# HansiZeng/RIPOR

Hardware: AMD Instinct MI355X
Metric: queries/sec, t5-base beam=10 len=32 over 8.8M-doc trie (constrained beam search) (higher is better)
Workload: dtype f32 via f16x2-split MFMA (fp32 accumulate)

## Files before the change

include/ripor_hip.h:

```cpp
#ifndef RIPOR_HIP_H
#define RIPOR_HIP_H

#include <stdint.h>

#ifdef __cplusplus
extern "C" {
#endif

typedef enum {
  RPR_OK = 0,
  RPR_ERR_INVALID = -1,
  RPR_ERR_HIP = -2,
  RPR_ERR_NO_DEVICE = -3,
  RPR_ERR_OOM = -4
} rpr_status;

typedef struct rpr_ctx rpr_ctx;
typedef struct rpr_model rpr_model;
typedef struct rpr_trie rpr_trie;

typedef struct {
  int32_t vocab_size, d_model, d_kv, d_ff, num_heads;
  int32_t num_layers, num_decoder_layers;
  int32_t rel_buckets, rel_max_distance;
// ... 62 lines not shown
int rpr_abi_version(void);
int rpr_set_precision(rpr_ctx* ctx, int precision);
int rpr_get_precision(const rpr_ctx* ctx);

int rpr_rel_bucket(int rel, int bidirectional, int num_buckets, int max_distance);

int rpr_load_model(rpr_ctx* ctx, const rpr_model_desc* desc, rpr_model** out_model);
void rpr_free_model(rpr_model* model);

int rpr_build_trie(rpr_ctx* ctx, const uint16_t* codes, int64_t N, int32_t L, int32_t V, rpr_trie** out_trie);
void rpr_free_trie(rpr_trie* trie);
int64_t rpr_trie_num_rows(const rpr_trie* trie);
const int64_t* rpr_trie_perm(const rpr_trie* trie);
int rpr_trie_save(const rpr_trie* trie, const char* path);
int rpr_trie_build_file(const uint16_t* codes, int64_t N, int32_t L, int32_t V, const char* keys, int64_t key_bytes,
                        int64_t src_size, int64_t src_mtime_ns, const char* path);
int rpr_trie_file_info(const char* path, int64_t* N, int32_t* L, int32_t* V, int64_t* key_bytes, int64_t* src_size,
                       int64_t* src_mtime_ns);
int rpr_trie_load(rpr_ctx* ctx, const char* path, rpr_trie** out_trie);
int rpr_trie_file_validate(const char* path);
int rpr_trie_dims(const rpr_trie* trie, int64_t* N, int32_t* L, int32_t* V, int64_t* key_bytes);
int rpr_trie_keys(const rpr_trie* trie, char* out);
int rpr_trie_set_vocab(rpr_trie* trie, int32_t V);
int rpr_trie_mask(rpr_ctx* ctx, const rpr_trie* trie, const int32_t* prefix, int32_t R, int32_t T,
                  uint8_t* out_mask);

typedef struct rpr_d2s rpr_d2s;
int rpr_d2s_open(const char* path, rpr_d2s** out);
int rpr_d2s_dims(const rpr_d2s* h, int64_t* N, int32_t* L, int64_t* key_bytes);
int rpr_d2s_copy(const rpr_d2s* h, uint16_t* codes, char* keys);
void rpr_d2s_close(rpr_d2s* h);

int rpr_search(rpr_ctx* ctx, rpr_model* model, rpr_trie* trie, const int32_t* input_ids,
               const int32_t* attention_mask, int32_t Q, int32_t Lq, int32_t B, int32_t L, uint32_t flags,
               int32_t* out_tokens, float* out_scores, int64_t* out_row_lo, int64_t* out_row_hi,
               const rpr_debug_taps* taps, void* stream);

int rpr_search_margins(rpr_ctx* ctx, rpr_model* model, rpr_trie* trie, const int32_t* input_ids,
                       const int32_t* attention_mask, int32_t Q, int32_t Lq, int32_t B, int32_t L, uint32_t flags,
                       int32_t* out_tokens, float* out_scores, int64_t* out_row_lo, int64_t* out_row_hi,
                       double* out_margin, const rpr_debug_taps* taps, void* stream);

int rpr_set_lane_split(rpr_ctx* ctx, int32_t min_rows);
int32_t rpr_lane_split(rpr_ctx* ctx);

int rpr_set_forced_tail(rpr_ctx* ctx, int32_t mode);
int32_t rpr_forced_tail(const rpr_ctx* ctx);
int rpr_set_fork_depths(rpr_ctx* ctx, int32_t n, const int32_t* depths);
int rpr_fork_depths(rpr_ctx* ctx, rpr_model* model, rpr_trie* trie, int32_t Q, int32_t B, int32_t L, uint32_t flags,
                    int32_t* out_depths);
int rpr_set_l0_table(rpr_ctx* ctx, int32_t mode);
int64_t rpr_l0_table_bytes(const rpr_ctx* ctx, const rpr_model* model);
int rpr_trie_single_frac(const uint16_t* codes, int64_t N, int32_t Lc, int32_t L, double* out_frac);
int rpr_last_fork_stats(rpr_ctx* ctx, int32_t* out_depths, int32_t* out_forced, int32_t* out_left);

int rpr_lngknp_forward(rpr_ctx* ctx, rpr_model* model, const int32_t* input_ids, const int32_t* attention_mask,
                       int32_t bz, int32_t Lq, const int32_t* doc_codes, int32_t n_docs, int32_t L,
                       const float* teacher_pos, const float* teacher_neg, const int32_t* prefix_lens, int32_t n_prefix,
                       float* out_losses, float* out_position_scores, void* stream);

int64_t rpr_param_count(rpr_model* model);
int64_t rpr_param_total(rpr_model* model);
int rpr_param_info(rpr_model* model, int64_t index, const float** ptr, int64_t* numel, int64_t* offset);
int rpr_lngknp_backward(rpr_ctx* ctx, rpr_model* model, const int32_t* input_ids, const int32_t* attention_mask, int32_t bz,
                        int32_t Lq, const int32_t* doc_codes, int32_t L, const float* teacher_pos, const float* teacher_neg,
                        const int32_t* prefix_lens, int32_t n_prefix, float* out_losses, float* flat_grads, void* stream);
typedef void (*rpr_grad_bucket_cb)(void* user, int64_t offset, int64_t numel);
int rpr_lngknp_backward_buckets(rpr_ctx* ctx, rpr_model* model, const int32_t* input_ids, const int32_t* attention_mask,
                                int32_t bz, int32_t Lq, const int32_t* doc_codes, int32_t L, const float* teacher_pos,
                                const float* teacher_neg, const int32_t* prefix_lens, int32_t n_prefix, float* out_losses,
                                float* flat_grads, void* stream, void* comm_stream, rpr_grad_bucket_cb on_bucket, void* user);
int rpr_seq2seq_forward(rpr_ctx* ctx, rpr_model* model, const int32_t* input_ids, const int32_t* attention_mask, int32_t bz,
                        int32_t Lq, const int32_t* labels, int32_t L, float* out_loss, float* out_label_logprob, void* stream);
int rpr_seq2seq_backward(rpr_ctx* ctx, rpr_model* model, const int32_t* input_ids, const int32_t* attention_mask, int32_t bz,
                         int32_t Lq, const int32_t* labels, int32_t L, float* out_loss, float* flat_grads, void* stream);
int rpr_seq2seq_backward_buckets(rpr_ctx* ctx, rpr_model* model, const int32_t* input_ids, const int32_t* attention_mask,
                                 int32_t bz, int32_t Lq, const int32_t* labels, int32_t L, float* out_loss, float* flat_grads,
                                 void* stream, void* comm_stream, rpr_grad_bucket_cb on_bucket, void* user);
int rpr_adamw_step(rpr_ctx* ctx, rpr_model* model, const float* flat_grads, float* exp_avg, float* exp_avg_sq, int64_t step,
                   float lr, float beta1, float beta2, float eps, float weight_decay, float max_grad_norm,
                   float* out_grad_norm, void* stream);

#define RPR_STATUS_SATURATED 1u
#define RPR_STATUS_EMPTY_QUERY 2u
#define RPR_STATUS_TAIL_LEFTOVER 4u
int rpr_get_status(rpr_ctx* ctx, void* stream, uint32_t* out_flags, int clear);
int rpr_status_words_async(rpr_ctx* ctx, void* stream, uint32_t* host_words, int clear);
int rpr_model_f32_only(const rpr_model* model);

int rpr_profile_enable(rpr_ctx* ctx, int enable);
int rpr_profile_reset(rpr_ctx* ctx);
int rpr_profile_get(rpr_ctx* ctx, int kernel_class, rpr_kernel_stats* out);
int64_t rpr_workspace_bytes(const rpr_ctx* ctx);

int rpr_op_linear(rpr_ctx* ctx, const float* A, const float* W, const float* residual, float* C,
                  int32_t M, int32_t N, int32_t K, int32_t relu, void* stream);
int rpr_op_linear_bf16(rpr_ctx* ctx, const float* A, const float* W, const float* residual, float* C,
                       int32_t M, int32_t N, int32_t K, int32_t relu, int32_t n_products, void* stream);
int rpr_op_rmsnorm(rpr_ctx* ctx, const float* x, const float* w, float* out, int32_t rows, int32_t d,
                   float eps, void* stream);
int rpr_encode(rpr_ctx* ctx, rpr_model* model, const int32_t* input_ids, const int32_t* attention_mask,
               int32_t Q, int32_t Lq, float* out, void* stream);

int rpr_rq_train(rpr_ctx* ctx, const float* x, int64_t n, int32_t d, int32_t M, int32_t K, int32_t niter,
                 const int32_t* init_idx, float* codebooks, double* level_mse, void* stream);
int rpr_rq_encode(rpr_ctx* ctx, const float* x, int64_t n, int32_t d, const float* codebooks, int32_t M, int32_t K,
// ... 17 lines not shown
```

ripor_amd/_lib.py:

```python
from __future__ import annotations

import ctypes as C
import os
from typing import Optional

LIB_NAME = "libripor_hip_dev.so" if os.environ.get("RPR_DEV_LIB", "0") not in ("", "0") else "libripor_hip.so"
LIB_PATH = os.path.join(os.path.dirname(os.path.abspath(__file__)), LIB_NAME)

(K_GEMM, K_DEC_SELF_ATTN, K_DEC_CROSS_ATTN, K_ENC_ATTN, K_RMSNORM, K_SELECT, K_OTHER, K_GEMM_SMALL, K_TAIL_SELF_ATTN, K_FORK,
 K_COUNT) = range(11)
KERNEL_CLASS_NAMES = ["gemm", "dec_self_attn", "dec_cross_attn", "enc_attn", "rmsnorm", "select", "other", "gemm_small",
                      "tail_self_attn", "fork"]
STATUS_SATURATED, STATUS_EMPTY_QUERY, STATUS_TAIL_LEFTOVER = 1, 2, 4
ABI_VERSION = 4

PREC_F32, PREC_F16X2, PREC_BF16 = 0, 1, 2
FLAG_LOG_SOFTMAX = 1
FLAG_NO_GRAPH = 2


class RiporHipError(RuntimeError):
    pass


# ... 50 lines not shown
                                     C.POINTER(C.c_int64), C.POINTER(C.c_int64), C.POINTER(C.c_int64)]),
    "rpr_trie_file_validate": (C.c_int, [C.c_char_p]),
    "rpr_trie_dims": (C.c_int, [C.c_void_p, C.POINTER(C.c_int64), C.POINTER(C.c_int32), C.POINTER(C.c_int32),
                                C.POINTER(C.c_int64)]),
    "rpr_trie_keys": (C.c_int, [C.c_void_p, C.c_void_p]),
    "rpr_trie_set_vocab": (C.c_int, [C.c_void_p, C.c_int32]),
    "rpr_d2s_open": (C.c_int, [C.c_char_p, C.POINTER(C.c_void_p)]),
    "rpr_d2s_dims": (C.c_int, [C.c_void_p, C.POINTER(C.c_int64), C.POINTER(C.c_int32), C.POINTER(C.c_int64)]),
    "rpr_d2s_copy": (C.c_int, [C.c_void_p, C.c_void_p, C.c_void_p]),
    "rpr_d2s_close": (None, [C.c_void_p]),
    "rpr_trie_mask": (C.c_int, [C.c_void_p, C.c_void_p, C.c_void_p, C.c_int32, C.c_int32, C.c_void_p]),
    "rpr_search": (C.c_int, [C.c_void_p, C.c_void_p, C.c_void_p, C.c_void_p, C.c_void_p, C.c_int32, C.c_int32,
                             C.c_int32, C.c_int32, C.c_uint32, C.c_void_p, C.c_void_p, C.c_void_p, C.c_void_p,
                             C.POINTER(DebugTaps), C.c_void_p]),
    "rpr_search_margins": (C.c_int, [C.c_void_p, C.c_void_p, C.c_void_p, C.c_void_p, C.c_void_p, C.c_int32, C.c_int32,
                                     C.c_int32, C.c_int32, C.c_uint32, C.c_void_p, C.c_void_p, C.c_void_p, C.c_void_p,
                                     C.c_void_p, C.POINTER(DebugTaps), C.c_void_p]),
    "rpr_lngknp_forward": (C.c_int, [C.c_void_p, C.c_void_p, C.c_void_p, C.c_void_p, C.c_int32, C.c_int32, C.c_void_p,
                                     C.c_int32, C.c_int32, C.c_void_p, C.c_void_p, C.c_void_p, C.c_int32, C.c_void_p,
                                     C.c_void_p, C.c_void_p]),
    "rpr_param_count": (C.c_int64, [C.c_void_p]),
    "rpr_param_total": (C.c_int64, [C.c_void_p]),
    "rpr_param_info": (C.c_int, [C.c_void_p, C.c_int64, C.POINTER(C.c_void_p), C.POINTER(C.c_int64), C.POINTER(C.c_int64)]),
    "rpr_lngknp_backward": (C.c_int, [C.c_void_p, C.c_void_p, C.c_void_p, C.c_void_p, C.c_int32, C.c_int32, C.c_void_p, C.c_int32,
                                      C.c_void_p, C.c_void_p, C.c_void_p, C.c_int32, C.c_void_p, C.c_void_p, C.c_void_p]),
    "rpr_lngknp_backward_buckets": (C.c_int, [C.c_void_p, C.c_void_p, C.c_void_p, C.c_void_p, C.c_int32, C.c_int32, C.c_void_p,
                                              C.c_int32, C.c_void_p, C.c_void_p, C.c_void_p, C.c_int32, C.c_void_p, C.c_void_p,
                                              C.c_void_p, C.c_void_p, C.c_void_p, C.c_void_p]),
    "rpr_seq2seq_forward": (C.c_int, [C.c_void_p, C.c_void_p, C.c_void_p, C.c_void_p, C.c_int32, C.c_int32, C.c_void_p, C.c_int32,
                                      C.c_void_p, C.c_void_p, C.c_void_p]),
    "rpr_seq2seq_backward": (C.c_int, [C.c_void_p, C.c_void_p, C.c_void_p, C.c_void_p, C.c_int32, C.c_int32, C.c_void_p, C.c_int32,
                                       C.c_void_p, C.c_void_p, C.c_void_p]),
    "rpr_seq2seq_backward_buckets": (C.c_int, [C.c_void_p, C.c_void_p, C.c_void_p, C.c_void_p, C.c_int32, C.c_int32, C.c_void_p,
                                               C.c_int32, C.c_void_p, C.c_void_p, C.c_void_p, C.c_void_p, C.c_void_p, C.c_void_p]),
    "rpr_adamw_step": (C.c_int, [C.c_void_p, C.c_void_p, C.c_void_p, C.c_void_p, C.c_void_p, C.c_int64, C.c_float, C.c_float,
                                 C.c_float, C.c_float, C.c_float, C.c_float, C.c_void_p, C.c_void_p]),
    "rpr_get_status": (C.c_int, [C.c_void_p, C.c_void_p, C.POINTER(C.c_uint32), C.c_int]),
    "rpr_status_words_async": (C.c_int, [C.c_void_p, C.c_void_p, C.c_void_p, C.c_int]),
    "rpr_model_f32_only": (C.c_int, [C.c_void_p]),
    "rpr_profile_enable": (C.c_int, [C.c_void_p, C.c_int]),
    "rpr_profile_reset": (C.c_int, [C.c_void_p]),
    "rpr_profile_get": (C.c_int, [C.c_void_p, C.c_int, C.POINTER(KernelStats)]),
    "rpr_workspace_bytes": (C.c_int64, [C.c_void_p]),
    "rpr_set_lane_split": (C.c_int, [C.c_void_p, C.c_int32]),
    "rpr_lane_split": (C.c_int32, [C.c_void_p]),
    "rpr_set_l0_table": (C.c_int, [C.c_void_p, C.c_int32]),
    "rpr_l0_table_bytes": (C.c_int64, [C.c_void_p, C.c_void_p]),
    "rpr_set_forced_tail": (C.c_int, [C.c_void_p, C.c_int32]),
    "rpr_forced_tail": (C.c_int32, [C.c_void_p]),
    "rpr_set_fork_depths": (C.c_int, [C.c_void_p, C.c_int32, C.POINTER(C.c_int32)]),
    "rpr_fork_depths": (C.c_int, [C.c_void_p, C.c_void_p, C.c_void_p, C.c_int32, C.c_int32, C.c_int32, C.c_uint32,
                                  C.POINTER(C.c_int32)]),
    "rpr_trie_single_frac": (C.c_int, [C.c_void_p, C.c_int64, C.c_int32, C.c_int32, C.POINTER(C.c_double)]),
    "rpr_last_fork_stats": (C.c_int, [C.c_void_p, C.POINTER(C.c_int32), C.POINTER(C.c_int32), C.POINTER(C.c_int32)]),
    "rpr_op_linear": (C.c_int, [C.c_void_p, C.c_void_p, C.c_void_p, C.c_void_p, C.c_void_p, C.c_int32, C.c_int32,
                                C.c_int32, C.c_int32, C.c_void_p]),
    "rpr_op_linear_bf16": (C.c_int, [C.c_void_p, C.c_void_p, C.c_void_p, C.c_void_p, C.c_void_p, C.c_int32, C.c_int32,
                                     C.c_int32, C.c_int32, C.c_int32, C.c_void_p]),
    "rpr_op_rmsnorm": (C.c_int, [C.c_void_p, C.c_void_p, C.c_void_p, C.c_void_p, C.c_int32, C.c_int32, C.c_float,
                                 C.c_void_p]),
    "rpr_encode": (C.c_int, [C.c_void_p, C.c_void_p, C.c_void_p, C.c_void_p, C.c_int32, C.c_int32, C.c_void_p,
                             C.c_void_p]),
    "rpr_rq_train": (C.c_int, [C.c_void_p, C.c_void_p, C.c_int64, C.c_int32, C.c_int32, C.c_int32, C.c_int32,
                               C.POINTER(C.c_int32), C.c_void_p, C.POINTER(C.c_double), C.c_void_p]),
    "rpr_rq_encode": (C.c_int, [C.c_void_p, C.c_void_p, C.c_int64, C.c_int32, C.c_void_p, C.c_int32, C.c_int32,
                                C.c_void_p, C.POINTER(C.c_double), C.c_void_p]),
    "rpr_rq_encode_beam": (C.c_int, [C.c_void_p, C.c_void_p, C.c_int64, C.c_int32, C.c_void_p, C.c_int32, C.c_int32, C.c_int32,
                                     C.c_void_p, C.POINTER(C.c_double), C.c_void_p]),
    "rpr_embed": (C.c_int, [C.c_void_p, C.c_void_p, C.c_void_p, C.c_void_p, C.c_int32, C.c_int32, C.c_void_p, C.c_void_p]),
    "rpr_rq_search": (C.c_int, [C.c_void_p, C.c_void_p, C.c_int32, C.c_int32, C.c_void_p, C.c_int32, C.c_int32, C.c_void_p,
                                C.c_int64, C.c_int32, C.c_void_p, C.c_void_p, C.c_void_p]),
    "rpr_flat_search": (C.c_int, [C.c_void_p, C.c_void_p, C.c_int32, C.c_int32, C.c_void_p, C.c_int64, C.c_int64, C.c_int32,
                                  C.c_void_p, C.c_void_p, C.c_int32, C.c_void_p]),
}

_lib: Optional[C.CDLL] = None


def load() -> C.CDLL:
    global _lib
    if _lib is not None:
        return _lib
    if not os.path.exists(LIB_PATH):
        raise RiporHipError(
            f"{LIB_PATH} not found: build it with `python -c 'import __graft_entry__ as g; g.build()'` "
            "(hipcc --offload-arch=gfx950). There is no CPU fallback for the search path.")
    import torch
    hip_rt = os.path.join(os.path.dirname(torch.__file__), "lib", "libamdhip64.so")
    if os.path.exists(hip_rt):
        C.CDLL(hip_rt, mode=C.RTLD_GLOBAL)
    lib = C.CDLL(LIB_PATH)
    for name, (res, args) in SIGNATURES.items():
        fn = getattr(lib, name)
        fn.restype = res
        fn.argtypes = args
    _lib = lib
    return lib


def check(status: int, what: str = "") -> None:
    if status != 0:
        msg = load().rpr_last_error()
        raise RiporHipError(f"{what or 'libripor_hip'} failed (status {status}): "
                            f"{msg.decode('utf-8', 'replace') if msg else ''}")
```

ripor_amd/csrc/api.hip:

```cpp
#include <algorithm>
#include <cmath>
#include <cstdio>
#include <cstdlib>
#include <cstring>
#include <map>
#include <memory>
#include <tuple>
#include <vector>

#include "internal.h"

namespace rpr {

static thread_local std::string g_err;
void set_error(const std::string& msg) { g_err = msg; }
int hip_fail(hipError_t e, const char* what, const char* file, int line) {
  g_err = std::string("HIP error ") + hipGetErrorName(e) + " (" + hipGetErrorString(e) + ") in " + what + " at " +
          file + ":" + std::to_string(line);
  (void)hipGetLastError();
  return e == hipErrorOutOfMemory ? RPR_ERR_OOM : RPR_ERR_HIP;
}

int rel_bucket(int rel, int bidirectional, int num_buckets, int max_distance) {
  int bucket = 0, n;
  if (bidirectional) {
    num_buckets /= 2;
    if (rel > 0) bucket += num_buckets;
    n = rel < 0 ? -rel : rel;
  } else {
    n = rel < 0 ? -rel : 0;
  }
  const int max_exact = num_buckets / 2;
  if (n < max_exact) return bucket + n;
  const float v = logf((float)n / (float)max_exact) / (float)log((double)max_distance / (double)max_exact) *
                  (float)(num_buckets - max_exact);
  int large = max_exact + (int)v;
  if (large > num_buckets - 1) large = num_buckets - 1;
  return bucket + large;
}

int compute_logit_bound(rpr_ctx* c, rpr_model* m, hipStream_t s, float* out) {
  const auto& d = m->d;
  float* slot = reinterpret_cast<float*>(c->status + 9);
  RPR_HIP(hipMemsetAsync(slot, 0, 4, s));
  RPR_HIP(launch_max_row_norm(d.out_embeds, d.dec_final_ln, d.L * d.V, d.d_model, slot, s));
  float mx = 0.f;
  RPR_HIP(hipMemcpyAsync(&mx, slot, 4, hipMemcpyDeviceToHost, s));
  RPR_HIP(hipStreamSynchronize(s));
  const float post = d.scaleup_output_hidden ? (float)pow((double)d.d_model, -0.5) : 1.0f;
  *out = 1.001f * mx * sqrtf((float)d.d_model) * post + 1.0f;
  return RPR_OK;
}

int refresh_weight_planes(rpr_ctx* c, rpr_model* m, hipStream_t s) {
  unsigned int* probe = c->status + 8;
  RPR_HIP(hipMemsetAsync(probe, 0, 4, s));
  for (const auto& j : m->plane_jobs)
    RPR_HIP(launch_split_planes(j.w, j.dst, j.n, j.plane_stride ? j.plane_stride : j.n, s, W_PLANE_SCALE * j.pre, j.ln, m->d.d_model, probe));
  unsigned int sat = 0;
  RPR_HIP(hipMemcpyAsync(&sat, probe, 4, hipMemcpyDeviceToHost, s));
  RPR_HIP(hipStreamSynchronize(s));
  m->f32_only = sat != 0;
  m->l0_valid = false;
  float lb = m->logit_bound;
  const int e = compute_logit_bound(c, m, s, &lb);
  if (e) return e;
  if (lb != m->logit_bound) {
    m->logit_bound = lb;
    for (auto it = c->graphs.begin(); it != c->graphs.end();) {
      if (it->first.m == m) { (void)hipGraphExecDestroy(it->second); it = c->graphs.erase(it); } else ++it;
    }
  }
  return RPR_OK;
}

}

using namespace rpr;

namespace {

struct PrecGuard {
  rpr_ctx* c; int saved;
  PrecGuard(rpr_ctx* c_, const rpr_model* m) : c(c_), saved(c_->precision) {
    if (c->precision == RPR_PREC_BF16) c->precision = RPR_PREC_F16X2;
    if (m && m->f32_only) c->precision = RPR_PREC_F32;
  }
  ~PrecGuard() { c->precision = saved; }
};

int flush_profile(rpr_ctx* c) {
  std::map<const int*, int> live;
  for (auto& r : c->recs) {
    RPR_HIP(hipEventSynchronize(r.b));
    float ms = 0.f;
    RPR_HIP(hipEventElapsedTime(&ms, r.a, r.b));
    double scale = 1.0;
    if (r.live_dev && r.live_static > 0) {
      auto it = live.find(r.live_dev);
      if (it == live.end()) {
        int n = r.live_static;
        RPR_HIP(hipMemcpy(&n, r.live_dev, sizeof(int), hipMemcpyDeviceToHost));
        it = live.emplace(r.live_dev, n).first;
      }
      scale = (double)std::min(std::max(it->second, 0), r.live_static) / (double)r.live_static;
    }
    auto& d = c->done[r.cls];
    d.total_ms += ms; d.launches += 1; d.flops += r.flops * scale; d.bytes += r.bytes * scale;
    c->pool.push_back(r.a); c->pool.push_back(r.b);
  }
  c->recs.clear();
  return 0;
}

}

extern "C" {

int rpr_abi_version(void) { return 4; }
const char* rpr_last_error(void) { return g_err.c_str(); }

int rpr_rel_bucket(int rel, int bidirectional, int num_buckets, int max_distance) {
  return rel_bucket(rel, bidirectional, num_buckets, max_distance);
}

int rpr_init(int device, rpr_ctx** out_ctx) {
// ... 240 lines not shown

int64_t rpr_trie_num_rows(const rpr_trie* t) { return t ? t->N : 0; }
const int64_t* rpr_trie_perm(const rpr_trie* t) { return t ? t->perm.data() : nullptr; }

int rpr_trie_save(const rpr_trie* t, const char* path) {
  RPR_REQUIRE(t && path, "NULL argument");
  if (save_trie_file(path, t->host_sorted, t->perm, t->N, t->L, t->V, t->keys, 0, 0) != 0) {
    set_error(std::string("cannot write trie file ") + path);
    return RPR_ERR_INVALID;
  }
  return RPR_OK;
}

int rpr_trie_build_file(const uint16_t* codes, int64_t N, int32_t L, int32_t V, const char* keys, int64_t key_bytes,
                        int64_t src_size, int64_t src_mtime_ns, const char* path) {
  RPR_REQUIRE(codes && path, "NULL argument");
  RPR_REQUIRE(N > 0 && N < ((int64_t)1 << 31) - 1, "N out of range");
  RPR_REQUIRE(L >= 1 && L <= 4096 && V >= 1 && V <= 65536, "L or V out of range");
  RPR_REQUIRE(key_bytes >= 0 && (key_bytes == 0 || keys), "keys missing");
  for (int64_t i = 0; i < N * L; ++i) RPR_REQUIRE(codes[i] < V, "code >= V");
  try {
    std::vector<uint16_t> sorted;
    std::vector<int64_t> perm;
    sort_codes(codes, N, L, sorted, perm);
    const std::string k = key_bytes ? std::string(keys, (size_t)key_bytes) : std::string();
    if (save_trie_file(path, sorted, perm, N, L, V, k, src_size, src_mtime_ns) != 0) {
      set_error(std::string("cannot write trie file ") + path);
      return RPR_ERR_INVALID;
    }
  } catch (const std::exception& ex) {
    set_error(std::string("rpr_trie_build_file: ") + ex.what());
    return RPR_ERR_OOM;
  }
  return RPR_OK;
}

int rpr_trie_single_frac(const uint16_t* codes, int64_t N, int32_t Lc, int32_t L, double* out_frac) {
  RPR_REQUIRE(codes && out_frac, "NULL argument");
  RPR_REQUIRE(N > 0 && N < ((int64_t)1 << 31) - 1 && Lc >= 1 && Lc <= 4096 && L >= 1 && L <= Lc, "N, Lc or L out of range");
  try {
    std::vector<uint16_t> sorted;
    std::vector<int64_t> perm;
    sort_codes(codes, N, Lc, sorted, perm);
    std::vector<double> f;
    trie_single_frac(sorted.data(), N, Lc, L, f);
    for (int t = 0; t <= L; ++t) out_frac[t] = f[(size_t)t];
  } catch (const std::exception& ex) {
    set_error(std::string("rpr_trie_single_frac: ") + ex.what());
    return RPR_ERR_OOM;
  }
  return RPR_OK;
}

int rpr_trie_file_info(const char* path, int64_t* N, int32_t* L, int32_t* V, int64_t* key_bytes, int64_t* src_size,
                       int64_t* src_mtime_ns) {
  RPR_REQUIRE(path, "NULL argument");
  int64_t h[6];
  if (trie_file_info(path, h) != 0) { set_error(std::string("not a readable RPRTRIE2 file: ") + path); return RPR_ERR_INVALID; }
  if (N) *N = h[0];
  if (L) *L = (int32_t)h[1];
  if (V) *V = (int32_t)h[2];
  if (key_bytes) *key_bytes = h[3];
  if (src_size) *src_size = h[4];
  if (src_mtime_ns) *src_mtime_ns = h[5];
  return RPR_OK;
}

int rpr_trie_file_validate(const char* path) {
  RPR_REQUIRE(path, "NULL argument");
  try {
    std::vector<uint16_t> sorted; std::vector<int64_t> perm; std::string keys, err;
    int64_t N; int L, V;
    if (load_trie_file(path, sorted, perm, N, L, V, keys, err) != 0) {
      set_error(std::string("invalid trie file ") + path + ": " + err);
      return RPR_ERR_INVALID;
    }
  } catch (const std::exception& ex) {
    set_error(std::string("rpr_trie_file_validate: ") + ex.what());
    return RPR_ERR_OOM;
  }
  return RPR_OK;
}

int rpr_trie_load(rpr_ctx* c, const char* path, rpr_trie** out) {
  RPR_REQUIRE(c && path && out, "NULL argument");
  try {
    auto t = std::make_unique<rpr_trie>();
    t->ctx = c;
    std::string err;
    if (load_trie_file(path, t->host_sorted, t->perm, t->N, t->L, t->V, t->keys, err) != 0) {
      set_error(std::string("cannot load trie file ") + path + ": " + err);
      return RPR_ERR_INVALID;
    }
    int e = upload_trie(c, t);
    if (e) return e;
    *out = t.release();
  } catch (const std::exception& ex) {
    set_error(std::string("rpr_trie_load: ") + ex.what());
    return RPR_ERR_OOM;
  }
  return RPR_OK;
}

int rpr_trie_dims(const rpr_trie* t, int64_t* N, int32_t* L, int32_t* V, int64_t* key_bytes) {
  RPR_REQUIRE(t, "NULL trie");
  if (N) *N = t->N;
// ... 61 lines not shown
  DevTmp dp, dm;
  RPR_HIP(dp.alloc((size_t)R * T * 4));
  RPR_HIP(dm.alloc((size_t)R * t->V));
  RPR_HIP(hipMemcpy(dp.p, prefix, (size_t)R * T * 4, hipMemcpyHostToDevice));
  RPR_HIP(launch_prefix_mask(t->codes, t->L, t->N, dp.as<int32_t>(), R, T, t->V, dm.as<uint8_t>(), nullptr));
  RPR_HIP(hipMemcpy(out_mask, dm.p, (size_t)R * t->V, hipMemcpyDeviceToHost));
  return RPR_OK;
}

}

namespace {

bool ensure_lanes(rpr_ctx* c) {
  if (c->lanes_state) return c->lanes_state > 0;
  c->lanes_state = -1;
  hipDeviceProp_t prop;
  if (hipGetDeviceProperties(&prop, c->device) != hipSuccess) { (void)hipGetLastError(); return false; }
  const int cus = prop.multiProcessorCount, words = (cus + 31) / 32;
  if (cus < 64 || words > 32) return false;
  c->lane_cus = cus / 2;
  for (int i = 0; i < 2; ++i) {
    uint32_t mask[32] = {0};
    for (int k = (i == 0 ? 0 : cus / 2); k < (i == 0 ? cus / 2 : cus); ++k) mask[k >> 5] |= 1u << (k & 31);
    if (hipExtStreamCreateWithCUMask(&c->lanes[i].stream, (uint32_t)words, mask) != hipSuccess ||
        hipEventCreateWithFlags(&c->lanes[i].done, hipEventDisableTiming) != hipSuccess) {
      (void)hipGetLastError();
      return false;
    }
  }
  if (hipEventCreateWithFlags(&c->fork_ev, hipEventDisableTiming) != hipSuccess) { (void)hipGetLastError(); return false; }
  c->lanes_state = 1;
  return true;
}

std::vector<int> choose_forks(rpr_ctx* c, const rpr_model* m, rpr_trie* tr, int Q, int B, int L, unsigned flags, bool taps,
                              bool* drop_last) {
  std::vector<int> forks;
  *drop_last = false;
  if (!c->forced_tail || taps || L < 3 || !std::isfinite(m->logit_bound)) return forks;
  const double per_step = 2.0 * (double)m->logit_bound + ((flags & RPR_FLAG_LOG_SOFTMAX) ? log((double)m->d.V) : 0.0);
  if (1e8 - L * per_step <= 1e7) return forks;
  if (c->n_fork_override >= 0) {
    int prev = 0;
    for (int i = 0; i < c->n_fork_override; ++i) {
      const int t = c->fork_override[i];
      if (t > prev && t <= L - 1) { forks.push_back(t); prev = t; }
    }
    *drop_last = c->forced_tail == 2 && !forks.empty();
    return forks;
  }
  auto it = tr->single_frac.find(L);
  if (it == tr->single_frac.end()) {
    std::vector<double> f;
    trie_single_frac(tr->host_sorted.data(), tr->N, tr->L, L, f);
    it = tr->single_frac.emplace(L, std::move(f)).first;
  }
  const std::vector<double>& f = it->second;
  auto p_forced = [&](int t) { return std::pow(f[(size_t)t], (double)B); };
  int t0 = 0;
  for (int t = 1; t <= L - 2 && !t0; ++t) if (p_forced(t) >= 0.5) t0 = t;
  const int min_tail = (int64_t)Q * B <= 4096 ? 2 : 8;
  if (!t0 || L - t0 < min_tail) return forks;
  forks.push_back(t0);
  if (c->forced_tail == 2 && (double)Q * (1.0 - p_forced(t0)) <= 0.05) { *drop_last = true; return forks; }
  for (int t = t0 + 1; t <= L - 2 && t <= t0 + 12; ++t)
    if ((double)Q * (1.0 - p_forced(t)) <= 0.05) { forks.push_back(t); break; }
  *drop_last = c->forced_tail == 2 && forks.size() == 2;
  return forks;
}

int pack_forks(const std::vector<int>& forks, bool drop_last) {
  int v = drop_last ? (1 << 30) : 0;
  for (size_t i = 0; i < forks.size(); ++i) v |= forks[i] << (8 * i);
  return v;
}

int search_one(rpr_ctx* c, rpr_model* m, rpr_trie* tr, const int32_t* input_ids, const int32_t* attention_mask, int32_t Q,
               int32_t Lq, int32_t B, int32_t L, uint32_t flags, int32_t* out_tokens, float* out_scores, int64_t* out_row_lo,
               int64_t* out_row_hi, double* out_margin, const rpr_debug_taps* taps, hipStream_t s, int lane) {
  struct WsGuard {
    rpr_ctx* c; int lane;
    WsGuard(rpr_ctx* c_, int l) : c(c_), lane(l) { if (lane >= 0) { std::swap(c->ws, c->lanes[lane].ws); c->cur_cus = c->lane_cus; c->cur_lane = lane; } }
    ~WsGuard() { if (lane >= 0) { std::swap(c->ws, c->lanes[lane].ws); c->cur_cus = 0; c->cur_lane = -1; } }
  } ws_guard(c, lane);
  PrecGuard prec_guard(c, m);
  bool drop_last = false;
  const std::vector<int> forks = choose_forks(c, m, tr, Q, B, L, flags, taps != nullptr, &drop_last);
  int e = alloc_workspace(c, m, Q, Lq, B, L, forks, drop_last, (flags & RPR_FLAG_LOG_SOFTMAX) != 0);
  if (e) return e;
  c->last_forks = forks;
  c->last_ws_mask |= lane >= 0 ? (2 << lane) : 1;
  Workspace& w = c->ws;
  const size_t T = (size_t)Q * Lq, R = (size_t)Q * B;
  RPR_HIP(hipMemcpyAsync(w.ids.p, input_ids, T * 4, hipMemcpyDeviceToDevice, s));
  RPR_HIP(hipMemcpyAsync(w.mask.p, attention_mask, T * 4, hipMemcpyDeviceToDevice, s));

  const bool eager = (flags & RPR_FLAG_NO_GRAPH) || taps || c->profiling;
  if (eager) {
    Launcher Ln{c, s};
    enqueue_search(Ln, c, m, tr, Q, Lq, B, L, flags, taps, forks, drop_last);
    if (Ln.err) return Ln.err;
  } else {
    auto env_int = [](const char* n, int dflt) { const char* e = getenv(n); return e ? atoi(e) : dflt; };
    const unsigned dbg = (env_int("RPR_TAIL_RANK_REPLAY", 0) ? 1u : 0u) | ((unsigned)(env_int("RPR_SELECT_RADIX", -1) + 1) << 1);
    const unsigned l0 = m->l0_ready(c) ? (unsigned)c->l0_mode : 0u;
    const unsigned mg = c->cur_margins ? 1u : 0u;
    GraphKey key{m, tr, Q, Lq, B, L, flags | ((unsigned)c->precision << 16) | (dbg << 20) | (l0 << 24) | (mg << 28), lane,
                 pack_forks(forks, drop_last)};
    auto it = c->graphs.find(key);
    if (it == c->graphs.end()) {
      hipGraph_t graph = nullptr;
      RPR_HIP(hipStreamBeginCapture(c->cap_stream, hipStreamCaptureModeThreadLocal));
      Launcher Ln{c, c->cap_stream};
      enqueue_search(Ln, c, m, tr, Q, Lq, B, L, flags, nullptr, forks, drop_last);
      hipError_t ce = hipStreamEndCapture(c->cap_stream, &graph);
      if (Ln.err) { if (graph) (void)hipGraphDestroy(graph); return Ln.err; }
      if (ce != hipSuccess) return hip_fail(ce, "hipStreamEndCapture", __FILE__, __LINE__);
      hipGraphExec_t exec = nullptr;
      hipError_t ie = hipGraphInstantiate(&exec, graph, nullptr, nullptr, 0);
      (void)hipGraphDestroy(graph);
      if (ie != hipSuccess) return hip_fail(ie, "hipGraphInstantiate", __FILE__, __LINE__);
      it = c->graphs.emplace(key, exec).first;
    }
    RPR_HIP(hipGraphLaunch(it->second, s));
  }
  RPR_HIP(hipMemcpyAsync(out_tokens, w.o_tokens.p, R * (size_t)L * 4, hipMemcpyDeviceToDevice, s));
  RPR_HIP(hipMemcpyAsync(out_scores, w.o_scores.p, R * 4, hipMemcpyDeviceToDevice, s));
  if (out_row_lo) RPR_HIP(hipMemcpyAsync(out_row_lo, w.o_lo.p, R * 8, hipMemcpyDeviceToDevice, s));
  if (out_row_hi) RPR_HIP(hipMemcpyAsync(out_row_hi, w.o_hi.p, R * 8, hipMemcpyDeviceToDevice, s));
  if (out_margin) RPR_HIP(hipMemcpyAsync(out_margin, w.o_margin.p, (size_t)Q * 8, hipMemcpyDeviceToDevice, s));
  return RPR_OK;
}

int search_entry(rpr_ctx* c, rpr_model* m, rpr_trie* tr, const int32_t* input_ids, const int32_t* attention_mask,
                 int32_t Q, int32_t Lq, int32_t B, int32_t L, uint32_t flags, int32_t* out_tokens, float* out_scores,
                 int64_t* out_row_lo, int64_t* out_row_hi, double* out_margin, const rpr_debug_taps* taps, void* stream) {
  RPR_REQUIRE(c && m && tr && input_ids && attention_mask && out_tokens && out_scores, "NULL argument");
  struct MarginMode { rpr_ctx* c; MarginMode(rpr_ctx* c_, bool on) : c(c_) { c->cur_margins = on ? 1 : 0; } ~MarginMode() { c->cur_margins = 0; } }
      margin_mode(c, out_margin != nullptr);
  RPR_REQUIRE(m->ctx == c && tr->ctx == c, "model/trie belong to another ctx");
  RPR_REQUIRE(Q >= 1 && B >= 1 && B <= 65535, "Q or B out of range");
  RPR_REQUIRE(Lq >= 1 && Lq <= MAX_LQ, "Lq out of range (1..256)");
  RPR_REQUIRE(L >= 1 && L <= m->d.L && L <= tr->L, "L exceeds the model's decoder length or the trie depth");
  RPR_REQUIRE(tr->V == m->d.V, "trie V differs from the model's decoder vocab size");
  RPR_REQUIRE((int64_t)Q * B < ((int64_t)1 << 24), "Q*B too large");
  RPR_REQUIRE((int64_t)Q * B * m->d.num_heads < ((int64_t)1 << 32) / std::max<int64_t>(B, m->d.num_heads),
              "Q * num_beams * num_heads too large for this beam count: search fewer queries per call");
  RPR_REQUIRE(select_fits(B, m->Vp()), "num_beams * decoder vocab size too large for the select kernel (about 1600 beams at V=256)");
  RPR_REQUIRE(!taps || m->Vp() == m->d.V, "debug taps need a decoder vocab size that is a multiple of 64");
  RPR_HIP(hipSetDevice(c->device));
  hipStream_t s = reinterpret_cast<hipStream_t>(stream);
  { const int pe = ensure_weight_planes(c, m, s); if (pe) return pe; }
  { const int te = ensure_l0_table(c, m, s); if (te) return te; }
  c->last_ws_mask = 0;
  if (c->lane_min_rows > 0 && (int64_t)Q * B >= c->lane_min_rows && Q >= 2 && !taps && ensure_lanes(c)) {
    const int32_t Qh[2] = {(Q + 1) / 2, Q / 2};
    for (int i = 0; i < 2; ++i) {
      std::swap(c->ws, c->lanes[i].ws);
      int e;
      {
        PrecGuard prec_guard(c, m);
// ... 14 lines not shown
                         out_tokens + r0 * L, out_scores + r0, out_row_lo ? out_row_lo + r0 : nullptr,
                         out_row_hi ? out_row_hi + r0 : nullptr, out_margin ? out_margin + q0 : nullptr, nullptr, ln.stream, i);
      if (e) {
        for (int k = 0; k < 2; ++k) (void)hipStreamSynchronize(c->lanes[k].stream);
        return e;
      }
      RPR_HIP(hipEventRecord(ln.done, ln.stream));
      q0 += Qh[i];
    }
    for (int i = 0; i < 2; ++i) RPR_HIP(hipStreamWaitEvent(s, c->lanes[i].done, 0));
    return RPR_OK;
  }
  return search_one(c, m, tr, input_ids, attention_mask, Q, Lq, B, L, flags, out_tokens, out_scores, out_row_lo, out_row_hi, out_margin,
                    taps, s, -1);
}

}

extern "C" {

int rpr_search(rpr_ctx* c, rpr_model* m, rpr_trie* tr, const int32_t* input_ids, const int32_t* attention_mask,
               int32_t Q, int32_t Lq, int32_t B, int32_t L, uint32_t flags, int32_t* out_tokens, float* out_scores,
               int64_t* out_row_lo, int64_t* out_row_hi, const rpr_debug_taps* taps, void* stream) {
  return search_entry(c, m, tr, input_ids, attention_mask, Q, Lq, B, L, flags, out_tokens, out_scores, out_row_lo, out_row_hi,
                      nullptr, taps, stream);
}

int rpr_search_margins(rpr_ctx* c, rpr_model* m, rpr_trie* tr, const int32_t* input_ids, const int32_t* attention_mask,
                       int32_t Q, int32_t Lq, int32_t B, int32_t L, uint32_t flags, int32_t* out_tokens, float* out_scores,
                       int64_t* out_row_lo, int64_t* out_row_hi, double* out_margin, const rpr_debug_taps* taps, void* stream) {
  RPR_REQUIRE(out_margin != nullptr, "out_margin is NULL");
  return search_entry(c, m, tr, input_ids, attention_mask, Q, Lq, B, L, flags, out_tokens, out_scores, out_row_lo, out_row_hi,
                      out_margin, taps, stream);
}

int rpr_set_lane_split(rpr_ctx* c, int32_t min_rows) {
  RPR_REQUIRE(c && min_rows >= 0, "NULL ctx or negative threshold");
  c->lane_min_rows = min_rows;
  return RPR_OK;
}
int32_t rpr_lane_split(rpr_ctx* c) {
  if (!c || c->lane_min_rows <= 0) return 0;
  (void)hipSetDevice(c->device);
  return ensure_lanes(c) ? c->lane_min_rows : 0;
}

int rpr_set_l0_table(rpr_ctx* c, int32_t mode) {
  RPR_REQUIRE(c && mode >= 0 && mode <= 2, "mode must be 0 (never), 1 (where the ping-pong GEMM would run) or 2 (always)");
  c->l0_mode = mode;
  return RPR_OK;
}
int64_t rpr_l0_table_bytes(const rpr_ctx* c, const rpr_model* m) { return c && m && m->l0_ready(c) ? (int64_t)m->l0_bytes() : 0; }

int rpr_set_forced_tail(rpr_ctx* c, int32_t mode) {
  RPR_REQUIRE(c && mode >= 0 && mode <= 2, "mode must be 0 (off), 1 (exact) or 2 (optimistic)");
  c->forced_tail = mode;
  return RPR_OK;
}
int32_t rpr_forced_tail(const rpr_ctx* c) { return c ? c->forced_tail : -1; }

int rpr_set_fork_depths(rpr_ctx* c, int32_t n, const int32_t* depths) {
  RPR_REQUIRE(c && n >= -1 && n <= MAX_FORKS && (n <= 0 || depths), "n out of range (-1 = automatic, 0..2 explicit depths)");
  c->n_fork_override = n;
  for (int i = 0; i < n; ++i) {
    RPR_REQUIRE(depths[i] >= 1 && depths[i] < 256 && (i == 0 || depths[i] > depths[i - 1]), "fork depths must be ascending and >= 1");
    c->fork_override[i] = depths[i];
  }
  return RPR_OK;
}

int rpr_fork_depths(rpr_ctx* c, rpr_model* m, rpr_trie* tr, int32_t Q, int32_t B, int32_t L, uint32_t flags, int32_t* out_depths) {
  RPR_REQUIRE(c && m && tr && out_depths, "NULL argument");
  RPR_REQUIRE(Q >= 1 && B >= 1 && L >= 1 && L <= tr->L, "Q, B or L out of range");
  bool drop_last = false;
  const std::vector<int> f = choose_forks(c, m, tr, Q, B, L, flags, false, &drop_last);
  for (size_t i = 0; i < f.size(); ++i) out_depths[i] = f[i];
  return (int)f.size();
}

int rpr_last_fork_stats(rpr_ctx* c, int32_t* out_depths, int32_t* out_forced, int32_t* out_left) {
  RPR_REQUIRE(c && out_depths && out_forced && out_left, "NULL argument");
  RPR_HIP(hipSetDevice(c->device));
  RPR_HIP(hipDeviceSynchronize());
  const int n = (int)c->last_forks.size();
  for (int k = 0; k < n; ++k) {
    out_depths[k] = c->last_forks[(size_t)k]; out_forced[k] = 0; out_left[k] = 0;
    const Workspace* wss[3] = {&c->ws, &c->lanes[0].ws, &c->lanes[1].ws};
    for (int i = 0; i < 3; ++i) {
      if (!(c->last_ws_mask & (1 << i)) || !wss[i]->tail[k].cnt.p || !wss[i]->stage[k].cnt.p) continue;
      int32_t a = 0, b = 0;
      RPR_HIP(hipMemcpy(&a, wss[i]->tail[k].cnt.p, 4, hipMemcpyDeviceToHost));
      RPR_HIP(hipMemcpy(&b, wss[i]->stage[k].cnt.p, 4, hipMemcpyDeviceToHost));
      out_forced[k] += a; out_left[k] += b;
    }
  }
  return n;
}

int rpr_lngknp_forward(rpr_ctx* c, rpr_model* m, const int32_t* input_ids, const int32_t* attention_mask, int32_t bz,
                       int32_t Lq, const int32_t* doc_codes, int32_t n_docs, int32_t L, const float* teacher_pos,
                       const float* teacher_neg, const int32_t* prefix_lens, int32_t n_prefix, float* out_losses,
                       float* out_position_scores, void* stream) {
  RPR_REQUIRE(c && m && input_ids && attention_mask && doc_codes, "NULL argument");
  RPR_REQUIRE(m->ctx == c, "model belongs to another ctx");
  RPR_REQUIRE(bz >= 1 && Lq >= 1 && Lq <= MAX_LQ, "bz or Lq out of range");
  RPR_REQUIRE(L >= 1 && L <= m->d.L && L <= MAX_LQ, "smtid length exceeds the model's decoder length");
  RPR_REQUIRE(n_docs >= 1 && (int64_t)bz * n_docs * L < ((int64_t)1 << 24), "n_docs out of range");
  RPR_REQUIRE(m->d.d_kv == DKV, "the teacher-forced kernels are written for d_kv == 64 (t5-base / t5-large)");
  RPR_REQUIRE(n_prefix >= 0 && n_prefix <= 8, "n_prefix out of range (0..8)");
  RPR_REQUIRE(n_prefix == 0 || (n_docs == 2 && teacher_pos && teacher_neg && prefix_lens && out_losses),
              "the margin losses need n_docs == 2 (positive, negative), teacher scores, prefix lengths and out_losses");
  RPR_REQUIRE(out_losses || out_position_scores, "nothing to return");
  RPR_HIP(hipSetDevice(c->device));
  hipStream_t s = reinterpret_cast<hipStream_t>(stream);
  int e = ensure_weight_planes(c, m, s);
  if (e) return e;
  e = alloc_train_workspace(c, m, bz, Lq, n_docs, L);
  if (e) return e;
  Workspace& w = c->ws;
  const size_t T = (size_t)bz * Lq, R = (size_t)bz * n_docs * L;
  RPR_HIP(hipMemcpyAsync(w.ids.p, input_ids, T * 4, hipMemcpyDeviceToDevice, s));
  RPR_HIP(hipMemcpyAsync(w.mask.p, attention_mask, T * 4, hipMemcpyDeviceToDevice, s));
  float* scores = P<float>(w.tr_misc);
  int32_t* codes = reinterpret_cast<int32_t*>(scores + R);
  RPR_HIP(hipMemcpyAsync(codes, doc_codes, R * 4, hipMemcpyDeviceToDevice, s));
  PrecGuard prec_guard(c, m);
  Launcher Ln{c, s};
  enqueue_train_forward(Ln, c, m, bz, Lq, n_docs, L, codes, scores);
  if (Ln.err) return Ln.err;
  if (n_prefix > 0)
    RPR_HIP(launch_margin_mse(scores, teacher_pos, teacher_neg, prefix_lens, n_prefix, bz, L, out_losses, nullptr, s));
  if (out_position_scores) RPR_HIP(hipMemcpyAsync(out_position_scores, scores, R * 4, hipMemcpyDeviceToDevice, s));
  return RPR_OK;
}

int rpr_encode(rpr_ctx* c, rpr_model* m, const int32_t* input_ids, const int32_t* attention_mask, int32_t Q,
               int32_t Lq, float* out, void* stream) {
  RPR_REQUIRE(c && m && input_ids && attention_mask && out, "NULL argument");
  RPR_REQUIRE(Q >= 1 && Lq >= 1 && Lq <= MAX_LQ, "Q or Lq out of range");
  RPR_HIP(hipSetDevice(c->device));
  hipStream_t s = reinterpret_cast<hipStream_t>(stream);
  int e = ensure_weight_planes(c, m, s);
  if (e) return e;
  e = alloc_workspace(c, m, Q, Lq, 1, 1);
// ... 157 lines not shown
```

ripor_amd/csrc/common.h:

```cpp
#pragma once
#include <hip/hip_runtime.h>
#include <hip/hip_fp16.h>
#include <stdint.h>
#include <stdlib.h>
#include <string>

#include "../../include/ripor_hip.h"

namespace rpr {

constexpr int WAVE = 64;
constexpr int MAX_LQ = 256;
constexpr int MAX_DEC_LEN = 64;
constexpr int DKV = 64;

#ifdef RPR_DEV_SWITCHES
inline const char* dev_getenv(const char* name) { return getenv(name); }
#else
inline const char* dev_getenv(const char*) { return nullptr; }
#endif

void set_error(const std::string& msg);
int hip_fail(hipError_t e, const char* what, const char* file, int line);

// ... 341 lines not shown
  const int* nq_dev;
};
hipError_t launch_select(const SelectArgs& a, hipStream_t s);
bool select_radix_fits(int B, int V);
bool select_radix_wanted(int B, int V);
size_t select_radix_ws_bytes(int Q, int B, int V);
void select_radix_carve(RadixWs& w, void* base, int32_t* chi, int Q, int B, int V);
hipError_t init_select_radix_attributes();
hipError_t launch_select_radix_reset(const RadixWs& w, int Q, hipStream_t s);
hipError_t launch_select_radix(const SelectArgs& a, hipStream_t s);
bool select_fits(int B, int V);

struct MarginArgs {
  const float* logits;
  const double* cur_score;
  const double* nxt_score;
  const unsigned long long* valid;
  const uint16_t* codes; int Lc, t;
  const int32_t* cur_lo; const int32_t* cur_hi;
  int Q, B, V, Vreal, log_softmax, shared0;
  const int* nq_dev;
  const int32_t* qmap;
  double* out;
};
constexpr int MARGIN_MAX_V = 65536;
hipError_t launch_margin_init(double* out, int Q, hipStream_t s);
hipError_t launch_prune_margin(const MarginArgs& a, hipStream_t s);

struct FinalizeArgs {
  BeamState st;
  int Q, B, L;
  int32_t* out_tokens;
  float* out_scores;
  int64_t* out_lo;
  int64_t* out_hi;
  const int* nq_dev;
  const int32_t* qmap;
};
hipError_t launch_finalize(const FinalizeArgs& a, hipStream_t s);

hipError_t launch_prefix_mask(const uint16_t* codes, int Lc, int64_t N, const int32_t* prefix, int R, int T,
                              int V, uint8_t* out_mask, hipStream_t s);
hipError_t launch_zero_u64(unsigned long long* p, size_t n, hipStream_t s);
hipError_t launch_mask_lengths(const int32_t* mask, int32_t* lens, int Q, int Lq, hipStream_t s,
                               unsigned int* status = nullptr);

struct ForkArgs {
  BeamState st;
  const uint16_t* codes; int Lc;
  int Qcap; const int* nq_dev;
  int B, T, L;
  double spread_max;
  int32_t* flag;
};
hipError_t launch_fork_classify(const ForkArgs& a, hipStream_t s);
hipError_t launch_fork_scan(const int32_t* flag, int Qcap, const int* nq_dev, int B, int Lt, int32_t* flist, int32_t* tail_cnt,
                            int32_t* src, int32_t* next_cnt, hipStream_t s);
struct StageIO {
  const int32_t* qmap;
  const int32_t* offs;
  const int32_t* last;
  const int32_t* mask;
};
struct StageOut { int32_t* qmap; int32_t* offs; int32_t* last; int32_t* mask; };
hipError_t launch_gather_stage_io(const StageIO& src, const StageOut& dst, const int32_t* list, const int* n_dev, int Qcap, int Lq,
                                  hipStream_t s);
hipError_t launch_compact_beams(const BeamState& from, const BeamState& to, const int32_t* src, const int* n_dev, int Qcap, int B, int T,
                                hipStream_t s);
struct KvCopyArgs {
  const float* k_from; const float* v_from; float* k_to; float* v_to;
  size_t layer_from, q_from, h_from;
  size_t layer_to, q_to, h_to;
  const int32_t* src; const int* n_dev;
  int Qcap, nd, H, n;
};
hipError_t launch_kv_copy(const KvCopyArgs& a, hipStream_t s);
hipError_t launch_tail_tokens(const BeamState& st, const uint16_t* codes, int Lc, const int32_t* flist, const int* nf_dev, int Qcap,
                              int B, int T, int L, uint16_t* tokens, hipStream_t s);
hipError_t launch_tail_embed(const float* in_embeds, const uint16_t* tokens, float* out, int rows, const int* rows_dev, int T, int L,
                             int d, int V, hipStream_t s, XOut xo = XOut{});
hipError_t launch_tail_l0_qkv(const float* table, const uint16_t* tokens, float* qkv, int rows, const int* rows_dev, int T, int L,
                              int V, int n3, hipStream_t s);
struct TailSelfAttnArgs {
  const float* qkv;
  const float* kcache;
  const float* vcache;
  size_t q_stride, h_stride, pos_stride, slot_stride;
  const uint16_t* anc; int anc_ld;
  const int32_t* flist;
  const int* nseq_dev;
  const float* rel_bias; const int32_t* bucket;
  float* out; __half* out_h; size_t o_ps; unsigned int* sat;
  int nseq_cap, B, H, T, L;
  int dkv = 0;
};
hipError_t launch_tail_self_attn(const TailSelfAttnArgs& a, hipStream_t s);
hipError_t launch_tail_cross_attn(const DecCrossAttnArgs& a, hipStream_t s);
hipError_t launch_step_cross_attn(const DecCrossAttnArgs& a, hipStream_t s);
hipError_t launch_tail_gold(const float* x, const float* ln, const float* out_embeds, const uint16_t* tokens, float* gold, int rows,
                            const int* rows_dev, int T, int L, int d, int V, float eps, float post, hipStream_t s,
                            const __half* x_h = nullptr, size_t x_ps = 0);
hipError_t launch_tail_logprob(const float* logits, const uint16_t* tokens, float* gold, int rows, const int* rows_dev, int T, int L,
                               int V, hipStream_t s);
struct TailRankArgs {
  BeamState st;
  const int32_t* flist; const int32_t* qmap; const int* nf_dev;
  const uint16_t* tokens;
  const float* gold;
  int Qcap, B, T, L;
  int32_t* out_tokens; float* out_scores; int64_t* out_lo; int64_t* out_hi;
  int replay = 0;
};
hipError_t launch_tail_rank(const TailRankArgs& a, hipStream_t s);
hipError_t launch_flag_nonzero(const int* cnt, unsigned int* flag, hipStream_t s);
hipError_t launch_max_row_norm(const float* E, const float* w, int rows, int d, float* out , hipStream_t s);
hipError_t init_tail_kernel_attributes();

hipError_t launch_train_dec_embed(const float* start, const float* in_embeds, const int32_t* codes, float* out, int S,
                                  int L, int d, int V, hipStream_t s, XOut xo = XOut{});
hipError_t launch_gold_scores(const float* x, const float* ln, const float* out_embeds, const int32_t* codes, float* scores,
                              int S, int L, int d, int V, float eps, float post, hipStream_t s,
                              const __half* x_h = nullptr, size_t x_ps = 0, float* hidden = nullptr);
hipError_t launch_margin_mse(const float* scores, const float* teacher_pos, const float* teacher_neg, const int32_t* prefix_lens,
                             int n_prefix, int bz, int L, float* losses, float* margins, hipStream_t s);
hipError_t init_train_kernel_attributes();
hipError_t launch_absmax2(const float* x0, size_t n0, const float* x1, size_t n1, float* out, hipStream_t s);
hipError_t launch_split_dyn(const float* x, int R, int C, int ldi, __half* out, const float* amax, hipStream_t s);
hipError_t launch_split_dyn_T(const float* x, int R, int C, int ldi, int Rpad, __half* out_t, __half* out_plain, const float* amax,
                              hipStream_t s);
hipError_t launch_to_bf16(const float* x, int R, int C, int ldi, void* out, hipStream_t s);
hipError_t launch_to_bf16_T(const float* x, int R, int C, int ldi, int Rpad, void* out_t, void* out_plain, hipStream_t s,
                            const float* relu_act = nullptr, int ldt = 0);
struct WSeg { const float* src; int R, C; unsigned long long off; };
hipError_t launch_weights_bf16(const WSeg* segs, const int* pref, int nseg, int ntiles, void* plain, void* tr, hipStream_t s);
hipError_t launch_transpose_pad(const float* in, float* out, int R, int C, int ldi, int Rpad, hipStream_t s);
hipError_t launch_relu_bwd(float* dy, const float* act, size_t n, hipStream_t s);
hipError_t launch_rmsnorm_bf16_T(const float* x, const float* w, int rows, int d, float eps, float post, void* out_plain, void* out_t,
                                 int Rpad, int ldt, hipStream_t s);
hipError_t launch_rmsnorm_bwd(const float* x, const float* w, const float* dh, const float* dres, float* dx_out, float* w_part,
                              float* dw, int rows, int d, float eps, float post, int accumulate_dw, hipStream_t s);
struct ColsumSites {
  static constexpr int MAXS = 4;
  const float* part[MAXS]; float* out[MAXS]; int nparts[MAXS]; int n;
};
int rmsnorm_bwd_parts(int rows);
hipError_t launch_colsum_multi(const ColsumSites& p, int d, hipStream_t s);
size_t self_attn_bwd_smem(int Ls, int buckets);
hipError_t launch_self_attn_bwd(const float* qkv, const float* dO, const int32_t* mask, const float* rel_bias, const int32_t* bucket,
                                float* dqkv, float* dbias_part, float* dbias, int S, int Ls, int H, int buckets, int causal,
                                hipStream_t s);
size_t cross_attn_bwd_smem(int n, int Lq);
hipError_t launch_cross_attn_bwd(const float* q, const float* xk, const float* xv, int xld, const int32_t* mask, const float* dO,
                                 float* dq, float* dxk, float* dxv, int bz, int n, int Lq, int H, hipStream_t s);
hipError_t launch_scatter_rows_fix(const float* src, const int32_t* idx, unsigned long long* acc, int rows, int d, hipStream_t s);
hipError_t launch_fix_flush(unsigned long long* acc, float* dst, size_t n, hipStream_t s);
hipError_t launch_train_indices(const int32_t* codes, int32_t* in_idx, int32_t* out_idx, int S, int L, int V, hipStream_t s);
hipError_t launch_sum_selected_rows(const float* src, const int32_t* sel, float* out, int rows, int d, hipStream_t s);
hipError_t launch_margin_mse_bwd(const float* margins, const float* teacher_pos, const float* teacher_neg, const int32_t* prefix_lens,
                                 int n_prefix, int bz, int L, float* dscores, hipStream_t s);
hipError_t launch_gold_score_bwd(const float* x, const float* ln, const float* out_embeds, const int32_t* out_idx, const float* dscores,
                                 float* dh, float* de, int rows, int d, float eps, float post, hipStream_t s);
int s2s_head_smem_ok(int V);
hipError_t launch_s2s_head_fwd(const float* hF, const float* E, const int32_t* labels, float* dlogits, float* row_loss, float* label_lp,
                               float* loss, int bz, int L, int d, int V, hipStream_t s);
// ... 10 lines not shown
```

ripor_amd/csrc/internal.h:

```cpp
#pragma once
#include <map>
#include <memory>
#include <string>
#include <tuple>
#include <type_traits>
#include <vector>

#include "common.h"
#include "gemm_route.h"
#include "trie.h"

namespace rpr {

struct DevBuf {
  void* p = nullptr;
  size_t cap = 0;
};

}

using rpr::DevBuf;

struct rpr_model {
  rpr_ctx* ctx;
// ... 9 lines not shown
  int Vp() const { return (d.V + 63) & ~63; }
  bool f32_only = false;
  bool planes_dirty = false;
  float* l0_table = nullptr;
  bool l0_valid = false;
  unsigned l0_epoch = 0;
  int l0_state = 0;
  size_t l0_rows() const { return rpr::l0_table_rows(d.L, d.V); }
  size_t l0_bytes() const { return rpr::l0_table_bytes(d.L, d.V, inner()); }
  bool l0_ready(const rpr_ctx* c) const;
  std::vector<void*> owned;
  struct PlaneJob { const float* w; size_t n; __half* dst; const float* ln; float pre; size_t plane_stride; };
  std::vector<PlaneJob> plane_jobs;
  struct ParamRef { int kind; int layer; float* ptr; size_t numel; size_t offset; };
  std::vector<ParamRef> params;
  size_t params_total = 0;
  float logit_bound = INFINITY;
  int inner() const { return d.num_heads * d.d_kv; }
  ~rpr_model() {
    if (enc_bucket) (void)hipFree(enc_bucket);
    if (dec_bucket) (void)hipFree(dec_bucket);
    for (void* p : owned) (void)hipFree(p);
  }
};

struct rpr_trie {
  rpr_ctx* ctx;
  int64_t N;
  int L, V;
  uint16_t* codes = nullptr;
  int32_t* lvl0 = nullptr;
  int32_t* lvl1 = nullptr;
  int lvl_V = 0;
  int32_t* idx2 = nullptr;
  int32_t* d_start[rpr::TRIE_MAX_DEEP] = {};
  uint16_t* d_tok[rpr::TRIE_MAX_DEEP] = {};
  int d_n[rpr::TRIE_MAX_DEEP] = {};
  int n_deep = 0;
  void free_levels() {
    if (lvl0) (void)hipFree(lvl0);
    if (lvl1) (void)hipFree(lvl1);
    if (idx2) (void)hipFree(idx2);
    for (int i = 0; i < rpr::TRIE_MAX_DEEP; ++i) {
      if (d_start[i]) (void)hipFree(d_start[i]);
      if (d_tok[i]) (void)hipFree(d_tok[i]);
      d_start[i] = nullptr; d_tok[i] = nullptr; d_n[i] = 0;
    }
    lvl0 = lvl1 = idx2 = nullptr; n_deep = 0; lvl_V = 0;
  }
  std::vector<int64_t> perm;
  std::vector<uint16_t> host_sorted;
  std::string keys;
  std::map<int, std::vector<double>> single_frac;
  ~rpr_trie() { if (codes) (void)hipFree(codes); free_levels(); }
};

struct rpr_d2s {
  std::vector<uint16_t> codes;
  std::string keys;
  int64_t N = 0;
  int L = 0;
};

struct GraphKey {
  const rpr_model* m; const rpr_trie* t; int Q, Lq, B, L; unsigned flags; int lane;
  int forks;
  bool operator<(const GraphKey& o) const {
    return std::tie(m, t, Q, Lq, B, L, flags, lane, forks) < std::tie(o.m, o.t, o.Q, o.Lq, o.B, o.L, o.flags, o.lane, o.forks);
  }
};

struct StageBufs {
  DevBuf qmap;
  DevBuf cnt;
  DevBuf src;
  DevBuf offs, last, mask;
  DevBuf kcache, vcache;
  DevBuf score[2], lo[2], hi[2], tokens[2], anc[2];
};
struct TailBufs {
  DevBuf flag, flist;
  DevBuf cnt;
  DevBuf qmap, offs, last, mask;
  DevBuf tokens;
  DevBuf gold;
};
constexpr int MAX_FORKS = 2;

struct Workspace {
  DevBuf ids, mask, last, offs, row_src, ex, eh, eqkv, eattn, eff, enc_out, xkv;
  DevBuf x, h, q, attn, ff, logits, kcache, vcache, lb;
  DevBuf sel_rs;
  DevBuf score[2], lo[2], hi[2], tokens[2], anc[2];
  DevBuf o_tokens, o_scores, o_lo, o_hi;
  DevBuf mg_valid, o_margin;
  DevBuf eattn_h, eff_h, enc_out_h, attn_h, ff_h, ex_h, x_h, ssq_e, ssq_d;
  DevBuf tr_x, tr_misc;
  DevBuf part;
  StageBufs stage[MAX_FORKS];
  TailBufs tail[MAX_FORKS];
  DevBuf t_x, t_h, t_qkv, t_q, t_attn, t_ff, t_x_h, t_attn_h, t_ff_h, t_ssq;
  DevBuf t_logits;
  DevBuf rq_r, rq_code, rq_hist, rq_order, rq_cnorm, rq_part, rq_idx;
  DevBuf rq_lut, rq_sel;
  DevBuf flat_sc;
  DevBuf rq_r2, rq_bnorm, rq_cand, rq_bhist;
};

static_assert(sizeof(Workspace) % sizeof(DevBuf) == 0 && std::is_standard_layout<Workspace>::value,
              "Workspace must consist of DevBuf members only (rpr_free_ctx walks it as an array)");

struct Lane {
  Workspace ws;
  hipStream_t stream = nullptr;
  hipEvent_t done = nullptr;
};

struct rpr_ctx {
  int device;
  int precision = RPR_PREC_F16X2;
  unsigned int* status = nullptr;
  unsigned int* status_host = nullptr;
  struct TrainWs* tws = nullptr;
  Workspace ws;
  Lane lanes[2];
  int lanes_state = 0;
  int lane_min_rows = 10240;
  hipEvent_t fork_ev = nullptr;
  int cur_cus = 0;
  int lane_cus = 0;
  int cur_lane = -1;
  int cur_no_row_split = 0;
  int cur_small_live = 0;
  int cur_margins = 0;
  int forced_tail = 1;
  int fork_override[MAX_FORKS] = {0, 0};
  int n_fork_override = -1;
  std::vector<int> last_forks;
  int last_ws_mask = 0;
  size_t ws_bytes = 0;
  int enc_rows_accounted = 0;
  unsigned l0_epoch = 0;
  int l0_mode = 1;
  hipStream_t cap_stream = nullptr;
  std::map<GraphKey, hipGraphExec_t> graphs;
  bool profiling = false;
  struct Rec { int cls; hipEvent_t a, b; double flops, bytes; const int* live_dev; int live_static; };
  std::vector<Rec> recs;
  std::vector<hipEvent_t> pool;
  rpr_kernel_stats done[RPR_K_COUNT];
};

inline bool rpr_model::l0_ready(const rpr_ctx* c) const { return c->l0_mode > 0 && l0_table && l0_valid && l0_epoch == c->l0_epoch; }

namespace rpr {

int refresh_weight_planes(rpr_ctx* c, rpr_model* m, hipStream_t s);
inline int ensure_weight_planes(rpr_ctx* c, rpr_model* m, hipStream_t s) {
  if (!m->planes_dirty) return 0;
  const int e = refresh_weight_planes(c, m, s);
  if (!e) m->planes_dirty = false;
  return e;
}
int ensure_l0_table(rpr_ctx* c, rpr_model* m, hipStream_t s);
void free_train_ws(rpr_ctx* c);
void train_forget_model(rpr_ctx* c, const rpr_model* m);

inline int ensure(rpr_ctx* c, DevBuf& b, size_t bytes) {
  if (bytes <= b.cap) return 0;
  if (b.p) {
    RPR_HIP(hipFree(b.p));
    c->ws_bytes -= b.cap;
    b.p = nullptr; b.cap = 0;
    for (auto& g : c->graphs) (void)hipGraphExecDestroy(g.second);
    c->graphs.clear();
  }
  const size_t want = (bytes + 255) & ~(size_t)255;
  RPR_HIP(hipMalloc(&b.p, want));
  b.cap = want;
  c->ws_bytes += want;
  return 0;
}

template <class T> T* P(const DevBuf& b) { return reinterpret_cast<T*>(b.p); }

struct DevTmp {
  void* p = nullptr;
  hipError_t alloc(size_t bytes) { return hipMalloc(&p, bytes); }
  ~DevTmp() { if (p) (void)hipFree(p); }
  template <class T> T* as() const { return reinterpret_cast<T*>(p); }
};

struct Launcher {
  rpr_ctx* c;
  hipStream_t s;
  int err = 0;
  const int* live_dev = nullptr;
  int live_static = 0;
  void account_live(const int* dev, int rows_static) { live_dev = dev; live_static = rows_static; }
  hipEvent_t get_event() {
    if (!c->pool.empty()) { hipEvent_t e = c->pool.back(); c->pool.pop_back(); return e; }
    hipEvent_t e = nullptr;
    if (hipEventCreate(&e) != hipSuccess) return nullptr;
    return e;
  }
  template <class F> void run(int cls, double flops, double bytes, F&& f, const int* cls_after = nullptr) {
    if (err) return;
    hipEvent_t ea = nullptr, eb = nullptr;
    if (c->profiling) {
// ... 46 lines not shown
```

ripor_amd/csrc/passes.hip:

```cpp
#include <cmath>
#include <vector>

#include "internal.h"

namespace rpr {

LinOut out_f32(float* p, int ld, int N, const float* resid, int relu) {
  LinOut o{};
  o.f[0] = o.f[1] = o.f[2] = p; o.ldo[0] = o.ldo[1] = o.ldo[2] = ld; o.split_n = N; o.resid = resid; o.relu = relu;
  return o;
}

namespace {

GemmH2Args h2_args(const rpr_ctx* c, const LinIn& A, const LinW& W, int M, const LinOut& O, const int* m_dev) {
  const int Nh = W.Nh ? W.Nh : W.N;
  GemmH2Args g{};
  g.A = A.h; g.a_ps = A.ps; g.lda = A.ld; g.W = W.h; g.w_ps = W.ps ? W.ps : (size_t)W.N * W.K; g.ldw = W.K;
  g.resid = O.resid; g.ldr = O.ldo[0];
  for (int i = 0; i < 3; ++i) { g.out[i] = O.f[i]; g.ldo[i] = O.ldo[i]; }
  g.split_n = O.split_n; g.out_h = O.h; g.o_ps = O.ps; g.ldoh = O.ldh;
  g.M = M; g.N = Nh; g.K = W.K; g.relu = O.relu;
  g.rm_B = O.rm_B; g.rm_stride = O.rm_stride; g.rm_slot = O.rm_slot; g.rm_head = O.rm_head; g.rm_dshift = O.rm_dshift;
  g.m_dev = m_dev; g.acc_scale = 1.0f / (W_PLANE_SCALE * A.scale); g.plane_scale = O.plane_scale;
  g.row_ssq = A.ssq; g.inv_d_fix = A.inv_d_fix; g.eps = A.eps;
  g.resid_h = O.resid_h; g.r_ps = O.ps; g.ldrh = O.ldh; g.ssq_out = O.ssq_out;
  g.sat = c->status;
  g.cus = c->cur_cus;
  g.small_live = m_dev ? c->cur_small_live : 0;
  g.no_row_split = W.row_split_ok ? 0 : c->cur_no_row_split;
  g.force_pp = W.force_pp ? 1 : 0;
  if (!W.no_scratch) { g.part = P<float>(c->ws.part); g.part_cap = c->ws.part.cap / sizeof(float); g.mid_split = 1; }
  return g;
}

}

void linear(Launcher& L, const LinIn& A, const LinW& W, int M, const LinOut& O, const int* m_dev, int m_acc) {
  const double Ma = m_acc >= 0 ? m_acc : M;
  const double fl = 2.0 * Ma * (double)W.N * W.K;
  const double by = 4.0 * (Ma * W.K + (double)W.N * W.K + Ma * W.N * ((O.resid || O.resid_h) ? 2 : 1));
  hipStream_t s = L.s;
  if (L.c->precision == RPR_PREC_F16X2) {
    GemmH2Args g = h2_args(L.c, A, W, M, O, m_dev);
    L.run(RPR_K_GEMM, fl, by, [&] { return launch_gemm_h2(g, s); }, &g.kernel_cls);
  } else {
    GemmArgs g{};
    g.A = A.f; g.lda = A.ld; g.W = W.f; g.ldw = W.K; g.resid = O.resid; g.ldr = O.ldo[0];
    for (int i = 0; i < 3; ++i) { g.out[i] = O.f[i]; g.ldo[i] = O.ldo[i]; }
    g.split_n = O.split_n; g.M = M; g.N = W.N; g.K = W.K; g.relu = O.relu;
    g.rm_B = O.rm_B; g.rm_stride = O.rm_stride; g.rm_slot = O.rm_slot; g.rm_head = O.rm_head; g.rm_dshift = O.rm_dshift;
    g.m_dev = m_dev;
    L.run(RPR_K_GEMM, fl, by, [&] { return launch_gemm(g, s); });
  }
}

int alloc_workspace(rpr_ctx* c, const rpr_model* m, int Q, int Lq, int B, int L, const std::vector<int>& forks, bool drop_last, bool log_softmax) {
  const auto& d = m->d;
  const size_t T = (size_t)Q * Lq, R = (size_t)Q * B, inner = m->inner(), dm = d.d_model, dff = d.d_ff;
  const size_t nd = d.num_decoder_layers, ne = d.num_layers, f = sizeof(float);
  Workspace& w = c->ws;
  int e = 0;
  auto E = [&](DevBuf& b, size_t bytes) { if (!e) e = ensure(c, b, bytes); };
  E(w.ids, T * 4); E(w.mask, T * 4); E(w.last, (size_t)Q * 4); E(w.offs, ((size_t)Q + 1) * 4); E(w.row_src, T * 4);
  E(w.ex, T * dm * f); E(w.eh, T * dm * f); E(w.eqkv, T * 3 * inner * f); E(w.eattn, T * inner * f);
  E(w.eff, T * dff * f); E(w.enc_out, T * dm * f); E(w.xkv, T * nd * 2 * inner * f);
  E(w.x, R * dm * f); E(w.h, R * dm * f); E(w.q, R * inner * f); E(w.attn, R * inner * f);
  E(w.ff, R * dff * f); E(w.logits, R * (size_t)m->Vp() * f);
  const size_t depth0 = forks.empty() ? (size_t)L : (size_t)forks[0];
  E(w.kcache, nd * depth0 * R * inner * f); E(w.vcache, nd * depth0 * R * inner * f);
  E(w.lb, R * (size_t)m->Vp() * 4 * 2);
  if (select_radix_wanted(B, m->Vp())) E(w.sel_rs, select_radix_ws_bytes(Q, B, m->Vp()));
  for (int i = 0; i < 2; ++i) {
    E(w.score[i], R * 8); E(w.lo[i], R * 4); E(w.hi[i], R * 4);
    E(w.tokens[i], R * (size_t)L * 2); E(w.anc[i], R * (size_t)L * 2);
  }
  E(w.o_tokens, R * (size_t)L * 4); E(w.o_scores, R * 4); E(w.o_lo, R * 8); E(w.o_hi, R * 8);
  if (c->cur_margins) { E(w.mg_valid, R * (size_t)m->Vp() / 8); E(w.o_margin, (size_t)Q * 8); }
  const size_t hb = sizeof(__half) * 2;
  E(w.eattn_h, T * inner * hb); E(w.eff_h, T * dff * hb); E(w.enc_out_h, T * dm * hb);
  E(w.attn_h, R * inner * hb); E(w.ff_h, R * dff * hb);
  E(w.ex_h, T * dm * hb); E(w.x_h, R * dm * hb);
  E(w.ssq_e, (2 * ne + 1) * T * 8); E(w.ssq_d, (3 * nd + 1) * R * 8);
  E(w.part, (size_t)9 << 20 << 2);
  for (size_t k = 0; k < forks.size(); ++k) {
    const size_t depth = k + 1 < forks.size() ? (size_t)forks[k + 1] : (size_t)L, Lt = (size_t)(L - forks[k]);
    StageBufs& sb = w.stage[k];
    E(sb.cnt, 16); E(sb.src, (size_t)Q * 4);
    if (!(drop_last && k + 1 == forks.size())) {
      E(sb.qmap, (size_t)Q * 4); E(sb.offs, (size_t)Q * 4); E(sb.last, (size_t)Q * 4); E(sb.mask, T * 4);
      E(sb.kcache, nd * depth * R * inner * f); E(sb.vcache, nd * depth * R * inner * f);
      for (int i = 0; i < 2; ++i) {
        E(sb.score[i], R * 8); E(sb.lo[i], R * 4); E(sb.hi[i], R * 4);
        E(sb.tokens[i], R * (size_t)L * 2); E(sb.anc[i], R * (size_t)L * 2);
      }
    }
    TailBufs& tb = w.tail[k];
    E(tb.flag, (size_t)Q * 4); E(tb.flist, (size_t)Q * 4); E(tb.cnt, 16);
    E(tb.qmap, (size_t)Q * 4); E(tb.offs, (size_t)Q * 4); E(tb.last, (size_t)Q * 4); E(tb.mask, T * 4);
    E(tb.tokens, R * (size_t)L * 2); E(tb.gold, R * Lt * f);
  }
  if (!forks.empty()) {
    const size_t Rt = R * (size_t)(L - forks[0]);
    E(w.t_qkv, Rt * 3 * inner * f); E(w.t_q, Rt * inner * f);
    if (c->precision == RPR_PREC_F16X2 && !m->f32_only) {
      E(w.t_x_h, Rt * dm * hb); E(w.t_attn_h, Rt * inner * hb); E(w.t_ff_h, Rt * dff * hb); E(w.t_ssq, (3 * nd + 1) * Rt * 8);
    } else {
      E(w.t_x, Rt * dm * f); E(w.t_h, Rt * dm * f); E(w.t_attn, Rt * inner * f); E(w.t_ff, Rt * dff * f);
    }
    if (log_softmax) { E(w.t_h, Rt * dm * f); E(w.t_logits, Rt * (size_t)d.V * f); }
  }
  return e;
}

namespace {

struct XStream {
  __half* x_h; size_t ps; unsigned long long* ssq; size_t rows; int dm; float eps;
  LinIn in(int site) const {
    LinIn a{nullptr, x_h, ps, dm, X_PLANE_SCALE};
    a.ssq = ssq + (size_t)site * rows; a.inv_d_fix = 1.0f / ((float)dm * SSQ_FIX); a.eps = eps;
    return a;
  }
  LinOut out(int site) const {
    LinOut o{};
    o.split_n = dm; o.h = x_h; o.ps = ps; o.ldh = dm; o.plane_scale = X_PLANE_SCALE;
    o.resid_h = x_h; o.ssq_out = ssq + (size_t)site * rows;
    return o;
  }
};

struct PassBufs { const DevBuf &x, &h, &attn, &ff, &x_h, &attn_h, &ff_h, &ssq; };

struct Pass {
  Launcher& Ln;
  const bool h2;
  const int spl, layers, dm, inner, dff;
  int M; const int* const m_dev; int m_acc;
  const int norm_acc;
  float *const x, *const h, *const attn, *const ff; __half *const attn_h, *const ff_h;
  const size_t ps_i, ps_f;
  const XStream xs;
  const float post;

  Pass(Launcher& Ln_, const rpr_model* m, const PassBufs& b, int spl_, int layers_, int rows_cap, const int* m_dev_, int m_acc_)
      : Ln(Ln_), h2(Ln_.c->precision == RPR_PREC_F16X2), spl(spl_), layers(layers_), dm(m->d.d_model), inner(m->inner()),
        dff(m->d.d_ff), M(rows_cap), m_dev(m_dev_), m_acc(m_acc_), norm_acc(m_acc_), x(P<float>(b.x)), h(P<float>(b.h)),
        attn(P<float>(b.attn)), ff(P<float>(b.ff)), attn_h(P<__half>(b.attn_h)), ff_h(P<__half>(b.ff_h)),
        ps_i((size_t)rows_cap * inner), ps_f((size_t)rows_cap * dff),
        xs{P<__half>(b.x_h), (size_t)rows_cap * dm, P<unsigned long long>(b.ssq), (size_t)rows_cap, dm, m->d.layer_norm_eps},
        post(m->d.scaleup_output_hidden ? (float)pow((double)dm, -0.5) : 1.0f) {}

  void rows(int M_, int m_acc_) { M = M_; m_acc = m_acc_; }
  int site(int layer, int k) const { return layer * spl + k; }
  void zero_ssq() {
    if (h2) Ln.run(RPR_K_OTHER, 0, 0, [&] { return launch_zero_u64(xs.ssq, (size_t)(spl * layers + 1) * xs.rows, Ln.s); });
// ... 181 lines not shown
        DecCrossAttnArgs a{qb, xk, xk + inner, xld, sv.io.mask, p.attn, Q, Bt, H, Lq, p.attn_planes(), p.ps_i,
                           sv.io.last, sv.io.offs, 0, c->status, sv.nq_dev};
        a.dkv = d.d_kv;
        Ln.run(RPR_K_DEC_CROSS_ATTN, 4.0 * Ma * H * (double)Lq * d.d_kv,
               4.0 * ((double)Ma * inner * 2 + 2.0 * (Ma / Bt) * (double)Lq * inner), [&] { return launch_step_cross_attn(a, s); });
      }
      p.attn_out(i, 1, m->dec_xo[i], m->h_dec_xo[i]);
      p.ff_block(i, 2, m->dec_ln2[i], m->dec_wi[i], m->h_dec_wi[i], m->dec_wo[i], m->h_dec_wo[i]);
    }
    float* lg = (taps && taps->step_logits) ? taps->step_logits + (size_t)t * R * V : logits;
    {
      LinW wt{d.out_embeds + (size_t)t * V * dm, m->h_out_embeds + (size_t)t * Vp * dm, V, dm};
      wt.ps = (size_t)d.L * Vp * dm; wt.Nh = Vp; wt.no_scratch = true; wt.row_split_ok = true;
      p.project(p.normed(nd, 0, d.dec_final_ln, p.post), wt, out_f32(lg, Vp, p.h2 ? Vp : V));
    }
    SelectArgs sa{};
    sa.logits = lg; sa.codes = tr->codes; sa.Lc = tr->L; sa.cur = cur; sa.nxt = nxt;
    sa.lb_scratch = P<int32_t>(w.lb); sa.Q = Q; sa.B = B; sa.V = Vp; sa.Vreal = V; sa.t = t;
    if (tr->lvl_V == tr->V) {
      sa.lvl0 = tr->lvl0; sa.lvl1 = tr->lvl1; sa.lvl_V = tr->lvl_V;
      sa.idx2 = tr->idx2; sa.n_deep = tr->n_deep;
      for (int i = 0; i < tr->n_deep; ++i) { sa.d_start[i] = tr->d_start[i]; sa.d_tok[i] = tr->d_tok[i]; sa.d_n[i] = tr->d_n[i]; }
    }
    if (w.sel_rs.p && select_radix_wanted(B, Vp) && w.sel_rs.cap >= select_radix_ws_bytes(Q, B, Vp))
      select_radix_carve(sa.rs, w.sel_rs.p, P<int32_t>(w.lb) + (size_t)R * Vp, Q, B, Vp);
    sa.log_softmax = (sd.flags & RPR_FLAG_LOG_SOFTMAX) ? 1 : 0;
    sa.shared0 = (Bt != B) ? 1 : 0;
    sa.nq_dev = sv.nq_dev;
    if (taps) {
      sa.tap_scores = taps->step_scores ? taps->step_scores + (size_t)t * R : nullptr;
      sa.tap_tokens = taps->step_tokens ? taps->step_tokens + (size_t)t * R : nullptr;
      sa.tap_parent = taps->step_parent ? taps->step_parent + (size_t)t * R : nullptr;
      sa.tap_valid = taps->step_valid ? reinterpret_cast<unsigned long long*>(taps->step_valid) + (size_t)t * ((size_t)R * V / 64) : nullptr;
    }
    if (c->cur_margins && !sa.tap_valid && !sa.shared0) sa.tap_valid = P<unsigned long long>(w.mg_valid);
    Ln.run(RPR_K_SELECT, 0, (double)Ma * V * 4 + (double)Ma * 40, [&] { return launch_select(sa, s); });
    if (c->cur_margins) {
      MarginArgs ma{lg, cur.score, nxt.score, sa.tap_valid, tr->codes, tr->L, t, cur.lo, cur.hi, Q, B, Vp, V, sa.log_softmax,
                    sa.shared0, sv.nq_dev, sv.io.qmap, P<double>(w.o_margin)};
      Ln.run(RPR_K_SELECT, 0, (double)Ma * V * 4, [&] { return launch_prune_margin(ma, s); });
    }
  }
  Ln.account_live(nullptr, 0);
}

StageView enqueue_fork(Launcher& Ln, rpr_ctx* c, const rpr_model* m, const rpr_trie* tr, const SearchDims& sd, const StageView& sv,
                       int T, int next_depth, TailBufs& tb, StageBufs& nb, bool compact) {
  const auto& d = m->d;
  const int Q = sv.Qcap, B = sd.B, L = sd.L, Lq = sd.Lq, inner = m->inner(), nd = d.num_decoder_layers, H = d.num_heads;
  hipStream_t s = Ln.s;
  const BeamState st = sv.st[T & 1];
  const double per_step = (sd.flags & RPR_FLAG_LOG_SOFTMAX) ? 2.0 * (double)m->logit_bound + log((double)d.V) : 2.0 * (double)m->logit_bound;
  const double spread_max = 1e8 - (double)(L - T) * per_step;
  ForkArgs fa{st, tr->codes, tr->L, Q, sv.nq_dev, B, T, L, spread_max, P<int32_t>(tb.flag)};
  Ln.run(RPR_K_FORK, 0, 0, [&] { return launch_fork_classify(fa, s); });
  Ln.run(RPR_K_FORK, 0, 0, [&] {
    return launch_fork_scan(P<int32_t>(tb.flag), Q, sv.nq_dev, B, L - T, P<int32_t>(tb.flist), P<int32_t>(tb.cnt), P<int32_t>(nb.src),
                            P<int32_t>(nb.cnt), s);
  });
  Ln.run(RPR_K_FORK, 0, 0, [&] {
    return launch_gather_stage_io(sv.io, StageOut{P<int32_t>(tb.qmap), P<int32_t>(tb.offs), P<int32_t>(tb.last), P<int32_t>(tb.mask)},
                                  P<int32_t>(tb.flist), P<int>(tb.cnt), Q, Lq, s);
  });
  Ln.run(RPR_K_FORK, 0, 0, [&] {
    return launch_tail_tokens(st, tr->codes, tr->L, P<int32_t>(tb.flist), P<int>(tb.cnt), Q, B, T, L, P<uint16_t>(tb.tokens), s);
  });
  StageView nv{};
  if (!compact) {
    Ln.run(RPR_K_FORK, 0, 0, [&] { return launch_flag_nonzero(P<int>(nb.cnt), c->status + 2, s); });
    return nv;
  }
  nv.Qcap = Q; nv.nq_dev = P<int>(nb.cnt); nv.nrows_dev = P<int>(nb.cnt) + 1;
  nv.io = StageIO{P<int32_t>(nb.qmap), P<int32_t>(nb.offs), P<int32_t>(nb.last), P<int32_t>(nb.mask)};
  nv.kcache = P<float>(nb.kcache); nv.vcache = P<float>(nb.vcache); nv.depth = next_depth; nv.dkv = sv.dkv;
  for (int i = 0; i < 2; ++i) nv.st[i] = beam_state(nb.score, nb.lo, nb.hi, nb.tokens, nb.anc, i, L);
  Ln.run(RPR_K_FORK, 0, 0, [&] {
    return launch_gather_stage_io(sv.io, StageOut{P<int32_t>(nb.qmap), P<int32_t>(nb.offs), P<int32_t>(nb.last), P<int32_t>(nb.mask)},
                                  P<int32_t>(nb.src), nv.nq_dev, Q, Lq, s);
  });
  Ln.run(RPR_K_FORK, 0, 0, [&] { return launch_compact_beams(st, nv.st[T & 1], P<int32_t>(nb.src), nv.nq_dev, Q, B, T, s); });
  KvCopyArgs kc{sv.kcache, sv.vcache, nv.kcache, nv.vcache, sv.kv_layer(B, inner), sv.kv_q(B, inner), sv.kv_h(B),
                nv.kv_layer(B, inner), nv.kv_q(B, inner), nv.kv_h(B), P<int32_t>(nb.src), nv.nq_dev, Q, nd, H, T * B * sv.dkv};
  Ln.run(RPR_K_FORK, 0, 0, [&] { return launch_kv_copy(kc, s); });
  return nv;
}

void enqueue_tail(Launcher& Ln, rpr_ctx* c, const rpr_model* m, const SearchDims& sd, const StageView& sv, int T, TailBufs& tb) {
  const auto& d = m->d;
  Workspace& w = c->ws;
  const int Q = sv.Qcap, B = sd.B, L = sd.L, Lq = sd.Lq, Lt = L - T, S = Q * B, R = S * Lt;
  const int inner = m->inner(), dm = d.d_model, H = d.num_heads, nd = d.num_decoder_layers, V = d.V, xld = sd.xld;
  hipStream_t s = Ln.s;
  const int* nf_dev = P<int>(tb.cnt);
  const int* nseq_dev = nf_dev + 1;
  const int* nrows_dev = nf_dev + 2;
  const int Ra = live_count(Ln, nrows_dev, R);
  float *qkv = P<float>(w.t_qkv), *qb = P<float>(w.t_q);
  Pass p(Ln, m, {w.t_x, w.t_h, w.t_attn, w.t_ff, w.t_x_h, w.t_attn_h, w.t_ff_h, w.t_ssq}, 3, nd, R, nrows_dev, Ra);
  p.zero_ssq();
  Ln.run(RPR_K_OTHER, 0, 2.0 * Ra * dm * 4, [&] {
    return launch_tail_embed(d.in_embeds, P<uint16_t>(tb.tokens), p.x, R, nrows_dev, T, L, dm, V, s, p.embed_out());
  });
  const size_t kv_pos = (size_t)B * sv.dkv;
  for (int i = 0; i < nd; ++i) {
    const LinOut o_qkv = out_f32(qkv, 3 * inner, 3 * inner);
    if (i == 0 && p.l0_replaces(m, o_qkv))
      Ln.run(RPR_K_OTHER, 0, 2.0 * Ra * 3 * inner * 4, [&] {
        return launch_tail_l0_qkv(m->l0_table, P<uint16_t>(tb.tokens), qkv, R, nrows_dev, T, L, V, 3 * inner, s);
      });
    else
      p.project(p.normed(i, 0, m->dec_ln0[i]), {m->dec_qkv[i], m->h_dec_qkv[i], 3 * inner, dm}, o_qkv);
    {
      const size_t ls = sv.kv_layer(B, inner);
      TailSelfAttnArgs a{qkv, sv.kcache + i * ls, sv.vcache + i * ls, sv.kv_q(B, inner), sv.kv_h(B), kv_pos, (size_t)sv.dkv,
                         sv.st[T & 1].anc, L, P<int32_t>(tb.flist), nseq_dev, d.dec_rel_bias, m->dec_bucket, p.attn,
                         p.attn_planes(), p.ps_i, c->status, S, B, H, T, L};
      a.dkv = d.d_kv;
      Ln.run(RPR_K_TAIL_SELF_ATTN, 2.0 * Ra * H * (double)(L + T + 1) * sv.dkv, 4.0 * ((double)Ra * 4 * inner + 2.0 * (Ra / Lt) * (double)T * inner),
             [&] { return launch_tail_self_attn(a, s); });
    }
    p.attn_out(i, 0, m->dec_o[i], m->h_dec_o[i]);
    p.project(p.normed(i, 1, m->dec_ln1[i]), {m->dec_xq[i], m->h_dec_xq[i], inner, dm}, out_f32(qb, inner, inner));
    {
      const float* xk = P<float>(w.xkv) + (size_t)i * 2 * inner;
      DecCrossAttnArgs a{qb, xk, xk + inner, xld, P<int32_t>(tb.mask), p.attn, Q, B * Lt, H, Lq, p.attn_planes(), p.ps_i,
                         P<int32_t>(tb.last), P<int32_t>(tb.offs), 0, c->status, nf_dev};
      a.dkv = d.d_kv;
      Ln.run(RPR_K_DEC_CROSS_ATTN, 4.0 * Ra * H * (double)Lq * sv.dkv, 4.0 * ((double)Ra * inner * 2 + 2.0 * (Ra / (B * Lt)) * (double)Lq * inner),
             [&] { return launch_tail_cross_attn(a, s); });
    }
    p.attn_out(i, 1, m->dec_xo[i], m->h_dec_xo[i]);
    p.ff_block(i, 2, m->dec_ln2[i], m->dec_wi[i], m->h_dec_wi[i], m->dec_wo[i], m->h_dec_wo[i]);
  }
  if (sd.flags & RPR_FLAG_LOG_SOFTMAX) {
    float* lg = P<float>(w.t_logits);
    Ln.run(RPR_K_RMSNORM, 0, 2.0 * Ra * dm * 4, [&] {
      return launch_rmsnorm(p.x, d.dec_final_ln, p.h, R, dm, p.xs.eps, s, p.post, nullptr, 0, nrows_dev, nullptr, p.x_planes(), p.xs.ps);
    });
    for (int pos = T; pos < L; ++pos) {
      GemmArgs g{};
      g.A = p.h + (size_t)(pos - T) * dm; g.lda = Lt * dm;
      g.W = d.out_embeds + (size_t)pos * V * dm; g.ldw = dm;
      for (int i = 0; i < 3; ++i) { g.out[i] = lg + (size_t)(pos - T) * V; g.ldo[i] = Lt * V; }
      g.split_n = V; g.M = S; g.N = V; g.K = dm; g.m_dev = nseq_dev;
      Ln.run(RPR_K_GEMM_SMALL, 2.0 * (Ra / Lt) * (double)V * dm, 4.0 * ((double)(Ra / Lt) * (dm + V) + (double)V * dm),
             [&] { return launch_gemm(g, s); });
    }
    Ln.run(RPR_K_OTHER, 0, 4.0 * Ra * V, [&] {
      return launch_tail_logprob(lg, P<uint16_t>(tb.tokens), P<float>(tb.gold), R, nrows_dev, T, L, V, s);
    });
  } else {
    Ln.run(RPR_K_OTHER, 2.0 * Ra * dm, 4.0 * 2 * Ra * dm, [&] {
      return launch_tail_gold(p.x, d.dec_final_ln, d.out_embeds, P<uint16_t>(tb.tokens), P<float>(tb.gold), R, nrows_dev, T, L, dm, V, p.xs.eps,
                              p.post, s, p.x_planes(), p.xs.ps);
    });
  }
  TailRankArgs ra{sv.st[T & 1], P<int32_t>(tb.flist), P<int32_t>(tb.qmap), nf_dev, P<uint16_t>(tb.tokens), P<float>(tb.gold), Q, B, T, L,
                  P<int32_t>(w.o_tokens), P<float>(w.o_scores), P<int64_t>(w.o_lo), P<int64_t>(w.o_hi)};
  Ln.run(RPR_K_FORK, 0, 0, [&] { return launch_tail_rank(ra, s); });
  Ln.account_live(nullptr, 0);
}

}

void enqueue_search(Launcher& Ln, rpr_ctx* c, const rpr_model* m, const rpr_trie* tr, int Q, int Lq, int B, int L,
                    unsigned flags, const rpr_debug_taps* taps, const std::vector<int>& forks, bool drop_last) {
  const auto& d = m->d;
  Workspace& w = c->ws;
  const int T = Q * Lq, inner = m->inner(), dm = d.d_model;
  const int nd = d.num_decoder_layers;
  hipStream_t s = Ln.s;
  Ln.run(RPR_K_OTHER, 0, 0, [&] { return launch_mask_lengths(P<int32_t>(w.mask), P<int32_t>(w.last), Q, Lq, s, c->status + 1); });
  const bool packed = !taps;
  c->cur_no_row_split = packed ? 1 : 0;
  enqueue_encoder(Ln, c, m, Q, Lq, packed);
  if (taps && taps->encoder_out && !Ln.err) {
    hipError_t e = hipMemcpyAsync(taps->encoder_out, w.enc_out.p, (size_t)T * dm * 4, hipMemcpyDeviceToDevice, s);
    if (e != hipSuccess) { Ln.err = hip_fail(e, "tap copy", __FILE__, __LINE__); return; }
  }
  const int xld = nd * 2 * inner;
  Ln.account_live(packed ? P<int>(w.offs) + Q : nullptr, T);
  linear(Ln, {P<float>(w.enc_out), P<__half>(w.enc_out_h), (size_t)T * dm, dm}, {d.dec_xkv, m->h_dec_xkv, xld, dm}, T,
         out_f32(P<float>(w.xkv), xld, xld), packed ? P<int>(w.offs) + Q : nullptr, c->enc_rows_accounted);
  Ln.account_live(nullptr, 0);
  c->cur_no_row_split = 0;

  const SearchDims sd{Q, Lq, B, L, xld, packed, flags};
  StageView sv{};
  sv.Qcap = Q;
  sv.io = StageIO{nullptr, packed ? P<int32_t>(w.offs) : nullptr, P<int32_t>(w.last), P<int32_t>(w.mask)};
  sv.kcache = P<float>(w.kcache); sv.vcache = P<float>(w.vcache); sv.depth = forks.empty() ? L : forks[0]; sv.dkv = d.d_kv;
  for (int i = 0; i < 2; ++i) sv.st[i] = beam_state(w.score, w.lo, w.hi, w.tokens, w.anc, i, L);
  Ln.run(RPR_K_OTHER, 0, 0, [&] { return launch_init_beams(sv.st[0], Q, B, tr->N, s); });
  if (c->cur_margins) Ln.run(RPR_K_OTHER, 0, 0, [&] { return launch_margin_init(P<double>(w.o_margin), Q, s); });
  if (w.sel_rs.p && select_radix_wanted(B, m->Vp()) && w.sel_rs.cap >= select_radix_ws_bytes(Q, B, m->Vp())) {
    RadixWs rs;
    select_radix_carve(rs, w.sel_rs.p, nullptr, Q, B, m->Vp());
    Ln.run(RPR_K_OTHER, 0, 0, [&] { return launch_select_radix_reset(rs, Q, s); });
  }

  const bool shared0 = !taps && B > 1;
  struct SmallLive { rpr_ctx* c; ~SmallLive() { c->cur_small_live = 0; } } small_guard{c};
  constexpr int small_live_rows = 1024;
  int t0 = 0;
  for (size_t k = 0; k <= forks.size(); ++k) {
    const int t1 = k < forks.size() ? forks[k] : L;
    c->cur_small_live = k >= 1 ? small_live_rows : 0;
    enqueue_steps(Ln, c, m, tr, sd, sv, t0, t1, shared0, taps);
    if (k < forks.size()) {
      const int next_depth = k + 1 < forks.size() ? forks[k + 1] : L;
      const bool last_dropped = drop_last && k + 1 == forks.size();
      const StageView nv = enqueue_fork(Ln, c, m, tr, sd, sv, t1, next_depth, w.tail[k], w.stage[k], !last_dropped);
      enqueue_tail(Ln, c, m, sd, sv, t1, w.tail[k]);
      if (last_dropped) return;
      sv = nv;
    }
    t0 = t1;
  }
  FinalizeArgs fa{sv.st[L & 1], sv.Qcap, B, L, P<int32_t>(w.o_tokens), P<float>(w.o_scores),
                  P<int64_t>(w.o_lo), P<int64_t>(w.o_hi), sv.nq_dev, sv.io.qmap};
  Ln.run(RPR_K_OTHER, 0, 0, [&] { return launch_finalize(fa, s); });
}

void enqueue_train_forward(Launcher& Ln, rpr_ctx* c, const rpr_model* m, int bz, int Lq, int ndoc, int L,
                           const int32_t* codes , float* pos_scores , float* hidden) {
  const auto& d = m->d;
  Workspace& w = c->ws;
  const int T = bz * Lq, S = bz * ndoc, R = S * L, inner = m->inner(), dm = d.d_model, H = d.num_heads;
  const int nd = d.num_decoder_layers, V = d.V;
  hipStream_t s = Ln.s;
  Ln.run(RPR_K_OTHER, 0, 0, [&] { return launch_mask_lengths(P<int32_t>(w.mask), P<int32_t>(w.last), bz, Lq, s, c->status + 1); });
  c->cur_no_row_split = 1;
  enqueue_encoder(Ln, c, m, bz, Lq, true);
  const int xld = nd * 2 * inner;
  linear(Ln, {P<float>(w.enc_out), P<__half>(w.enc_out_h), (size_t)T * dm, dm}, {d.dec_xkv, m->h_dec_xkv, xld, dm}, T,
         out_f32(P<float>(w.xkv), xld, xld), P<int>(w.offs) + bz, c->enc_rows_accounted);
  Ln.account_live(nullptr, 0);
  c->cur_no_row_split = 0;

  float *qkv = P<float>(w.tr_x), *qb = P<float>(w.q);
  Pass p(Ln, m, {w.x, w.h, w.attn, w.ff, w.x_h, w.attn_h, w.ff_h, w.ssq_d}, 3, nd, R, nullptr, R);
  p.zero_ssq();
  Ln.run(RPR_K_OTHER, 0, 2.0 * R * dm * 4, [&] {
    return launch_train_dec_embed(d.start_embed, d.in_embeds, codes, p.x, S, L, dm, V, s, p.embed_out());
  });
  for (int i = 0; i < nd; ++i) {
    p.project(p.normed(i, 0, m->dec_ln0[i]), {m->dec_qkv[i], m->h_dec_qkv[i], 3 * inner, dm}, out_f32(qkv, 3 * inner, 3 * inner));
    {
      EncAttnArgs a{qkv, nullptr, d.dec_rel_bias, m->dec_bucket, p.attn, S, L, H, d.rel_buckets,
                    p.attn_planes(), p.ps_i, nullptr, nullptr, c->status, 1};
      Ln.run(RPR_K_ENC_ATTN, 2.0 * S * H * (double)L * L * DKV, 4.0 * R * 4 * inner, [&] { return launch_enc_attn(a, s); });
    }
    p.attn_out(i, 0, m->dec_o[i], m->h_dec_o[i]);
    p.project(p.normed(i, 1, m->dec_ln1[i]), {m->dec_xq[i], m->h_dec_xq[i], inner, dm}, out_f32(qb, inner, inner));
    {
      const float* xk = P<float>(w.xkv) + (size_t)i * 2 * inner;
      DecCrossAttnArgs a{qb, xk, xk + inner, xld, P<int32_t>(w.mask), p.attn, bz, ndoc * L, H, Lq, p.attn_planes(), p.ps_i,
                         P<int32_t>(w.last), P<int32_t>(w.offs), 0, c->status};
      Ln.run(RPR_K_DEC_CROSS_ATTN, 4.0 * R * H * (double)Lq * DKV, 4.0 * ((double)R * inner * 2 + 2.0 * bz * (double)Lq * inner),
             [&] { return launch_dec_cross_attn(a, s); });
    }
    p.attn_out(i, 1, m->dec_xo[i], m->h_dec_xo[i]);
    p.ff_block(i, 2, m->dec_ln2[i], m->dec_wi[i], m->h_dec_wi[i], m->dec_wo[i], m->h_dec_wo[i]);
  }
  Ln.run(RPR_K_OTHER, 2.0 * R * dm, 4.0 * 2 * R * dm, [&] {
    return launch_gold_scores(p.x, d.dec_final_ln, d.out_embeds, codes, pos_scores, S, L, dm, V, p.xs.eps, p.post, s,
// ... 15 lines not shown
```

ripor_amd/csrc/tail_kernels.hip:

```cpp
#include <algorithm>
#include <cstdlib>

#include "common.h"
#include "kernel_utils.h"

namespace rpr {

__global__ __launch_bounds__(256) void fork_classify_kernel(ForkArgs a) {
  const int q = blockIdx.x * 4 + (threadIdx.x >> 6), lane = threadIdx.x & 63;
  if (q >= a.Qcap || (a.nq_dev && q >= *a.nq_dev)) return;
  const int r0 = q * a.B;
  bool ok = true;
  double smin = INFINITY, smax = -INFINITY;
  for (int b = lane; b < a.B; b += 64) {
    const int lo = a.st.lo[r0 + b], hi = a.st.hi[r0 + b];
    const double s = a.st.score[r0 + b];
    smin = fmin(smin, s); smax = fmax(smax, s);
    if (lo >= hi) { ok = false; continue; }
    if (hi - lo > 1) {
      const uint16_t* first = a.codes + (size_t)lo * a.Lc;
      const uint16_t* last = a.codes + (size_t)(hi - 1) * a.Lc;
      for (int p = a.T; p < a.L; ++p)
        if (first[p] != last[p]) { ok = false; break; }
    }
  }
#pragma unroll
  for (int o = 32; o > 0; o >>= 1) {
    smin = fmin(smin, __shfl_xor(smin, o, 64));
    smax = fmax(smax, __shfl_xor(smax, o, 64));
  }
  const bool all_ok = __all(ok);
  if (lane == 0) a.flag[q] = (all_ok && (smax - smin) < a.spread_max) ? 1 : 0;
}

hipError_t launch_fork_classify(const ForkArgs& a, hipStream_t s) {
  hipLaunchKernelGGL(fork_classify_kernel, dim3((a.Qcap + 3) / 4), dim3(256), 0, s, a);
  return hipGetLastError();
}

__global__ __launch_bounds__(1024) void fork_scan_kernel(const int32_t* __restrict__ flag, int Qcap, const int* __restrict__ nq_dev,
                                                          int B, int Lt, int32_t* __restrict__ flist, int32_t* __restrict__ tail_cnt,
                                                          int32_t* __restrict__ src, int32_t* __restrict__ next_cnt) {
  __shared__ int part[1024];
  __shared__ int carry;
  const int tid = threadIdx.x;
  const int n = nq_dev ? min(*nq_dev, Qcap) : Qcap;
  if (tid == 0) carry = 0;
  __syncthreads();
  for (int q0 = 0; q0 < n; q0 += 1024) {
    const int q = q0 + tid;
    const int v = (q < n && flag[q] != 0) ? 1 : 0;
    part[tid] = v;
    __syncthreads();
    for (int o = 1; o < 1024; o <<= 1) {
      const int add = tid >= o ? part[tid - o] : 0;
      __syncthreads();
      part[tid] += add;
      __syncthreads();
    }
    if (q < n) {
      const int nf_before = carry + part[tid] - v;
      if (v) flist[nf_before] = q; else src[q - nf_before] = q;
    }
    __syncthreads();
    if (tid == 1023) carry += part[1023];
    __syncthreads();
  }
  if (tid == 0) {
    const int nf = carry, nu = n - carry;
    tail_cnt[0] = nf; tail_cnt[1] = nf * B; tail_cnt[2] = nf * B * Lt; tail_cnt[3] = 0;
    next_cnt[0] = nu; next_cnt[1] = nu * B; next_cnt[2] = 0; next_cnt[3] = 0;
  }
}

hipError_t launch_fork_scan(const int32_t* flag, int Qcap, const int* nq_dev, int B, int Lt, int32_t* flist, int32_t* tail_cnt,
                            int32_t* src, int32_t* next_cnt, hipStream_t s) {
  hipLaunchKernelGGL(fork_scan_kernel, dim3(1), dim3(1024), 0, s, flag, Qcap, nq_dev, B, Lt, flist, tail_cnt, src, next_cnt);
  return hipGetLastError();
}

__global__ __launch_bounds__(256) void gather_stage_io_kernel(StageIO src, StageOut dst, const int32_t* __restrict__ list,
                                                               const int* __restrict__ n_dev, int Qcap, int Lq) {
  const int i = blockIdx.x * 4 + (threadIdx.x >> 6), lane = threadIdx.x & 63;
  if (i >= Qcap || i >= *n_dev) return;
  const int q = list[i];
  if (lane == 0) {
    dst.qmap[i] = src.qmap ? src.qmap[q] : q;
    dst.offs[i] = src.offs ? src.offs[q] : q * Lq;
    dst.last[i] = src.last[q];
  }
  for (int j = lane; j < Lq; j += 64) dst.mask[(size_t)i * Lq + j] = src.mask[(size_t)q * Lq + j];
}

hipError_t launch_gather_stage_io(const StageIO& src, const StageOut& dst, const int32_t* list, const int* n_dev, int Qcap, int Lq,
                                  hipStream_t s) {
  hipLaunchKernelGGL(gather_stage_io_kernel, dim3((Qcap + 3) / 4), dim3(256), 0, s, src, dst, list, n_dev, Qcap, Lq);
  return hipGetLastError();
}

__global__ __launch_bounds__(256) void compact_beams_kernel(BeamState from, BeamState to, const int32_t* __restrict__ src,
                                                             const int* __restrict__ n_dev, int B, int T) {
  const int i = blockIdx.x, tid = threadIdx.x;
  if (i >= *n_dev) return;
  const int q = src[i];
  const size_t rf = (size_t)q * B, rt = (size_t)i * B;
  for (int b = tid; b < B; b += 256) {
    to.score[rt + b] = from.score[rf + b];
    to.lo[rt + b] = from.lo[rf + b];
    to.hi[rt + b] = from.hi[rf + b];
  }
  for (int k = tid; k < B * T; k += 256) {
    const int b = k / T, p = k - b * T;
    to.tokens[(rt + b) * to.ld + p] = from.tokens[(rf + b) * from.ld + p];
    to.anc[(rt + b) * to.ld + p] = from.anc[(rf + b) * from.ld + p];
  }
}

hipError_t launch_compact_beams(const BeamState& from, const BeamState& to, const int32_t* src, const int* n_dev, int Qcap, int B, int T,
                                hipStream_t s) {
  hipLaunchKernelGGL(compact_beams_kernel, dim3(Qcap), dim3(256), 0, s, from, to, src, n_dev, B, T);
  return hipGetLastError();
}

__global__ __launch_bounds__(256) void kv_copy_kernel(KvCopyArgs a) {
  const int i = blockIdx.x;
  if (i >= *a.n_dev) return;
  const int lh = blockIdx.y, layer = lh / a.H, h = lh - layer * a.H;
  const size_t of = (size_t)layer * a.layer_from + (size_t)a.src[i] * a.q_from + (size_t)h * a.h_from;
  const size_t ot = (size_t)layer * a.layer_to + (size_t)i * a.q_to + (size_t)h * a.h_to;
  const float4* kf = reinterpret_cast<const float4*>(a.k_from + of);
// ... 30 lines not shown

__global__ __launch_bounds__(256) void tail_embed_kernel(const float* __restrict__ in_embeds, const uint16_t* __restrict__ tokens,
                                                          float* __restrict__ out, int rows, const int* __restrict__ rows_dev,
                                                          int T, int L, int d, int V, XOut xo) {
  const int row = blockIdx.x * 4 + (threadIdx.x >> 6), lane = threadIdx.x & 63;
  if (row >= rows || row >= *rows_dev) return;
  const int Lt = L - T, seq = row / Lt, p = T + (row - seq * Lt);
  const int tok = tokens[(size_t)seq * L + (p - 1)];
  copy_row_x(reinterpret_cast<const float4*>(in_embeds + ((size_t)(p - 1) * V + tok) * d), out, row, d, lane, xo);
}

hipError_t launch_tail_embed(const float* in_embeds, const uint16_t* tokens, float* out, int rows, const int* rows_dev, int T, int L,
                             int d, int V, hipStream_t s, XOut xo) {
  if (rows <= 0 || T < 1) return rows <= 0 ? hipSuccess : hipErrorInvalidValue;
  hipLaunchKernelGGL(tail_embed_kernel, dim3((rows + 3) / 4), dim3(256), 0, s, in_embeds, tokens, out, rows, rows_dev, T, L, d, V, xo);
  return hipGetLastError();
}

__global__ __launch_bounds__(256) void tail_l0_qkv_kernel(const float* __restrict__ table, const uint16_t* __restrict__ tokens,
                                                           float* __restrict__ qkv, int rows, const int* __restrict__ rows_dev,
                                                           int T, int L, int V, int n4) {
  const int row = blockIdx.x * 4 + (threadIdx.x >> 6), lane = threadIdx.x & 63;
  if (row >= rows || row >= *rows_dev) return;
  const int Lt = L - T, seq = row / Lt, p = T + (row - seq * Lt);
  const int tok = tokens[(size_t)seq * L + (p - 1)];
  const float4* src = reinterpret_cast<const float4*>(table) + ((size_t)(p - 1) * V + tok) * n4;
  float4* dst = reinterpret_cast<float4*>(qkv) + (size_t)row * n4;
#pragma unroll 4
  for (int i = lane; i < n4; i += 64) dst[i] = src[i];
}

hipError_t launch_tail_l0_qkv(const float* table, const uint16_t* tokens, float* qkv, int rows, const int* rows_dev, int T, int L,
                              int V, int n3, hipStream_t s) {
  if (rows <= 0 || T < 1 || (n3 & 3)) return rows <= 0 ? hipSuccess : hipErrorInvalidValue;
  hipLaunchKernelGGL(tail_l0_qkv_kernel, dim3((rows + 3) / 4), dim3(256), 0, s, table, tokens, qkv, rows, rows_dev, T, L, V, n3 >> 2);
  return hipGetLastError();
}

template <int D>
__global__ __launch_bounds__(256) void tail_self_attn_kernel(TailSelfAttnArgs a) {
  extern __shared__ __attribute__((aligned(16))) float smem[];
  constexpr int NV = D / 64;
  const int H = a.H, L = a.L, T = a.T, Lt = L - T, inner = H * D, ld = 3 * inner;
  const int seq = blockIdx.x / H, h = blockIdx.x - seq * H;
  if (seq >= *a.nseq_dev) return;
  float* Ks = smem;
  float* Vs = smem + (size_t)L * (D + 1);
  float* Ps = Vs + (size_t)L * D;
  float* Bs = Ps + 4 * 64;
  const int tid = threadIdx.x, lane = tid & 63, wave = tid >> 6;
  const int fi = seq / a.B, b = seq - fi * a.B;
  const int qi = a.flist[fi];
  const uint16_t* ancr = a.anc + ((size_t)qi * a.B + b) * a.anc_ld;
  const size_t cbase = (size_t)qi * a.q_stride + (size_t)h * a.h_stride;
  const float* tbase = a.qkv + (size_t)seq * Lt * ld + h * D;
  for (int i = tid; i < L * (D / 4); i += 256) {
    const int j = i / (D / 4), c = (i - j * (D / 4)) * 4;
    float4 kv, vv;
    if (j < T) {
      const size_t off = cbase + (size_t)j * a.pos_stride + (size_t)ancr[j] * a.slot_stride + c;
      kv = *reinterpret_cast<const float4*>(a.kcache + off);
      vv = *reinterpret_cast<const float4*>(a.vcache + off);
    } else {
      const float* r = tbase + (size_t)(j - T) * ld + c;
      kv = *reinterpret_cast<const float4*>(r + inner);
      vv = *reinterpret_cast<const float4*>(r + 2 * inner);
    }
    float* kd = Ks + j * (D + 1) + c;
    kd[0] = kv.x; kd[1] = kv.y; kd[2] = kv.z; kd[3] = kv.w;
    *reinterpret_cast<float4*>(Vs + j * D + c) = vv;
  }
  if (tid < 64) Bs[tid] = a.rel_bias[a.bucket[tid] * H + h];
  __syncthreads();
  float* P = Ps + wave * 64;
  for (int i = T + wave; i < L; i += 4) {
    float qv[NV];
#pragma unroll
    for (int v = 0; v < NV; ++v) qv[v] = tbase[(size_t)(i - T) * ld + 64 * v + lane];
    const int jc = lane <= i ? lane : i;
    const float* kr = Ks + jc * (D + 1);
    float acc = 0.f;
#pragma unroll
    for (int v = 0; v < NV; ++v)
#pragma unroll
      for (int d = 0; d < 64; ++d) {
        const float qd = __int_as_float(__builtin_amdgcn_readlane(__float_as_int(qv[v]), d));
        acc = fmaf(qd, kr[64 * v + d], acc);
      }
    const float sc = lane <= i ? acc + Bs[i - lane] : -INFINITY;
    const float mx = wave_max(sc);
    const float e = (sc == -INFINITY) ? 0.f : expf(sc - mx);
    const float sum = wave_sum(e);
    P[lane] = e / sum;
    __builtin_amdgcn_wave_barrier();
    float o[NV];
#pragma unroll
    for (int v = 0; v < NV; ++v) o[v] = 0.f;
    for (int j = 0; j <= i; ++j)
#pragma unroll
      for (int v = 0; v < NV; ++v) o[v] = fmaf(P[j], Vs[j * D + 64 * v + lane], o[v]);
#pragma unroll
    for (int v = 0; v < NV; ++v) {
      const size_t oidx = ((size_t)seq * Lt + (i - T)) * inner + h * D + 64 * v + lane;
      if (a.out_h) {
        __half hi, lo;
        split_f16(o[v] * A_PLANE_SCALE, hi, lo, a.sat);
        a.out_h[oidx] = hi;
// ... 63 lines not shown
      o[1] = __builtin_amdgcn_mfma_f32_32x32x2f32(p[kt][kk], vr[32], o[1], 0, 0, 0);
    }
}

__device__ __forceinline__ void store_o_tile(const f32x16 (&o)[2], float* strip, int lane, int i0, int nrows, size_t row_base, int inner,
                                             int hcol, float* out, __half* out_h, size_t o_ps, unsigned int* sat) {
  const int d = lane & 31, half = lane >> 5;
  __builtin_amdgcn_wave_barrier();
#pragma unroll
  for (int r = 0; r < 16; ++r) {
    const int i = (r & 3) + 8 * (r >> 2) + 4 * half;
    strip[i * 64 + d] = o[0][r];
    strip[i * 64 + 32 + d] = o[1][r];
  }
  __builtin_amdgcn_wave_barrier();
  const int c8 = (lane & 7) * 8;
#pragma unroll
  for (int k = 0; k < 4; ++k) {
    const int il = k * 8 + (lane >> 3), i = i0 + il;
    if (i >= nrows) continue;
    const float4 v0 = *reinterpret_cast<const float4*>(strip + il * 64 + c8);
    const float4 v1 = *reinterpret_cast<const float4*>(strip + il * 64 + c8 + 4);
    const size_t oidx = (row_base + i) * inner + hcol + c8;
    if (out_h) {
      __half h[8], l[8];
      const float x[8] = {v0.x, v0.y, v0.z, v0.w, v1.x, v1.y, v1.z, v1.w};
#pragma unroll
      for (int e = 0; e < 8; ++e) split_f16(x[e] * A_PLANE_SCALE, h[e], l[e], sat);
      *reinterpret_cast<uint4*>(out_h + oidx) = *reinterpret_cast<uint4*>(h);
      *reinterpret_cast<uint4*>(out_h + o_ps + oidx) = *reinterpret_cast<uint4*>(l);
    } else {
      *reinterpret_cast<float4*>(out + oidx) = v0;
      *reinterpret_cast<float4*>(out + oidx + 4) = v1;
    }
  }
  __builtin_amdgcn_wave_barrier();
}

template <int NKT, int OCC = 2>
__global__ __launch_bounds__(256, OCC) void tail_self_attn_mfma_kernel(TailSelfAttnArgs a) {
  extern __shared__ __attribute__((aligned(16))) float smem[];
  const int H = a.H, L = a.L, T = a.T, Lt = L - T, inner = H * DKV, ld = 3 * inner;
  const int wave = threadIdx.x >> 6, lane = threadIdx.x & 63, half = lane >> 5;
  const int w = blockIdx.x * 4 + wave;
  const int seq = w / H, h = w - seq * H;
  if (seq >= *a.nseq_dev) return;
  constexpr int WAVE_FLOATS = NKT * 32 * 64 + 64 + (NKT > 1 ? 32 * 64 : 0);
  float* Vs = smem + (size_t)wave * WAVE_FLOATS;
  float* Bs = Vs + NKT * 32 * 64;
  float* Os = NKT > 1 ? Bs + 64 : Vs;
  const int fi = seq / a.B, b = seq - fi * a.B;
  const int qi = a.flist[fi];
  const uint16_t* ancr = a.anc + ((size_t)qi * a.B + b) * a.anc_ld;
  const size_t cbase = (size_t)qi * a.q_stride + (size_t)h * a.h_stride;
  const float* tbase = a.qkv + (size_t)seq * Lt * ld + h * DKV;
  {
    const int g = lane >> 4, li = lane & 15;
#pragma unroll
    for (int it = 0; it < NKT * 8; ++it) {
      const int j = it * 4 + g;
      float4 v = make_float4(0.f, 0.f, 0.f, 0.f);
      if (j < L) {
        const float* vr = j < T ? a.vcache + cbase + (size_t)j * a.pos_stride + (size_t)ancr[j] * a.slot_stride
                                : tbase + (size_t)(j - T) * ld + 2 * inner;
        v = *reinterpret_cast<const float4*>(vr + li * 4);
      }
      *reinterpret_cast<float4*>(Vs + j * 64 + li * 4) = v;
    }
  }
  Bs[lane] = a.rel_bias[a.bucket[lane] * H + h];
  float4 kreg[NKT][8];
#pragma unroll
  for (int kt = 0; kt < NKT; ++kt) {
    const int j = kt * 32 + (lane & 31);
    const float* kr = nullptr;
    if (j < L)
      kr = j < T ? a.kcache + cbase + (size_t)j * a.pos_stride + (size_t)ancr[j] * a.slot_stride : tbase + (size_t)(j - T) * ld + inner;
    load_row_pieces(kr, half, kreg[kt]);
  }
  __builtin_amdgcn_wave_barrier();
  for (int i0 = 0; i0 < Lt; i0 += 32) {
    const int i = i0 + (lane & 31);
    float4 qreg[8];
    load_row_pieces(i < Lt ? tbase + (size_t)i * ld : nullptr, half, qreg);
    f32x16 s[NKT];
#pragma unroll
    for (int kt = 0; kt < NKT; ++kt) {
#pragma unroll
      for (int r = 0; r < 16; ++r) s[kt][r] = 0.f;
      mfma_scores(kreg[kt], qreg, s[kt]);
    }
    const int pq = T + (i < Lt ? i : Lt - 1);
#pragma unroll
    for (int kt = 0; kt < NKT; ++kt)
#pragma unroll
      for (int r = 0; r < 16; ++r) {
        const int j = kt * 32 + kappa(r, half);
        s[kt][r] = j <= pq ? s[kt][r] + Bs[pq - j] : -INFINITY;
      }
    softmax_rows<NKT>(s);
    f32x16 o[2];
#pragma unroll
    for (int r = 0; r < 16; ++r) { o[0][r] = 0.f; o[1][r] = 0.f; }
    mfma_pv<NKT>(s, Vs, lane, o);
    store_o_tile(o, Os, lane, i0, Lt, (size_t)seq * Lt, inner, h * DKV, a.out, a.out_h, a.o_ps, a.sat);
  }
}
// ... 138 lines not shown
        uint4 hi, lo;
        split8(x0, x1, hi, lo, bad);
        *reinterpret_cast<uint4*>(out_h_t + off) = hi;
        *reinterpret_cast<uint4*>(out_h_t + o_ps + off) = lo;
      } else {
        *reinterpret_cast<float4*>(out_t + off) = x0;
        *reinterpret_cast<float4*>(out_t + off + 4) = x1;
      }
    }
  }
  __builtin_amdgcn_wave_barrier();
}

__device__ __forceinline__ void softmax_row16(f32x16& s, int r_end = 16) {
  float mx = fmaxf(fmaxf(s[0], s[1]), fmaxf(s[2], s[3]));
#pragma unroll
  for (int q4 = 1; q4 < 4; ++q4)
    if (q4 * 4 < r_end) mx = fmaxf(mx, fmaxf(fmaxf(s[q4 * 4], s[q4 * 4 + 1]), fmaxf(s[q4 * 4 + 2], s[q4 * 4 + 3])));
  mx = fmaxf(mx, __shfl_xor(mx, 32, 64));
  float sum = 0.f;
#pragma unroll
  for (int q4 = 0; q4 < 4; ++q4) {
    if (q4 * 4 < r_end) {
#pragma unroll
      for (int r = q4 * 4; r < q4 * 4 + 4; ++r) {
        const float e = exp_nonpos(s[r] - mx);
        s[r] = e;
        sum += e;
      }
    } else {
#pragma unroll
      for (int r = q4 * 4; r < q4 * 4 + 4; ++r) s[r] = 0.f;
    }
  }
  sum += __shfl_xor(sum, 32, 64);
  const float inv = sum > 0.f ? 1.0f / sum : 0.f;
#pragma unroll
  for (int r = 0; r < 16; ++r) s[r] *= inv;
}

template <int OCC>
__global__ __launch_bounds__(256, OCC) void tail_self_attn_mfma_v2_kernel(TailSelfAttnArgs a, int HB, unsigned hb_magic, unsigned b_magic) {
  extern __shared__ __attribute__((aligned(16))) float smem[];
  const int H = a.H, L = a.L, T = a.T, Lt = L - T, inner = H * DKV, ld = 3 * inner;
  const int wave = __builtin_amdgcn_readfirstlane(threadIdx.x >> 6);
  const int lane = threadIdx.x & 63, half = lane >> 5, ln = lane & 31;
  const int seq = udiv_magic(blockIdx.x, HB, hb_magic);
  const int h = ((int)blockIdx.x - seq * HB) * 4 + wave;
  if (h >= H || seq >= *a.nseq_dev) return;
  float* Os = smem + wave * (32 * 64);
  const int fi = udiv_magic((unsigned)seq, a.B, b_magic), b = seq - fi * a.B;
  const int qi = a.flist[fi];
  const uint16_t* ancr = a.anc + ((size_t)qi * a.B + b) * a.anc_ld;
  const float* kc = a.kcache + (size_t)qi * a.q_stride + (size_t)h * a.h_stride;
  const float* vc = a.vcache + (size_t)qi * a.q_stride + (size_t)h * a.h_stride;
  const float* tbase = a.qkv + (size_t)seq * Lt * ld + h * DKV;
  const int kk_end = L > 24 ? 16 : L > 16 ? 12 : L > 8 ? 8 : 4;
  float4 kreg[8], qreg[8];
  {
    const int j = min(ln, L - 1);
    const int slot = ancr[j];
    const float* kr = j < T ? kc + (size_t)j * a.pos_stride + (size_t)slot * a.slot_stride : tbase + (j - T) * ld + inner;
    load_row_pieces(kr, half, kreg);
    load_row_pieces(tbase + min(ln, Lt - 1) * ld, half, qreg);
  }
  Os[lane < 32 ? 31 - lane : lane] = lane < 32 ? a.rel_bias[a.bucket[ln] * H + h] : 0.f;
  float v0[16], v1[16];
#pragma unroll
  for (int kk = 0; kk < 4; ++kk) {
    const int j = min(kk + 4 * half, L - 1);
    const int slot = ancr[j];
    const float* vr = j < T ? vc + (size_t)j * a.pos_stride + (size_t)slot * a.slot_stride : tbase + (j - T) * ld + 2 * inner;
    v0[kk] = vr[ln]; v1[kk] = vr[ln + 32];
  }
  const int voff = 4 * half * ld + ln;
#pragma unroll
  for (int q4 = 1; q4 < 4; ++q4) {
    if (q4 * 4 < kk_end) {
#pragma unroll
      for (int kk = q4 * 4; kk < q4 * 4 + 4; ++kk) {
        const int j0 = kappa(kk, 0);
        if (j0 + 4 < L) {
          const float* sb = tbase + 2 * inner + (j0 - T) * ld;
          v0[kk] = sb[voff]; v1[kk] = sb[voff + 32];
        } else {
          const float* vr = tbase + 2 * inner + (min(j0 + 4 * half, L - 1) - T) * ld;
          v0[kk] = vr[ln]; v1[kk] = vr[ln + 32];
        }
      }
    } else {
#pragma unroll
      for (int kk = q4 * 4; kk < q4 * 4 + 4; ++kk) { v0[kk] = 0.f; v1[kk] = 0.f; }
    }
  }
  const f32x16 z = {0.f, 0.f, 0.f, 0.f, 0.f, 0.f, 0.f, 0.f, 0.f, 0.f, 0.f, 0.f, 0.f, 0.f, 0.f, 0.f};
  f32x16 sc = mfma_scores_c(kreg, qreg, z);
  const int pq = T + min(ln, Lt - 1);
  {
    const float* brow = Os + (31 - pq + 4 * half);
    const int jl = pq - 4 * half;
#pragma unroll
    for (int r = 0; r < 16; ++r) {
      const int j0 = kappa(r, 0);
      sc[r] = j0 <= jl ? sc[r] + brow[j0] : -INFINITY;
    }
  }
  softmax_row16(sc, kk_end);
  f32x16 o[2];
// ... 596 lines not shown
  };
  float ss = 0.f;
  for (int k = lane; k < n4; k += 64) {
    const float4 v = load4(k);
    ss += v.x * v.x + v.y * v.y + v.z * v.z + v.w * v.w;
  }
  ss = wave_sum(ss);
  const float rs = rsqrtf(ss / (float)d + eps);
  float acc = 0.f;
  for (int k = lane; k < n4; k += 64) {
    const float4 v = load4(k), g = wr[k], e = er[k];
    float4 hd = make_float4(g.x * (v.x * rs), g.y * (v.y * rs), g.z * (v.z * rs), g.w * (v.w * rs));
    if (post != 1.0f) { hd.x *= post; hd.y *= post; hd.z *= post; hd.w *= post; }
    acc += (hd.x * e.x + hd.y * e.y) + (hd.z * e.z + hd.w * e.w);
  }
  acc = wave_sum(acc);
  if (lane == 0) gold[row] = acc;
}

hipError_t launch_tail_gold(const float* x, const float* ln, const float* out_embeds, const uint16_t* tokens, float* gold, int rows,
                            const int* rows_dev, int T, int L, int d, int V, float eps, float post, hipStream_t s, const __half* x_h,
                            size_t x_ps) {
  if (rows <= 0) return hipSuccess;
  hipLaunchKernelGGL(tail_gold_kernel, dim3((rows + 3) / 4), dim3(256), 0, s, x, ln, out_embeds, tokens, gold, rows, rows_dev, T, L, d, V,
                     eps, post, x_h, x_ps);
  return hipGetLastError();
}

__global__ __launch_bounds__(256) void tail_logprob_kernel(const float* __restrict__ logits, const uint16_t* __restrict__ tokens,
                                                            float* __restrict__ gold, int rows, const int* __restrict__ rows_dev, int T,
                                                            int L, int V) {
  const int row = blockIdx.x * 4 + (threadIdx.x >> 6), lane = threadIdx.x & 63;
  if (row >= rows || row >= *rows_dev) return;
  const int Lt = L - T, seq = row / Lt, p = T + (row - seq * Lt);
  const int tok = tokens[(size_t)seq * L + p];
  const float* lr = logits + (size_t)row * V;
  float mx = -INFINITY;
  for (int c = lane; c < V; c += 64) mx = fmaxf(mx, lr[c]);
  mx = wave_max(mx);
  float sm = 0.f;
  for (int c = lane; c < V; c += 64) sm += expf(lr[c] - mx);
#pragma unroll
  for (int o = 32; o > 0; o >>= 1) sm += __shfl_xor(sm, o, 64);
  if (lane == 0) gold[row] = (lr[tok] - mx) - logf(sm);
}

hipError_t launch_tail_logprob(const float* logits, const uint16_t* tokens, float* gold, int rows, const int* rows_dev, int T, int L,
                               int V, hipStream_t s) {
  if (rows <= 0) return hipSuccess;
  hipLaunchKernelGGL(tail_logprob_kernel, dim3((rows + 3) / 4), dim3(256), 0, s, logits, tokens, gold, rows, rows_dev, T, L, V);
  return hipGetLastError();
}

__global__ __launch_bounds__(1024) void tail_rank_kernel(TailRankArgs a) {
  extern __shared__ __attribute__((aligned(16))) unsigned char smem_raw[];
  const int i = blockIdx.x, tid = threadIdx.x, nt = blockDim.x;
  if (i >= *a.nf_dev) return;
  const int B = a.B, T = a.T, L = a.L, Lt = L - T;
  double* S = reinterpret_cast<double*>(smem_raw);
  int* pos = reinterpret_cast<int*>(S + B);
  int* npos = pos + B;
  __shared__ int tie;
  const int q = a.flist[i];
  const size_t r0 = (size_t)q * B;
  if (tid == 0) tie = a.replay;
  for (int b = tid; b < B; b += nt) {
    double s = a.st.score[r0 + b];
    const float* g = a.gold + ((size_t)i * B + b) * Lt;
    for (int t = 0; t < Lt; ++t) s = ((double)g[t] + 0.0) + s;
    S[b] = s / (double)(L + 1);
    pos[b] = b;
  }
  __syncthreads();
  for (int b = tid; b < B; b += nt) {
    const double s = S[b];
    int gt = 0, eq = 0;
    for (int k = 0; k < B; ++k) { const double o = S[k]; gt += o > s; eq += o == s; }
    npos[b] = gt;
    if (eq > 1) tie = 1;
  }
  __syncthreads();
  if (tie) {
    for (int b = tid; b < B; b += nt) S[b] = a.st.score[r0 + b];
    __syncthreads();
    for (int t = 0; t < Lt; ++t) {
      for (int b = tid; b < B; b += nt) S[b] = ((double)a.gold[((size_t)i * B + b) * Lt + t] + 0.0) + S[b];
      __syncthreads();
      for (int b = tid; b < B; b += nt) {
        const double s = S[b];
        const int pb = pos[b];
        int rk = 0;
        for (int k = 0; k < B; ++k) rk += (S[k] > s) || (S[k] == s && pos[k] < pb);
        npos[b] = rk;
      }
      __syncthreads();
      for (int b = tid; b < B; b += nt) pos[b] = npos[b];
      __syncthreads();
    }
    for (int b = tid; b < B; b += nt) S[b] = S[b] / (double)(L + 1);
    __syncthreads();
    for (int b = tid; b < B; b += nt) {
      const double s = S[b];
      const int pb = pos[b];
      int rk = 0;
      for (int k = 0; k < B; ++k) rk += (S[k] > s) || (S[k] == s && pos[k] > pb);
      npos[b] = rk;
    }
    __syncthreads();
  }
  const size_t o0 = (size_t)a.qmap[i] * B;
  for (int b = tid; b < B; b += nt) {
    const int rk = npos[b];
    a.out_scores[o0 + rk] = (float)S[b];
    a.out_lo[o0 + rk] = a.st.lo[r0 + b];
    a.out_hi[o0 + rk] = a.st.hi[r0 + b];
  }
  for (int k = tid; k < B * L; k += nt) {
    const int b = k / L, p = k - b * L;
    a.out_tokens[(o0 + npos[b]) * L + p] = (int32_t)a.tokens[((size_t)i * B + b) * L + p];
  }
}

hipError_t launch_tail_rank(const TailRankArgs& a_in, hipStream_t s) {
  const char* rp = getenv("RPR_TAIL_RANK_REPLAY");
  const int replay = rp ? atoi(rp) : 0;
  TailRankArgs a = a_in;
  if (replay) a.replay = 1;
  const size_t smem = (size_t)a.B * (sizeof(double) + 2 * sizeof(int)) + 16;
  hipLaunchKernelGGL(tail_rank_kernel, dim3(a.Qcap), dim3(a.B > 256 ? 1024 : 256), smem, s, a);
  return hipGetLastError();
}

__global__ void flag_nonzero_kernel(const int* __restrict__ cnt, unsigned int* __restrict__ flag) {
  if (threadIdx.x == 0 && *cnt != 0) *flag = 1u;
}

hipError_t launch_flag_nonzero(const int* cnt, unsigned int* flag, hipStream_t s) {
  hipLaunchKernelGGL(flag_nonzero_kernel, dim3(1), dim3(64), 0, s, cnt, flag);
  return hipGetLastError();
}

__global__ __launch_bounds__(256) void max_row_norm_kernel(const float* __restrict__ E, const float* __restrict__ w, int rows, int d,
                                                            float* __restrict__ out) {
  const int row = blockIdx.x * 4 + (threadIdx.x >> 6), lane = threadIdx.x & 63;
  if (row >= rows) return;
  float ss = 0.f;
  for (int k = lane; k < d; k += 64) {
    const float v = E[(size_t)row * d + k] * (w ? w[k] : 1.0f);
    ss = fmaf(v, v, ss);
  }
  ss = wave_sum(ss);
  if (lane == 0) {
    float n = sqrtf(ss);
    if (!(n >= 0.f)) n = INFINITY;
    atomicMax(reinterpret_cast<unsigned int*>(out), __float_as_uint(n));
  }
}

hipError_t launch_max_row_norm(const float* E, const float* w, int rows, int d, float* out, hipStream_t s) {
  if (rows <= 0) return hipSuccess;
  hipLaunchKernelGGL(max_row_norm_kernel, dim3((rows + 3) / 4), dim3(256), 0, s, E, w, rows, d, out);
  return hipGetLastError();
}

hipError_t init_tail_kernel_attributes() {
  hipError_t e = hipFuncSetAttribute(reinterpret_cast<const void*>(tail_self_attn_kernel<128>), hipFuncAttributeMaxDynamicSharedMemorySize,
                                     (int)tail_self_attn_smem(MAX_DEC_LEN, 128));
  if (e != hipSuccess) return e;
  e = hipFuncSetAttribute(reinterpret_cast<const void*>(tail_self_attn_mfma_kernel<2>), hipFuncAttributeMaxDynamicSharedMemorySize, 112 * 1024);
  if (e != hipSuccess) return e;
  e = hipFuncSetAttribute(reinterpret_cast<const void*>(tail_cross_attn_mfma_kernel<2>), hipFuncAttributeMaxDynamicSharedMemorySize, 80 * 1024);
  if (e != hipSuccess) return e;
  return hipFuncSetAttribute(reinterpret_cast<const void*>(tail_rank_kernel), hipFuncAttributeMaxDynamicSharedMemorySize, 64 * 1024);
}

}
```

ripor_amd/csrc/trie.cpp:

```cpp
#include <algorithm>
#include <atomic>
#include <cstdio>
#include <cstdlib>
#include <exception>
#include <string>
#include <thread>
#include <cstring>
#include <numeric>
#include <vector>

#include "trie.h"

namespace rpr {

struct SortKey {
  uint64_t key;
  int32_t idx;
};

int sort_codes(const uint16_t* codes, int64_t N, int L, std::vector<uint16_t>& sorted, std::vector<int64_t>& perm) {
  std::vector<SortKey> keys((size_t)N);
  const int pk = L < 4 ? L : 4;
  std::vector<int64_t> start(65537, 0);
  for (int64_t i = 0; i < N; ++i) start[(size_t)codes[i * L] + 1]++;
// ... 7 lines not shown
    }
  }
  auto cmp = [codes, L, pk](const SortKey& a, const SortKey& b) {
    if (a.key != b.key) return a.key < b.key;
    const uint16_t* ra = codes + (int64_t)a.idx * L;
    const uint16_t* rb = codes + (int64_t)b.idx * L;
    for (int l = pk; l < L; ++l)
      if (ra[l] != rb[l]) return ra[l] < rb[l];
    return a.idx < b.idx;
  };
  unsigned nthreads = std::thread::hardware_concurrency();
  if (const char* e = std::getenv("RPR_TRIE_THREADS")) nthreads = (unsigned)std::atoi(e);
  if (nthreads < 1) nthreads = 1;
  if (nthreads > 32) nthreads = 32;
  if (N < (1 << 16)) nthreads = 1;
  std::atomic<int> next{0};
  auto worker = [&] {
    for (;;) {
      const int v = next.fetch_add(1);
      if (v >= 65536) break;
      if (start[(size_t)v + 1] - start[(size_t)v] > 1)
        std::sort(keys.begin() + start[(size_t)v], keys.begin() + start[(size_t)v + 1], cmp);
    }
  };
  if (nthreads == 1) {
    worker();
  } else {
    std::vector<std::thread> pool;
    for (unsigned t = 0; t < nthreads; ++t) pool.emplace_back(worker);
    for (auto& th : pool) th.join();
  }
  sorted.resize((size_t)N * L);
  perm.resize((size_t)N);
  auto gather = [&](int64_t lo, int64_t hi) {
    for (int64_t i = lo; i < hi; ++i) {
      perm[(size_t)i] = keys[(size_t)i].idx;
      std::memcpy(&sorted[(size_t)i * L], codes + (int64_t)keys[(size_t)i].idx * L, sizeof(uint16_t) * L);
    }
  };
  if (nthreads == 1) {
    gather(0, N);
  } else {
    std::vector<std::thread> pool;
    const int64_t chunk = (N + nthreads - 1) / nthreads;
    for (unsigned t = 0; t < nthreads; ++t) {
      const int64_t lo = (int64_t)t * chunk, hi = lo + chunk < N ? lo + chunk : N;
      if (lo < hi) pool.emplace_back(gather, lo, hi);
    }
    for (auto& th : pool) th.join();
  }
  return 0;
}

void trie_single_frac(const uint16_t* sorted, int64_t N, int Lc, int L, std::vector<double>& frac) {
  std::vector<int64_t> nodes((size_t)L + 2, 0), single((size_t)L + 2, 0);
  int a = -1;
  for (int64_t i = 1; i <= N; ++i) {
    int c = -1;
    if (i < N) {
      const uint16_t* p = sorted + (size_t)(i - 1) * Lc;
      const uint16_t* q = p + Lc;
      c = 0;
      while (c < L && p[c] == q[c]) ++c;
      if (c == L) continue;
    }
    nodes[(size_t)(a + 1)] += 1;
    single[(size_t)((a > c ? a : c) + 1)] += 1;
    a = c;
  }
  frac.assign((size_t)L + 1, 0.0);
  int64_t n = 0, s = 0;
  for (int t = 0; t <= L; ++t) {
    n += nodes[(size_t)t];
    s += single[(size_t)t];
    frac[(size_t)t] = n ? (double)s / (double)n : 0.0;
  }
}

void build_child_levels(const uint16_t* sorted, int64_t N, int Lc, int V, int narrow, int max_levels, int64_t max_entries,
                        ChildLevels& out) {
  out = ChildLevels{};
  if (N <= 0 || Lc < 1 || V < 1) return;
  out.lvl0.assign((size_t)V + 1, (int32_t)N);
  {
    int next = 0;
    for (int64_t r = 0; r < N; ++r) {
      const int v = sorted[(size_t)r * Lc];
      while (next <= v) out.lvl0[(size_t)next++] = (int32_t)r;
    }
  }
  if (Lc < 2 || V > 1024) return;
  out.lvl1.assign((size_t)V * V + 1, (int32_t)N);
  {
    int64_t next = 0;
    for (int64_t r = 0; r < N; ++r) {
      const int64_t v = (int64_t)sorted[(size_t)r * Lc] * V + sorted[(size_t)r * Lc + 1];
      while (next <= v) out.lvl1[(size_t)next++] = (int32_t)r;
    }
  }
  if (Lc < 3 || max_levels < 1) return;
  std::vector<uint8_t> lcp((size_t)N, 0);
  for (int64_t r = 1; r < N; ++r) {
    const uint16_t* p = sorted + (size_t)(r - 1) * Lc;
    const uint16_t* q = p + Lc;
    int c = 0;
    while (c < Lc && c < 255 && p[c] == q[c]) ++c;
    lcp[(size_t)r] = (uint8_t)c;
  }
  out.idx2.assign((size_t)V * V, -1);
  int64_t total = 0;
  for (int t = 2; t < Lc && t < 255 && (int)out.deep.size() < max_levels; ++t) {
    ChildLevels::Level lv;
    int64_t a = 0;
    for (int64_t r = 1; r <= N; ++r) {
      if (r < N && lcp[(size_t)r] >= t) continue;
      if (r - a > narrow) {
        if (t == 2) out.idx2[(size_t)sorted[(size_t)a * Lc] * V + sorted[(size_t)a * Lc + 1]] = (int32_t)lv.start.size();
        for (int64_t k = a; k < r; ++k)
          if (k == a || lcp[(size_t)k] < t + 1) { lv.start.push_back((int32_t)k); lv.tok.push_back(sorted[(size_t)k * Lc + t]); }
      }
      a = r;
    }
    if (lv.start.empty()) break;
    total += (int64_t)lv.start.size();
    if (total > max_entries) { if (t == 2) std::fill(out.idx2.begin(), out.idx2.end(), -1); break; }
    out.deep.push_back(std::move(lv));
  }
}
// ... 153 lines not shown
```

ripor_amd/csrc/trie.h:

```cpp
#pragma once
#include <stdint.h>
#include <string>
#include <vector>

namespace rpr {
int sort_codes(const uint16_t* codes, int64_t N, int L, std::vector<uint16_t>& sorted, std::vector<int64_t>& perm);
int save_trie_file(const char* path, const std::vector<uint16_t>& sorted, const std::vector<int64_t>& perm,
                   int64_t N, int L, int V, const std::string& keys, int64_t src_size, int64_t src_mtime_ns);
int load_trie_file(const char* path, std::vector<uint16_t>& sorted, std::vector<int64_t>& perm, int64_t& N, int& L,
                   int& V, std::string& keys, std::string& err);
void trie_single_frac(const uint16_t* sorted, int64_t N, int Lc, int L, std::vector<double>& frac);
struct ChildLevels {
  std::vector<int32_t> lvl0, lvl1, idx2;
  struct Level { std::vector<int32_t> start; std::vector<uint16_t> tok; };
  std::vector<Level> deep;
};
void build_child_levels(const uint16_t* sorted, int64_t N, int Lc, int V, int narrow, int max_levels, int64_t max_entries,
                        ChildLevels& out);
int trie_file_info(const char* path, int64_t hdr_out[6]);
int read_docid_to_smtid(const char* path, std::vector<uint16_t>& codes, std::string& keys, int64_t& N, int& L,
                        std::string& err);
}
```

ripor_amd/engine.py:

```python
from __future__ import annotations

import ctypes as C
import threading
from dataclasses import dataclass
from typing import Dict, List, Optional, Sequence

import numpy as np
import torch

from . import _lib
from ._lib import RiporHipError, check

_contexts: Dict[int, "Context"] = {}


def _stream_ptr(device: torch.device) -> C.c_void_p:
    return C.c_void_p(torch.cuda.current_stream(device).cuda_stream)


class Context:

    def __init__(self, device_index: int):
        if not torch.cuda.is_available():
            raise RiporHipError("no HIP device visible to torch: the search path has no CPU fallback")
        self.lib = _lib.load()
        self.device = torch.device("cuda", device_index)
        h = C.c_void_p()
        check(self.lib.rpr_init(device_index, C.byref(h)), "rpr_init")
        self.handle = h

    @staticmethod
    def get(device=None) -> "Context":
        if device is None:
            idx = torch.cuda.current_device() if torch.cuda.is_available() else 0
        else:
            dev = torch.device(device) if not isinstance(device, int) else torch.device("cuda", device)
            if dev.type != "cuda":
                raise RiporHipError(f"device {dev} is not a HIP device: the search path has no CPU fallback")
            idx = dev.index if dev.index is not None else torch.cuda.current_device()
        if idx not in _contexts:
            _contexts[idx] = Context(idx)
        return _contexts[idx]

    def set_precision(self, name: str):
        check(self.lib.rpr_set_precision(self.handle, {"f32": _lib.PREC_F32, "f16x2": _lib.PREC_F16X2, "bf16": _lib.PREC_BF16}[name]),
              "rpr_set_precision")

    def get_precision(self) -> str:
        return {_lib.PREC_F32: "f32", _lib.PREC_F16X2: "f16x2", _lib.PREC_BF16: "bf16"}[int(self.lib.rpr_get_precision(self.handle))]

    def has_bf16(self) -> bool:
        return True

    def workspace_bytes(self) -> int:
        return int(self.lib.rpr_workspace_bytes(self.handle))

    def set_lane_split(self, min_rows: int):
        check(self.lib.rpr_set_lane_split(self.handle, int(min_rows)), "rpr_set_lane_split")

    def lane_split(self) -> int:
        return int(self.lib.rpr_lane_split(self.handle))

    def set_l0_table(self, mode: int):
        check(self.lib.rpr_set_l0_table(self.handle, int(mode)), "rpr_set_l0_table")

    def l0_table_bytes(self, model: "DeviceModel") -> int:
        return int(self.lib.rpr_l0_table_bytes(self.handle, model.handle))

    def set_forced_tail(self, mode):
        check(self.lib.rpr_set_forced_tail(self.handle, int(mode)), "rpr_set_forced_tail")

    def forced_tail(self) -> int:
        return int(self.lib.rpr_forced_tail(self.handle))

    def set_fork_depths(self, depths: Optional[Sequence[int]]):
        if depths is None:
            check(self.lib.rpr_set_fork_depths(self.handle, -1, None), "rpr_set_fork_depths")
        else:
            arr = (C.c_int32 * max(1, len(depths)))(*[int(d) for d in depths])
            check(self.lib.rpr_set_fork_depths(self.handle, len(depths), arr), "rpr_set_fork_depths")

    def fork_depths(self, model: "DeviceModel", trie: "DeviceTrie", Q: int, B: int, L: int, log_softmax: bool = False) -> List[int]:
        out = (C.c_int32 * 2)()
        n = int(self.lib.rpr_fork_depths(self.handle, model.handle, trie.handle, Q, B, L,
                                         _lib.FLAG_LOG_SOFTMAX if log_softmax else 0, out))
        if n < 0:
            check(n, "rpr_fork_depths")
        return [int(out[i]) for i in range(n)]

    def last_fork_stats(self) -> List[dict]:
        d, f, l = (C.c_int32 * 2)(), (C.c_int32 * 2)(), (C.c_int32 * 2)()
        n = int(self.lib.rpr_last_fork_stats(self.handle, d, f, l))
        if n < 0:
            check(n, "rpr_last_fork_stats")
        return [dict(depth=int(d[i]), forced=int(f[i]), left=int(l[i])) for i in range(n)]

    def status_async(self, clear: bool = True):
        words = torch.zeros(4, dtype=torch.int32).pin_memory()
        check(self.lib.rpr_status_words_async(self.handle, _stream_ptr(self.device), words.data_ptr(), 1 if clear else 0),
              "rpr_status_words_async")
        ev = torch.cuda.Event()
        ev.record(torch.cuda.current_stream(self.device))
        return StatusTicket(words, ev)

    def clear_status_async(self):
        check(self.lib.rpr_status_words_async(self.handle, _stream_ptr(self.device), None, 1), "rpr_status_words_async")

    def status(self, clear: bool = True) -> int:
        out = C.c_uint32(0)
        check(self.lib.rpr_get_status(self.handle, _stream_ptr(self.device), C.byref(out), 1 if clear else 0), "rpr_get_status")
        flags = int(out.value) | getattr(self, "_kept_status", 0)
        if clear:
            self._kept_status = 0
        return flags

    def keep_status(self, flags: int):
        self._kept_status = getattr(self, "_kept_status", 0) | int(flags)

    def profile_enable(self, on: bool):
        check(self.lib.rpr_profile_enable(self.handle, 1 if on else 0), "rpr_profile_enable")
# ... 50 lines not shown
    def flags(self) -> int:
        self._event.synchronize()
        w = self._words
        return ((_lib.STATUS_SATURATED if int(w[0]) else 0) | (_lib.STATUS_EMPTY_QUERY if int(w[1]) else 0) |
                (_lib.STATUS_TAIL_LEFTOVER if int(w[2]) else 0))


def rel_bucket(rel: int, bidirectional: bool, num_buckets: int = 32, max_distance: int = 128) -> int:
    return int(_lib.load().rpr_rel_bucket(rel, 1 if bidirectional else 0, num_buckets, max_distance))


def read_docid_to_smtid(path: str):
    lib = _lib.load()
    h = C.c_void_p()
    check(lib.rpr_d2s_open(path.encode(), C.byref(h)), "rpr_d2s_open")
    try:
        N, L, kb = C.c_int64(), C.c_int32(), C.c_int64()
        check(lib.rpr_d2s_dims(h, C.byref(N), C.byref(L), C.byref(kb)), "rpr_d2s_dims")
        codes = np.empty((N.value, L.value), dtype=np.uint16)
        keys = C.create_string_buffer(max(1, kb.value))
        check(lib.rpr_d2s_copy(h, codes.ctypes.data_as(C.c_void_p), keys), "rpr_d2s_copy")
        docids = keys.raw[:kb.value].decode("utf-8").split("\n")
    finally:
        lib.rpr_d2s_close(h)
    assert len(docids) == codes.shape[0], (len(docids), codes.shape)
    return docids, codes


def build_trie_file(codes: np.ndarray, V: int, path: str, docids: Optional[Sequence[str]] = None,
                    source_path: Optional[str] = None) -> None:
    import os
    lib = _lib.load()
    codes = np.ascontiguousarray(codes, dtype=np.uint16)
    N, L = codes.shape
    keys = "\n".join(docids).encode("utf-8") if docids is not None else b""
    if docids is not None and len(docids) != N:
        raise ValueError("one docid per code row expected")
    size = mtime = 0
    if source_path is not None:
        st = os.stat(source_path)
        size, mtime = st.st_size, st.st_mtime_ns
    check(lib.rpr_trie_build_file(codes.ctypes.data_as(C.c_void_p), N, L, int(V), keys, len(keys), size, mtime,
                                  path.encode()), "rpr_trie_build_file")


def trie_single_frac(codes: np.ndarray, L: Optional[int] = None) -> np.ndarray:
    lib = _lib.load()
    codes = np.ascontiguousarray(codes, dtype=np.uint16)
    N, Lc = codes.shape
    L = Lc if L is None else int(L)
    out = (C.c_double * (L + 1))()
    check(lib.rpr_trie_single_frac(codes.ctypes.data_as(C.c_void_p), N, Lc, L, out), "rpr_trie_single_frac")
    return np.asarray(list(out), dtype=np.float64)


def trie_file_info(path: str) -> dict:
    lib = _lib.load()
    n, l, v, kb, ss, sm = C.c_int64(), C.c_int32(), C.c_int32(), C.c_int64(), C.c_int64(), C.c_int64()
    check(lib.rpr_trie_file_info(path.encode(), C.byref(n), C.byref(l), C.byref(v), C.byref(kb), C.byref(ss), C.byref(sm)),
          "rpr_trie_file_info")
    return dict(N=n.value, L=l.value, V=v.value, key_bytes=kb.value, src_size=ss.value, src_mtime_ns=sm.value)


def _ptr_array(tensors: Sequence[torch.Tensor]):
    arr = (C.c_void_p * len(tensors))(*[t.data_ptr() for t in tensors])
    return arr


class DeviceModel:

    def __init__(self, ctx: Context, state_dict: Dict[str, torch.Tensor], cfg):
        self.ctx, self.cfg = ctx, cfg
        dev = ctx.device

        def g(name):
            t = state_dict[name]
            if isinstance(t, np.ndarray):
                t = torch.from_numpy(t)
            return t.to(device=dev, dtype=torch.float32).contiguous()

        L = len(cfg.decoder_vocab_sizes)
        V = int(cfg.decoder_vocab_sizes[0])
        if len(set(cfg.decoder_vocab_sizes)) != 1:
            raise ValueError("not valid decoder_vocab_size")
        shared_embeds = bool(cfg.shared_output_input_embeds)
        keep: List[torch.Tensor] = []
        self._names: List[tuple] = []

        def K(t):
            keep.append(t)
            return t

        def N(name, t, sl=None):
            self._names.append((name, t, sl))
            return t

        def attn_qkv(prefix):
            t = K(torch.cat([g(prefix + ".q.weight"), g(prefix + ".k.weight"), g(prefix + ".v.weight")], 0).contiguous())
            n = t.shape[0] // 3
            for j, w in enumerate("qkv"):
                N(f"{prefix}.{w}.weight", t, slice(j * n, (j + 1) * n))
            return t

        ne, nd = cfg.num_layers, cfg.num_decoder_layers
        enc = dict(ln0=[], qkv=[], o=[], ln1=[], wi=[], wo=[])
        for i in range(ne):
# ... 849 lines not shown
```

Baseline: 4947.

## Let forced-tail fork absorb queries with a few extra live sequences

Extends the forked tail path so that queries with up to a small budget of extra trie branches beyond the forced single-path beams can still enter the cheap tail stage. A pool of spare query slots holds the extra sequences, and a dedicated rank routine merges them with the original beams. Fork depth planning now uses a Poisson model of extra branches per node, so the fork can happen earlier and fewer queries fall back to the full decode. In exchange it adds workspace, extra kernels (fork_extras), a more complex ranking kernel, and new graph-key state.

```diff
diff --git a/include/ripor_hip.h b/include/ripor_hip.h
--- a/include/ripor_hip.h
+++ b/include/ripor_hip.h
@@ -138,6 +138,11 @@
 int rpr_set_l0_table(rpr_ctx* ctx, int32_t mode);
 int64_t rpr_l0_table_bytes(const rpr_ctx* ctx, const rpr_model* model);
 int rpr_trie_single_frac(const uint16_t* codes, int64_t N, int32_t Lc, int32_t L, double* out_frac);
+int rpr_trie_extra_mean(const uint16_t* codes, int64_t N, int32_t Lc, int32_t L, double* out_mean);
+int rpr_plan_forks(const double* single_frac, const double* extra_mean, int32_t Q, int32_t B, int32_t L, int32_t forced_tail,
+                   int32_t tail_extras, int32_t* out_depths, int32_t* out_drop_last);
+int rpr_set_tail_extras(rpr_ctx* ctx, int32_t mode);
+int32_t rpr_tail_extras(const rpr_ctx* ctx);
 int rpr_last_fork_stats(rpr_ctx* ctx, int32_t* out_depths, int32_t* out_forced, int32_t* out_left);
 
 int rpr_lngknp_forward(rpr_ctx* ctx, rpr_model* model, const int32_t* input_ids, const int32_t* attention_mask,
diff --git a/ripor_amd/_lib.py b/ripor_amd/_lib.py
--- a/ripor_amd/_lib.py
+++ b/ripor_amd/_lib.py
@@ -126,6 +126,11 @@
     "rpr_fork_depths": (C.c_int, [C.c_void_p, C.c_void_p, C.c_void_p, C.c_int32, C.c_int32, C.c_int32, C.c_uint32,
                                   C.POINTER(C.c_int32)]),
     "rpr_trie_single_frac": (C.c_int, [C.c_void_p, C.c_int64, C.c_int32, C.c_int32, C.POINTER(C.c_double)]),
+    "rpr_trie_extra_mean": (C.c_int, [C.c_void_p, C.c_int64, C.c_int32, C.c_int32, C.POINTER(C.c_double)]),
+    "rpr_plan_forks": (C.c_int, [C.POINTER(C.c_double), C.POINTER(C.c_double), C.c_int32, C.c_int32, C.c_int32, C.c_int32, C.c_int32,
+                                 C.POINTER(C.c_int32), C.POINTER(C.c_int32)]),
+    "rpr_set_tail_extras": (C.c_int, [C.c_void_p, C.c_int32]),
+    "rpr_tail_extras": (C.c_int32, [C.c_void_p]),
     "rpr_last_fork_stats": (C.c_int, [C.c_void_p, C.POINTER(C.c_int32), C.POINTER(C.c_int32), C.POINTER(C.c_int32)]),
     "rpr_op_linear": (C.c_int, [C.c_void_p, C.c_void_p, C.c_void_p, C.c_void_p, C.c_void_p, C.c_int32, C.c_int32,
                                 C.c_int32, C.c_int32, C.c_void_p]),
diff --git a/ripor_amd/csrc/api.hip b/ripor_amd/csrc/api.hip
--- a/ripor_amd/csrc/api.hip
+++ b/ripor_amd/csrc/api.hip
@@ -72,6 +72,51 @@
     }
   }
   return RPR_OK;
+}
+
+}
+
+namespace rpr {
+
+namespace {
+double poisson_pmf(double lam, int i) { return lam > 0 ? std::exp(-lam + i * std::log(lam) - std::lgamma((double)i + 1.0)) : (i == 0 ? 1.0 : 0.0); }
+double poisson_tail(double lam, int k) {
+  if (lam <= 0) return 0.0;
+  if (lam > 4.0 * k + 50.0) return 1.0;
+  double s = 0;
+  const int n = k + 60 + (int)(lam + 12.0 * std::sqrt(lam));
+  for (int i = k + 1; i <= n; ++i) s += poisson_pmf(lam, i);
+  return s < 1.0 ? s : 1.0;
+}
+double poisson_excess(double lam, int k) {
+  if (lam <= 0) return 0.0;
+  if (lam > 4.0 * k + 50.0) return lam;
+  double s = 0;
+  const int n = k + 60 + (int)(lam + 12.0 * std::sqrt(lam));
+  for (int i = k + 1; i <= n; ++i) s += (double)(i - k) * poisson_pmf(lam, i);
+  return s;
+}
+}
+
+std::vector<int> plan_forks(const double* f, const double* mu, int Q, int B, int L, int forced_tail, int E, int pool, bool* drop_last) {
+  std::vector<int> forks;
+  *drop_last = false;
+  auto p_forced = [&](int t) { return std::pow(f[t], (double)B); };
+  auto left = [&](int t) {
+    if (E <= 0) return (double)Q * (1.0 - p_forced(t));
+    const double lam = (double)B * mu[t];
+    return (double)Q * poisson_tail(lam, E) + poisson_excess((double)Q * (1.0 - std::exp(-lam)), pool);
+  };
+  int t0 = 0;
+  for (int t = 1; t <= L - 2 && !t0; ++t) if (p_forced(t) >= 0.5) t0 = t;
+  const int min_tail = (int64_t)Q * B <= 4096 ? 2 : 8;
+  if (!t0 || L - t0 < min_tail) return forks;
+  forks.push_back(t0);
+  if (forced_tail == 2 && left(t0) <= 0.05) { *drop_last = true; return forks; }
+  for (int t = t0 + 1; t <= L - 2 && t <= t0 + 12; ++t)
+    if (left(t) <= 0.05) { forks.push_back(t); break; }
+  *drop_last = forced_tail == 2 && forks.size() == 2;
+  return forks;
 }
 
 }
@@ -418,6 +463,34 @@
   return RPR_OK;
 }
 
+int rpr_trie_extra_mean(const uint16_t* codes, int64_t N, int32_t Lc, int32_t L, double* out_mean) {
+  RPR_REQUIRE(codes && out_mean, "NULL argument");
+  RPR_REQUIRE(N > 0 && N < ((int64_t)1 << 31) - 1 && Lc >= 1 && Lc <= 4096 && L >= 1 && L <= Lc, "N, Lc or L out of range");
+  try {
+    std::vector<uint16_t> sorted;
+    std::vector<int64_t> perm;
+    sort_codes(codes, N, Lc, sorted, perm);
+    std::vector<double> f, mu;
+    trie_single_frac(sorted.data(), N, Lc, L, f, &mu);
+    for (int t = 0; t <= L; ++t) out_mean[t] = mu[(size_t)t];
+  } catch (const std::exception& ex) {
+    set_error(std::string("rpr_trie_extra_mean: ") + ex.what());
+    return RPR_ERR_OOM;
+  }
+  return RPR_OK;
+}
+
+int rpr_plan_forks(const double* single_frac, const double* extra_mean, int32_t Q, int32_t B, int32_t L, int32_t forced_tail,
+                   int32_t tail_extras, int32_t* out_depths, int32_t* out_drop_last) {
+  RPR_REQUIRE(single_frac && extra_mean && out_depths && out_drop_last, "NULL argument");
+  RPR_REQUIRE(Q >= 1 && B >= 1 && L >= 1 && L < 256 && forced_tail >= 0 && forced_tail <= 2 && tail_extras >= -1, "argument out of range");
+  bool drop_last = false;
+  const std::vector<int> f = plan_forks(single_frac, extra_mean, Q, B, L, forced_tail, tail_extras_budget(tail_extras, Q, B, false), tail_extras_pool(Q), &drop_last);
+  for (size_t i = 0; i < f.size(); ++i) out_depths[i] = f[i];
+  *out_drop_last = drop_last ? 1 : 0;
+  return (int)f.size();
+}
+
 int rpr_trie_file_info(const char* path, int64_t* N, int32_t* L, int32_t* V, int64_t* key_bytes, int64_t* src_size,
                        int64_t* src_mtime_ns) {
   RPR_REQUIRE(path, "NULL argument");
@@ -585,22 +658,13 @@
   }
   auto it = tr->single_frac.find(L);
   if (it == tr->single_frac.end()) {
-    std::vector<double> f;
-    trie_single_frac(tr->host_sorted.data(), tr->N, tr->L, L, f);
+    std::vector<double> f, mu;
+    trie_single_frac(tr->host_sorted.data(), tr->N, tr->L, L, f, &mu);
     it = tr->single_frac.emplace(L, std::move(f)).first;
-  }
-  const std::vector<double>& f = it->second;
-  auto p_forced = [&](int t) { return std::pow(f[(size_t)t], (double)B); };
-  int t0 = 0;
-  for (int t = 1; t <= L - 2 && !t0; ++t) if (p_forced(t) >= 0.5) t0 = t;
-  const int min_tail = (int64_t)Q * B <= 4096 ? 2 : 8;
-  if (!t0 || L - t0 < min_tail) return forks;
-  forks.push_back(t0);
-  if (c->forced_tail == 2 && (double)Q * (1.0 - p_forced(t0)) <= 0.05) { *drop_last = true; return forks; }
-  for (int t = t0 + 1; t <= L - 2 && t <= t0 + 12; ++t)
-    if ((double)Q * (1.0 - p_forced(t)) <= 0.05) { forks.push_back(t); break; }
-  *drop_last = c->forced_tail == 2 && forks.size() == 2;
-  return forks;
+    tr->extra_mean[L] = std::move(mu);
+  }
+  const int E = tail_extras_budget(c->tail_extras, Q, B, c->cur_margins != 0);
+  return plan_forks(it->second.data(), tr->extra_mean[L].data(), Q, B, L, c->forced_tail, E, E > 0 ? tail_extras_pool(Q) : 0, drop_last);
 }
 
 int pack_forks(const std::vector<int>& forks, bool drop_last) {
@@ -639,8 +703,9 @@
     const unsigned dbg = (env_int("RPR_TAIL_RANK_REPLAY", 0) ? 1u : 0u) | ((unsigned)(env_int("RPR_SELECT_RADIX", -1) + 1) << 1);
     const unsigned l0 = m->l0_ready(c) ? (unsigned)c->l0_mode : 0u;
     const unsigned mg = c->cur_margins ? 1u : 0u;
+    const int ex = tail_extras_budget(c->tail_extras, Q, B, c->cur_margins != 0);
     GraphKey key{m, tr, Q, Lq, B, L, flags | ((unsigned)c->precision << 16) | (dbg << 20) | (l0 << 24) | (mg << 28), lane,
-                 pack_forks(forks, drop_last)};
+                 pack_forks(forks, drop_last) | (ex << 24)};
     auto it = c->graphs.find(key);
     if (it == c->graphs.end()) {
       hipGraph_t graph = nullptr;
@@ -761,6 +826,13 @@
 }
 int64_t rpr_l0_table_bytes(const rpr_ctx* c, const rpr_model* m) { return c && m && m->l0_ready(c) ? (int64_t)m->l0_bytes() : 0; }
 
+int rpr_set_tail_extras(rpr_ctx* c, int32_t mode) {
+  RPR_REQUIRE(c && mode >= -1 && mode <= 31, "mode must be -1 (automatic), 0 (off) or a budget of 1..31 extra sequences per query");
+  c->tail_extras = mode;
+  return RPR_OK;
+}
+int32_t rpr_tail_extras(const rpr_ctx* c) { return c ? c->tail_extras : -1; }
+
 int rpr_set_forced_tail(rpr_ctx* c, int32_t mode) {
   RPR_REQUIRE(c && mode >= 0 && mode <= 2, "mode must be 0 (off), 1 (exact) or 2 (optimistic)");
   c->forced_tail = mode;
@@ -798,7 +870,7 @@
     for (int i = 0; i < 3; ++i) {
       if (!(c->last_ws_mask & (1 << i)) || !wss[i]->tail[k].cnt.p || !wss[i]->stage[k].cnt.p) continue;
       int32_t a = 0, b = 0;
-      RPR_HIP(hipMemcpy(&a, wss[i]->tail[k].cnt.p, 4, hipMemcpyDeviceToHost));
+      RPR_HIP(hipMemcpy(&a, static_cast<const char*>(wss[i]->tail[k].cnt.p) + 12, 4, hipMemcpyDeviceToHost));
       RPR_HIP(hipMemcpy(&b, wss[i]->stage[k].cnt.p, 4, hipMemcpyDeviceToHost));
       out_forced[k] += a; out_left[k] += b;
     }
diff --git a/ripor_amd/csrc/common.h b/ripor_amd/csrc/common.h
--- a/ripor_amd/csrc/common.h
+++ b/ripor_amd/csrc/common.h
@@ -417,10 +417,20 @@
   int B, T, L;
   double spread_max;
   int32_t* flag;
+  int E = 0;
 };
 hipError_t launch_fork_classify(const ForkArgs& a, hipStream_t s);
-hipError_t launch_fork_scan(const int32_t* flag, int Qcap, const int* nq_dev, int B, int Lt, int32_t* flist, int32_t* tail_cnt,
-                            int32_t* src, int32_t* next_cnt, hipStream_t s);
+struct ForkScanArgs {
+  const int32_t* flag; int Qcap; const int* nq_dev; int B, Lt;
+  int32_t* flist;
+  int32_t* tail_cnt;
+  int32_t* src; int32_t* next_cnt;
+  int32_t* kvq;
+  int32_t* spare; int pool;
+};
+hipError_t launch_fork_scan(const ForkScanArgs& a, hipStream_t s);
+struct ForkExtrasArgs { BeamState st; const uint16_t* codes; int Lc; int Qcap, B, T, L, pool; int32_t* spare; };
+hipError_t launch_fork_extras(const ForkExtrasArgs& a, hipStream_t s);
 struct StageIO {
   const int32_t* qmap;
   const int32_t* offs;
@@ -458,6 +468,7 @@
   float* out; __half* out_h; size_t o_ps; unsigned int* sat;
   int nseq_cap, B, H, T, L;
   int dkv = 0;
+  const int32_t* kvq = nullptr;
 };
 hipError_t launch_tail_self_attn(const TailSelfAttnArgs& a, hipStream_t s);
 hipError_t launch_tail_cross_attn(const DecCrossAttnArgs& a, hipStream_t s);
@@ -475,6 +486,8 @@
   int Qcap, B, T, L;
   int32_t* out_tokens; float* out_scores; int64_t* out_lo; int64_t* out_hi;
   int replay = 0;
+  const int32_t* spare = nullptr; int pool = 0;
+  const uint16_t* codes = nullptr; int Lc = 0;
 };
 hipError_t launch_tail_rank(const TailRankArgs& a, hipStream_t s);
 hipError_t launch_flag_nonzero(const int* cnt, unsigned int* flag, hipStream_t s);
diff --git a/ripor_amd/csrc/internal.h b/ripor_amd/csrc/internal.h
--- a/ripor_amd/csrc/internal.h
+++ b/ripor_amd/csrc/internal.h
@@ -85,6 +85,7 @@
   std::vector<uint16_t> host_sorted;
   std::string keys;
   std::map<int, std::vector<double>> single_frac;
+  std::map<int, std::vector<double>> extra_mean;
   ~rpr_trie() { if (codes) (void)hipFree(codes); free_levels(); }
 };
 
@@ -114,6 +115,8 @@
 struct TailBufs {
   DevBuf flag, flist;
   DevBuf cnt;
+  DevBuf kvq;
+  DevBuf spare;
   DevBuf qmap, offs, last, mask;
   DevBuf tokens;
   DevBuf gold;
@@ -169,6 +172,7 @@
   int forced_tail = 1;
   int fork_override[MAX_FORKS] = {0, 0};
   int n_fork_override = -1;
+  int tail_extras = -1;
   std::vector<int> last_forks;
   int last_ws_mask = 0;
   size_t ws_bytes = 0;
@@ -188,6 +192,16 @@
 
 namespace rpr {
 
+constexpr int TAIL_EXTRAS_AUTO = 4;
+inline int tail_extras_budget(int mode, int Q, int B, bool margins) {
+  if (mode == 0 || B >= 32 || margins) return 0;
+  if (mode > 0) return mode < B ? mode : B;
+  return (int64_t)Q * B > 4096 ? (TAIL_EXTRAS_AUTO < B ? TAIL_EXTRAS_AUTO : B) : 0;
+}
+inline int tail_extras_pool(int Q) { return Q / 32 < 4 ? 4 : (Q / 32 > 64 ? 64 : Q / 32); }
+std::vector<int> plan_forks(const double* single_frac, const double* extra_mean, int Q, int B, int L, int forced_tail, int E, int pool,
+                            bool* drop_last);
+
 int refresh_weight_planes(rpr_ctx* c, rpr_model* m, hipStream_t s);
 inline int ensure_weight_planes(rpr_ctx* c, rpr_model* m, hipStream_t s) {
   if (!m->planes_dirty) return 0;
diff --git a/ripor_amd/csrc/passes.hip b/ripor_amd/csrc/passes.hip
--- a/ripor_amd/csrc/passes.hip
+++ b/ripor_amd/csrc/passes.hip
@@ -60,6 +60,8 @@
   const size_t T = (size_t)Q * Lq, R = (size_t)Q * B, inner = m->inner(), dm = d.d_model, dff = d.d_ff;
   const size_t nd = d.num_decoder_layers, ne = d.num_layers, f = sizeof(float);
   Workspace& w = c->ws;
+  const size_t pool = !forks.empty() && tail_extras_budget(c->tail_extras, Q, B, c->cur_margins != 0) > 0 ? (size_t)tail_extras_pool(Q) : 0;
+  const size_t Qt = (size_t)Q + pool, Rv = Qt * B;
   int e = 0;
   auto E = [&](DevBuf& b, size_t bytes) { if (!e) e = ensure(c, b, bytes); };
   E(w.ids, T * 4); E(w.mask, T * 4); E(w.last, (size_t)Q * 4); E(w.offs, ((size_t)Q + 1) * 4); E(w.row_src, T * 4);
@@ -72,8 +74,8 @@
   E(w.lb, R * (size_t)m->Vp() * 4 * 2);
   if (select_radix_wanted(B, m->Vp())) E(w.sel_rs, select_radix_ws_bytes(Q, B, m->Vp()));
   for (int i = 0; i < 2; ++i) {
-    E(w.score[i], R * 8); E(w.lo[i], R * 4); E(w.hi[i], R * 4);
-    E(w.tokens[i], R * (size_t)L * 2); E(w.anc[i], R * (size_t)L * 2);
+    E(w.score[i], Rv * 8); E(w.lo[i], Rv * 4); E(w.hi[i], Rv * 4);
+    E(w.tokens[i], Rv * (size_t)L * 2); E(w.anc[i], Rv * (size_t)L * 2);
   }
   E(w.o_tokens, R * (size_t)L * 4); E(w.o_scores, R * 4); E(w.o_lo, R * 8); E(w.o_hi, R * 8);
   if (c->cur_margins) { E(w.mg_valid, R * (size_t)m->Vp() / 8); E(w.o_margin, (size_t)Q * 8); }
@@ -91,17 +93,18 @@
       E(sb.qmap, (size_t)Q * 4); E(sb.offs, (size_t)Q * 4); E(sb.last, (size_t)Q * 4); E(sb.mask, T * 4);
       E(sb.kcache, nd * depth * R * inner * f); E(sb.vcache, nd * depth * R * inner * f);
       for (int i = 0; i < 2; ++i) {
-        E(sb.score[i], R * 8); E(sb.lo[i], R * 4); E(sb.hi[i], R * 4);
-        E(sb.tokens[i], R * (size_t)L * 2); E(sb.anc[i], R * (size_t)L * 2);
+        E(sb.score[i], Rv * 8); E(sb.lo[i], Rv * 4); E(sb.hi[i], Rv * 4);
+        E(sb.tokens[i], Rv * (size_t)L * 2); E(sb.anc[i], Rv * (size_t)L * 2);
       }
     }
     TailBufs& tb = w.tail[k];
-    E(tb.flag, (size_t)Q * 4); E(tb.flist, (size_t)Q * 4); E(tb.cnt, 16);
-    E(tb.qmap, (size_t)Q * 4); E(tb.offs, (size_t)Q * 4); E(tb.last, (size_t)Q * 4); E(tb.mask, T * 4);
-    E(tb.tokens, R * (size_t)L * 2); E(tb.gold, R * Lt * f);
+    E(tb.flag, (size_t)Q * 4); E(tb.flist, Qt * 4); E(tb.cnt, 16);
+    E(tb.kvq, Qt * 4); E(tb.spare, ((size_t)Q + 1 + pool + pool * B) * 4);
+    E(tb.qmap, Qt * 4); E(tb.offs, Qt * 4); E(tb.last, Qt * 4); E(tb.mask, Qt * Lq * 4);
+    E(tb.tokens, Rv * (size_t)L * 2); E(tb.gold, Rv * Lt * f);
   }
   if (!forks.empty()) {
-    const size_t Rt = R * (size_t)(L - forks[0]);
+    const size_t Rt = Rv * (size_t)(L - forks[0]);
     E(w.t_qkv, Rt * 3 * inner * f); E(w.t_q, Rt * inner * f);
     if (c->precision == RPR_PREC_F16X2 && !m->f32_only) {
       E(w.t_x_h, Rt * dm * hb); E(w.t_attn_h, Rt * inner * hb); E(w.t_ff_h, Rt * dff * hb); E(w.t_ssq, (3 * nd + 1) * Rt * 8);
@@ -389,18 +392,22 @@
   const BeamState st = sv.st[T & 1];
   const double per_step = (sd.flags & RPR_FLAG_LOG_SOFTMAX) ? 2.0 * (double)m->logit_bound + log((double)d.V) : 2.0 * (double)m->logit_bound;
   const double spread_max = 1e8 - (double)(L - T) * per_step;
-  ForkArgs fa{st, tr->codes, tr->L, Q, sv.nq_dev, B, T, L, spread_max, P<int32_t>(tb.flag)};
+  const int extras = tail_extras_budget(c->tail_extras, sd.Q, B, c->cur_margins != 0), pool = extras > 0 ? tail_extras_pool(sd.Q) : 0;
+  ForkArgs fa{st, tr->codes, tr->L, Q, sv.nq_dev, B, T, L, spread_max, P<int32_t>(tb.flag), extras};
   Ln.run(RPR_K_FORK, 0, 0, [&] { return launch_fork_classify(fa, s); });
-  Ln.run(RPR_K_FORK, 0, 0, [&] {
-    return launch_fork_scan(P<int32_t>(tb.flag), Q, sv.nq_dev, B, L - T, P<int32_t>(tb.flist), P<int32_t>(tb.cnt), P<int32_t>(nb.src),
-                            P<int32_t>(nb.cnt), s);
-  });
+  const ForkScanArgs fs{P<int32_t>(tb.flag), Q, sv.nq_dev, B, L - T, P<int32_t>(tb.flist), P<int32_t>(tb.cnt), P<int32_t>(nb.src),
+                        P<int32_t>(nb.cnt), P<int32_t>(tb.kvq), P<int32_t>(tb.spare), pool};
+  Ln.run(RPR_K_FORK, 0, 0, [&] { return launch_fork_scan(fs, s); });
+  if (pool > 0) {
+    const ForkExtrasArgs fe{st, tr->codes, tr->L, Q, B, T, L, pool, P<int32_t>(tb.spare)};
+    Ln.run(RPR_K_FORK, 0, 0, [&] { return launch_fork_extras(fe, s); });
+  }
   Ln.run(RPR_K_FORK, 0, 0, [&] {
     return launch_gather_stage_io(sv.io, StageOut{P<int32_t>(tb.qmap), P<int32_t>(tb.offs), P<int32_t>(tb.last), P<int32_t>(tb.mask)},
-                                  P<int32_t>(tb.flist), P<int>(tb.cnt), Q, Lq, s);
+                                  P<int32_t>(tb.kvq), P<int>(tb.cnt), Q + pool, Lq, s);
   });
   Ln.run(RPR_K_FORK, 0, 0, [&] {
-    return launch_tail_tokens(st, tr->codes, tr->L, P<int32_t>(tb.flist), P<int>(tb.cnt), Q, B, T, L, P<uint16_t>(tb.tokens), s);
+    return launch_tail_tokens(st, tr->codes, tr->L, P<int32_t>(tb.flist), P<int>(tb.cnt), Q + pool, B, T, L, P<uint16_t>(tb.tokens), s);
   });
   StageView nv{};
   if (!compact) {
@@ -422,10 +429,13 @@
   return nv;
 }
 
-void enqueue_tail(Launcher& Ln, rpr_ctx* c, const rpr_model* m, const SearchDims& sd, const StageView& sv, int T, TailBufs& tb) {
+void enqueue_tail(Launcher& Ln, rpr_ctx* c, const rpr_model* m, const rpr_trie* tr, const SearchDims& sd, const StageView& sv, int T,
+                  TailBufs& tb) {
   const auto& d = m->d;
   Workspace& w = c->ws;
-  const int Q = sv.Qcap, B = sd.B, L = sd.L, Lq = sd.Lq, Lt = L - T, S = Q * B, R = S * Lt;
+  const int pool = tail_extras_budget(c->tail_extras, sd.Q, sd.B, c->cur_margins != 0) > 0 ? tail_extras_pool(sd.Q) : 0;
+  const int Q = sv.Qcap + pool;
+  const int B = sd.B, L = sd.L, Lq = sd.Lq, Lt = L - T, S = Q * B, R = S * Lt;
   const int inner = m->inner(), dm = d.d_model, H = d.num_heads, nd = d.num_decoder_layers, V = d.V, xld = sd.xld;
   hipStream_t s = Ln.s;
   const int* nf_dev = P<int>(tb.cnt);
@@ -453,6 +463,7 @@
                          sv.st[T & 1].anc, L, P<int32_t>(tb.flist), nseq_dev, d.dec_rel_bias, m->dec_bucket, p.attn,
                          p.attn_planes(), p.ps_i, c->status, S, B, H, T, L};
       a.dkv = d.d_kv;
+      a.kvq = P<int32_t>(tb.kvq);
       Ln.run(RPR_K_TAIL_SELF_ATTN, 2.0 * Ra * H * (double)(L + T + 1) * sv.dkv, 4.0 * ((double)Ra * 4 * inner + 2.0 * (Ra / Lt) * (double)T * inner),
              [&] { return launch_tail_self_attn(a, s); });
     }
@@ -492,8 +503,9 @@
                               p.post, s, p.x_planes(), p.xs.ps);
     });
   }
-  TailRankArgs ra{sv.st[T & 1], P<int32_t>(tb.flist), P<int32_t>(tb.qmap), nf_dev, P<uint16_t>(tb.tokens), P<float>(tb.gold), Q, B, T, L,
+  TailRankArgs ra{sv.st[T & 1], P<int32_t>(tb.flist), P<int32_t>(tb.qmap), nf_dev + 3, P<uint16_t>(tb.tokens), P<float>(tb.gold), sv.Qcap, B, T, L,
                   P<int32_t>(w.o_tokens), P<float>(w.o_scores), P<int64_t>(w.o_lo), P<int64_t>(w.o_hi)};
+  ra.spare = P<int32_t>(tb.spare); ra.pool = pool; ra.codes = tr->codes; ra.Lc = tr->L;
   Ln.run(RPR_K_FORK, 0, 0, [&] { return launch_tail_rank(ra, s); });
   Ln.account_live(nullptr, 0);
 }
@@ -548,7 +560,7 @@
       const int next_depth = k + 1 < forks.size() ? forks[k + 1] : L;
       const bool last_dropped = drop_last && k + 1 == forks.size();
       const StageView nv = enqueue_fork(Ln, c, m, tr, sd, sv, t1, next_depth, w.tail[k], w.stage[k], !last_dropped);
-      enqueue_tail(Ln, c, m, sd, sv, t1, w.tail[k]);
+      enqueue_tail(Ln, c, m, tr, sd, sv, t1, w.tail[k]);
       if (last_dropped) return;
       sv = nv;
     }
diff --git a/ripor_amd/csrc/tail_kernels.hip b/ripor_amd/csrc/tail_kernels.hip
--- a/ripor_amd/csrc/tail_kernels.hip
+++ b/ripor_amd/csrc/tail_kernels.hip
@@ -5,12 +5,27 @@
 #include "kernel_utils.h"
 
 namespace rpr {
+
+__device__ inline int seq_run_end(const uint16_t* __restrict__ codes, int Lc, int r, int hi, int T, int L) {
+  const uint16_t* a = codes + (size_t)r * Lc;
+  int lo = r + 1;
+  while (lo < hi) {
+    const int mid = lo + ((hi - lo) >> 1);
+    const uint16_t* m = codes + (size_t)mid * Lc;
+    bool same = true;
+    for (int p = T; p < L; ++p)
+      if (a[p] != m[p]) { same = false; break; }
+    if (same) lo = mid + 1; else hi = mid;
+  }
+  return lo;
+}
 
 __global__ __launch_bounds__(256) void fork_classify_kernel(ForkArgs a) {
   const int q = blockIdx.x * 4 + (threadIdx.x >> 6), lane = threadIdx.x & 63;
   if (q >= a.Qcap || (a.nq_dev && q >= *a.nq_dev)) return;
   const int r0 = q * a.B;
   bool ok = true;
+  int extras = 0;
   double smin = INFINITY, smax = -INFINITY;
   for (int b = lane; b < a.B; b += 64) {
     const int lo = a.st.lo[r0 + b], hi = a.st.hi[r0 + b];
@@ -20,8 +35,15 @@
     if (hi - lo > 1) {
       const uint16_t* first = a.codes + (size_t)lo * a.Lc;
       const uint16_t* last = a.codes + (size_t)(hi - 1) * a.Lc;
+      bool one = true;
       for (int p = a.T; p < a.L; ++p)
-        if (first[p] != last[p]) { ok = false; break; }
+        if (first[p] != last[p]) { one = false; break; }
+      if (!one) {
+        if (a.E <= 0) { ok = false; continue; }
+        int n = 0;
+        for (int r = lo; r < hi && n <= a.E + 1; ++n) r = seq_run_end(a.codes, a.Lc, r, hi, a.T, a.L);
+        extras += n - 1;
+      }
     }
   }
 #pragma unroll
@@ -29,8 +51,12 @@
     smin = fmin(smin, __shfl_xor(smin, o, 64));
     smax = fmax(smax, __shfl_xor(smax, o, 64));
   }
-  const bool all_ok = __all(ok);
-  if (lane == 0) a.flag[q] = (all_ok && (smax - smin) < a.spread_max) ? 1 : 0;
+  if (a.E > 0) {
+#pragma unroll
+    for (int o = 32; o > 0; o >>= 1) extras += __shfl_xor(extras, o, 64);
+  }
+  const bool all_ok = __all(ok) && extras <= a.E;
+  if (lane == 0) a.flag[q] = (all_ok && (smax - smin) < a.spread_max) ? 1 + extras : 0;
 }
 
 hipError_t launch_fork_classify(const ForkArgs& a, hipStream_t s) {
@@ -38,44 +64,110 @@
   return hipGetLastError();
 }
 
-__global__ __launch_bounds__(1024) void fork_scan_kernel(const int32_t* __restrict__ flag, int Qcap, const int* __restrict__ nq_dev,
-                                                          int B, int Lt, int32_t* __restrict__ flist, int32_t* __restrict__ tail_cnt,
-                                                          int32_t* __restrict__ src, int32_t* __restrict__ next_cnt) {
+__device__ inline void block_scan_1024(int* part, int tid) {
+  __syncthreads();
+  for (int o = 1; o < 1024; o <<= 1) {
+    const int add = tid >= o ? part[tid - o] : 0;
+    __syncthreads();
+    part[tid] += add;
+    __syncthreads();
+  }
+}
+
+__global__ __launch_bounds__(1024) void fork_scan_kernel(ForkScanArgs a) {
   __shared__ int part[1024];
-  __shared__ int carry;
-  const int tid = threadIdx.x;
-  const int n = nq_dev ? min(*nq_dev, Qcap) : Qcap;
-  if (tid == 0) carry = 0;
+  __shared__ int carry, carry_x;
+  const int tid = threadIdx.x, Qcap = a.Qcap;
+  const int n = a.nq_dev ? min(*a.nq_dev, Qcap) : Qcap;
+  int32_t* sp_of = a.spare;
+  int32_t* owner = a.spare + Qcap + 1;
+  if (tid == 0) { carry = 0; carry_x = 0; }
   __syncthreads();
   for (int q0 = 0; q0 < n; q0 += 1024) {
     const int q = q0 + tid;
-    const int v = (q < n && flag[q] != 0) ? 1 : 0;
+    const int fl = q < n ? a.flag[q] : 0;
+    int k = -1;
+    if (a.pool > 0) {
+      const int x = fl > 1 ? 1 : 0;
+      part[tid] = x;
+      block_scan_1024(part, tid);
+      const int kx = carry_x + part[tid] - x;
+      if (x && kx < a.pool) k = kx;
+      __syncthreads();
+      if (tid == 1023) carry_x += part[1023];
+      __syncthreads();
+    }
+    const int v = (fl == 1 || k >= 0) ? 1 : 0;
     part[tid] = v;
-    __syncthreads();
-    for (int o = 1; o < 1024; o <<= 1) {
-      const int add = tid >= o ? part[tid - o] : 0;
-      __syncthreads();
-      part[tid] += add;
-      __syncthreads();
-    }
+    block_scan_1024(part, tid);
     if (q < n) {
       const int nf_before = carry + part[tid] - v;
-      if (v) flist[nf_before] = q; else src[q - nf_before] = q;
+      if (v) {
+        a.flist[nf_before] = q; a.kvq[nf_before] = q; sp_of[nf_before] = k;
+        if (k >= 0) owner[k] = q;
+      } else {
+        a.src[q - nf_before] = q;
+      }
     }
     __syncthreads();
     if (tid == 1023) carry += part[1023];
     __syncthreads();
   }
+  const int nf = carry, used = min(carry_x, a.pool);
+  for (int k = tid; k < used; k += 1024) { a.flist[nf + k] = Qcap + k; a.kvq[nf + k] = owner[k]; }
   if (tid == 0) {
-    const int nf = carry, nu = n - carry;
-    tail_cnt[0] = nf; tail_cnt[1] = nf * B; tail_cnt[2] = nf * B * Lt; tail_cnt[3] = 0;
-    next_cnt[0] = nu; next_cnt[1] = nu * B; next_cnt[2] = 0; next_cnt[3] = 0;
-  }
-}
-
-hipError_t launch_fork_scan(const int32_t* flag, int Qcap, const int* nq_dev, int B, int Lt, int32_t* flist, int32_t* tail_cnt,
-                            int32_t* src, int32_t* next_cnt, hipStream_t s) {
-  hipLaunchKernelGGL(fork_scan_kernel, dim3(1), dim3(1024), 0, s, flag, Qcap, nq_dev, B, Lt, flist, tail_cnt, src, next_cnt);
+    const int ne = nf + used, nu = n - nf;
+    a.tail_cnt[0] = ne; a.tail_cnt[1] = ne * a.B; a.tail_cnt[2] = ne * a.B * a.Lt; a.tail_cnt[3] = nf;
+    a.next_cnt[0] = nu; a.next_cnt[1] = nu * a.B; a.next_cnt[2] = 0; a.next_cnt[3] = 0;
+    a.spare[Qcap] = used;
+  }
+}
+
+hipError_t launch_fork_scan(const ForkScanArgs& a, hipStream_t s) {
+  hipLaunchKernelGGL(fork_scan_kernel, dim3(1), dim3(1024), 0, s, a);
+  return hipGetLastError();
+}
+
+__global__ __launch_bounds__(64) void fork_extras_kernel(ForkExtrasArgs a) {
+  const int k = blockIdx.x, tid = threadIdx.x, B = a.B, T = a.T;
+  if (k >= a.spare[a.Qcap]) return;
+  __shared__ int pb[32], plo[32], phi[32];
+  const int q = a.spare[a.Qcap + 1 + k];
+  const size_t r0 = (size_t)q * B, v0 = (size_t)(a.Qcap + k) * B;
+  int32_t* parent = a.spare + a.Qcap + 1 + a.pool + (size_t)k * B;
+  if (tid == 0) {
+    int s = 0;
+    for (int b = 0; b < B && s < B; ++b) {
+      const int lo = a.st.lo[r0 + b], hi = a.st.hi[r0 + b];
+      if (lo >= hi) continue;
+      for (int r = seq_run_end(a.codes, a.Lc, lo, hi, T, a.L); r < hi && s < B; ++s) {
+        const int e = seq_run_end(a.codes, a.Lc, r, hi, T, a.L);
+        pb[s] = b; plo[s] = r; phi[s] = e;
+        r = e;
+      }
+    }
+    for (; s < B; ++s) { pb[s] = -1; plo[s] = a.st.lo[r0]; phi[s] = a.st.hi[r0]; }
+  }
+  __syncthreads();
+  for (int s = tid; s < B; s += 64) {
+    const size_t src = r0 + (pb[s] > 0 ? pb[s] : 0);
+    a.st.score[v0 + s] = a.st.score[src];
+    a.st.lo[v0 + s] = plo[s];
+    a.st.hi[v0 + s] = phi[s];
+    parent[s] = pb[s];
+  }
+  for (int i = tid; i < B * T; i += 64) {
+    const int s = i / T, p = i - s * T;
+    const size_t src = r0 + (pb[s] > 0 ? pb[s] : 0);
+    a.st.tokens[(v0 + s) * a.st.ld + p] = a.st.tokens[src * a.st.ld + p];
+    a.st.anc[(v0 + s) * a.st.ld + p] = a.st.anc[src * a.st.ld + p];
+  }
+}
+
+hipError_t launch_fork_extras(const ForkExtrasArgs& a, hipStream_t s) {
+  if (a.pool <= 0) return hipSuccess;
+  if (a.B > 32) return hipErrorInvalidValue;
+  hipLaunchKernelGGL(fork_extras_kernel, dim3(a.pool), dim3(64), 0, s, a);
   return hipGetLastError();
 }
 
@@ -212,7 +304,7 @@
   const int fi = seq / a.B, b = seq - fi * a.B;
   const int qi = a.flist[fi];
   const uint16_t* ancr = a.anc + ((size_t)qi * a.B + b) * a.anc_ld;
-  const size_t cbase = (size_t)qi * a.q_stride + (size_t)h * a.h_stride;
+  const size_t cbase = (size_t)(a.kvq ? a.kvq[fi] : qi) * a.q_stride + (size_t)h * a.h_stride;
   const float* tbase = a.qkv + (size_t)seq * Lt * ld + h * D;
   for (int i = tid; i < L * (D / 4); i += 256) {
     const int j = i / (D / 4), c = (i - j * (D / 4)) * 4;
@@ -382,7 +474,7 @@
   const int fi = seq / a.B, b = seq - fi * a.B;
   const int qi = a.flist[fi];
   const uint16_t* ancr = a.anc + ((size_t)qi * a.B + b) * a.anc_ld;
-  const size_t cbase = (size_t)qi * a.q_stride + (size_t)h * a.h_stride;
+  const size_t cbase = (size_t)(a.kvq ? a.kvq[fi] : qi) * a.q_stride + (size_t)h * a.h_stride;
   const float* tbase = a.qkv + (size_t)seq * Lt * ld + h * DKV;
   {
     const int g = lane >> 4, li = lane & 15;
@@ -627,8 +719,9 @@
   const int fi = udiv_magic((unsigned)seq, a.B, b_magic), b = seq - fi * a.B;
   const int qi = a.flist[fi];
   const uint16_t* ancr = a.anc + ((size_t)qi * a.B + b) * a.anc_ld;
-  const float* kc = a.kcache + (size_t)qi * a.q_stride + (size_t)h * a.h_stride;
-  const float* vc = a.vcache + (size_t)qi * a.q_stride + (size_t)h * a.h_stride;
+  const int qc = a.kvq ? a.kvq[fi] : qi;
+  const float* kc = a.kcache + (size_t)qc * a.q_stride + (size_t)h * a.h_stride;
+  const float* vc = a.vcache + (size_t)qc * a.q_stride + (size_t)h * a.h_stride;
   const float* tbase = a.qkv + (size_t)seq * Lt * ld + h * DKV;
   const int kk_end = L > 24 ? 16 : L > 16 ? 12 : L > 8 ? 8 : 4;
   float4 kreg[8], qreg[8];
@@ -1331,10 +1424,94 @@
   return hipGetLastError();
 }
 
+__device__ void tail_rank_extras(const TailRankArgs& a, int i, int k) {
+  constexpr int CM = 64;
+  __shared__ double S[2][32], sc[CM];
+  __shared__ int slot[CM], lead[CM], flat[CM], nslot[CM], cseq[CM], alive[CM], orank[CM];
+  const int tid = threadIdx.x, nt = blockDim.x, B = a.B, T = a.T, L = a.L, Lt = L - T, C = 2 * B;
+  const int q = a.flist[i], es = *a.nf_dev + k;
+  const size_t r0 = (size_t)q * B, v0 = (size_t)(a.Qcap + k) * B;
+  const int32_t* parent = a.spare + a.Qcap + 1 + a.pool + (size_t)k * B;
+  if (tid < C) {
+    const int pb = tid < B ? tid : parent[tid - B];
+    alive[tid] = pb >= 0;
+    slot[tid] = pb >= 0 ? pb : 0;
+    cseq[tid] = tid < B ? i * B + tid : es * B + (tid - B);
+    orank[tid] = -1;
+  }
+  if (tid < B) S[0][tid] = a.st.score[r0 + tid];
+  __syncthreads();
+  int cur = 0;
+  for (int t = 0; t < Lt; ++t) {
+    const int p = T + t;
+    if (tid < C && alive[tid]) {
+      const int tok = a.tokens[(size_t)cseq[tid] * L + p], j = slot[tid];
+      int ld = tid;
+      for (int c = 0; c < tid; ++c)
+        if (alive[c] && slot[c] == j && a.tokens[(size_t)cseq[c] * L + p] == tok) { ld = c; break; }
+      lead[tid] = ld;
+      if (ld == tid) {
+        sc[tid] = ((double)a.gold[(size_t)cseq[tid] * Lt + t] + 0.0) + S[cur][j];
+        flat[tid] = j * 65536 + tok;
+      }
+    }
+    __syncthreads();
+    if (tid < C && alive[tid] && lead[tid] == tid) {
+      const double s = sc[tid];
+      const int fl = flat[tid];
+      int rk = 0;
+      for (int c = 0; c < C; ++c) rk += (alive[c] && lead[c] == c) && (sc[c] > s || (sc[c] == s && flat[c] < fl));
+      nslot[tid] = rk < B ? rk : -1;
+      if (rk < B) S[cur ^ 1][rk] = s;
+    }
+    __syncthreads();
+    if (tid < C && alive[tid]) {
+      const int ns = nslot[lead[tid]];
+      if (ns < 0) alive[tid] = 0; else slot[tid] = ns;
+    }
+    __syncthreads();
+    cur ^= 1;
+  }
+  if (tid < C && alive[tid]) {
+    bool first = true;
+    for (int c = 0; c < tid; ++c) first = first && !(alive[c] && slot[c] == slot[tid]);
+    if (first) {
+      const int pb = slot[tid];
+      const double s = S[cur][pb] / (double)(L + 1);
+      int rk = 0;
+      for (int c = 0; c < C; ++c) {
+        if (!alive[c] || c == tid) continue;
+        const double o = S[cur][slot[c]] / (double)(L + 1);
+        rk += (o > s) || (o == s && slot[c] > pb);
+      }
+      if (rk < B) {
+        const size_t o = (size_t)a.qmap[i] * B + rk;
+        orank[tid] = rk;
+        a.out_scores[o] = (float)s;
+        if (tid < B) {
+          const int lo = a.st.lo[r0 + tid];
+          a.out_lo[o] = lo;
+          a.out_hi[o] = seq_run_end(a.codes, a.Lc, lo, a.st.hi[r0 + tid], T, L);
+        } else {
+          a.out_lo[o] = a.st.lo[v0 + tid - B];
+          a.out_hi[o] = a.st.hi[v0 + tid - B];
+        }
+      }
+    }
+  }
+  __syncthreads();
+  const size_t o0 = (size_t)a.qmap[i] * B;
+  for (int x = tid; x < C * L; x += nt) {
+    const int c = x / L, p = x - c * L;
+    if (orank[c] >= 0) a.out_tokens[(o0 + orank[c]) * L + p] = (int32_t)a.tokens[(size_t)cseq[c] * L + p];
+  }
+}
+
 __global__ __launch_bounds__(1024) void tail_rank_kernel(TailRankArgs a) {
   extern __shared__ __attribute__((aligned(16))) unsigned char smem_raw[];
   const int i = blockIdx.x, tid = threadIdx.x, nt = blockDim.x;
   if (i >= *a.nf_dev) return;
+  if (a.pool > 0 && a.spare[i] >= 0) { tail_rank_extras(a, i, a.spare[i]); return; }
   const int B = a.B, T = a.T, L = a.L, Lt = L - T;
   double* S = reinterpret_cast<double*>(smem_raw);
   int* pos = reinterpret_cast<int*>(S + B);
@@ -1405,6 +1582,7 @@
   const int replay = rp ? atoi(rp) : 0;
   TailRankArgs a = a_in;
   if (replay) a.replay = 1;
+  if (a.pool > 0 && (a.B >= 32 || !a.spare || !a.codes)) return hipErrorInvalidValue;
   const size_t smem = (size_t)a.B * (sizeof(double) + 2 * sizeof(int)) + 16;
   hipLaunchKernelGGL(tail_rank_kernel, dim3(a.Qcap), dim3(a.B > 256 ? 1024 : 256), smem, s, a);
   return hipGetLastError();
diff --git a/ripor_amd/csrc/trie.cpp b/ripor_amd/csrc/trie.cpp
--- a/ripor_amd/csrc/trie.cpp
+++ b/ripor_amd/csrc/trie.cpp
@@ -83,7 +83,7 @@
   return 0;
 }
 
-void trie_single_frac(const uint16_t* sorted, int64_t N, int Lc, int L, std::vector<double>& frac) {
+void trie_single_frac(const uint16_t* sorted, int64_t N, int Lc, int L, std::vector<double>& frac, std::vector<double>* extra_mean) {
   std::vector<int64_t> nodes((size_t)L + 2, 0), single((size_t)L + 2, 0);
   int a = -1;
   for (int64_t i = 1; i <= N; ++i) {
@@ -100,11 +100,15 @@
     a = c;
   }
   frac.assign((size_t)L + 1, 0.0);
+  if (extra_mean) extra_mean->assign((size_t)L + 1, 0.0);
+  int64_t runs = 0;
+  for (int t = 0; t <= L + 1; ++t) runs += nodes[(size_t)t];
   int64_t n = 0, s = 0;
   for (int t = 0; t <= L; ++t) {
     n += nodes[(size_t)t];
     s += single[(size_t)t];
     frac[(size_t)t] = n ? (double)s / (double)n : 0.0;
+    if (extra_mean) (*extra_mean)[(size_t)t] = n ? (double)(runs - n) / (double)n : 0.0;
   }
 }
 
diff --git a/ripor_amd/csrc/trie.h b/ripor_amd/csrc/trie.h
--- a/ripor_amd/csrc/trie.h
+++ b/ripor_amd/csrc/trie.h
@@ -9,7 +9,8 @@
                    int64_t N, int L, int V, const std::string& keys, int64_t src_size, int64_t src_mtime_ns);
 int load_trie_file(const char* path, std::vector<uint16_t>& sorted, std::vector<int64_t>& perm, int64_t& N, int& L,
                    int& V, std::string& keys, std::string& err);
-void trie_single_frac(const uint16_t* sorted, int64_t N, int Lc, int L, std::vector<double>& frac);
+void trie_single_frac(const uint16_t* sorted, int64_t N, int Lc, int L, std::vector<double>& frac,
+                      std::vector<double>* extra_mean = nullptr);
 struct ChildLevels {
   std::vector<int32_t> lvl0, lvl1, idx2;
   struct Level { std::vector<int32_t> start; std::vector<uint16_t> tok; };
diff --git a/ripor_amd/engine.py b/ripor_amd/engine.py
--- a/ripor_amd/engine.py
+++ b/ripor_amd/engine.py
@@ -66,6 +66,12 @@
 
     def l0_table_bytes(self, model: "DeviceModel") -> int:
         return int(self.lib.rpr_l0_table_bytes(self.handle, model.handle))
+
+    def set_tail_extras(self, mode: int):
+        check(self.lib.rpr_set_tail_extras(self.handle, int(mode)), "rpr_set_tail_extras")
+
+    def tail_extras(self) -> int:
+        return int(self.lib.rpr_tail_extras(self.handle))
 
     def set_forced_tail(self, mode):
         check(self.lib.rpr_set_forced_tail(self.handle, int(mode)), "rpr_set_forced_tail")
@@ -222,6 +228,28 @@
     out = (C.c_double * (L + 1))()
     check(lib.rpr_trie_single_frac(codes.ctypes.data_as(C.c_void_p), N, Lc, L, out), "rpr_trie_single_frac")
     return np.asarray(list(out), dtype=np.float64)
+
+
+def trie_extra_mean(codes: np.ndarray, L: Optional[int] = None) -> np.ndarray:
+    lib = _lib.load()
+    codes = np.ascontiguousarray(codes, dtype=np.uint16)
+    N, Lc = codes.shape
+    L = Lc if L is None else int(L)
+    out = (C.c_double * (L + 1))()
+    check(lib.rpr_trie_extra_mean(codes.ctypes.data_as(C.c_void_p), N, Lc, L, out), "rpr_trie_extra_mean")
+    return np.array(out[:], dtype=np.float64)
+
+
+def plan_forks(single_frac: np.ndarray, extra_mean: np.ndarray, Q: int, B: int, L: int, forced_tail: int = 1,
+               tail_extras: int = -1):
+    lib = _lib.load()
+    f = (C.c_double * (L + 1))(*[float(x) for x in single_frac[:L + 1]])
+    mu = (C.c_double * (L + 1))(*[float(x) for x in extra_mean[:L + 1]])
+    depths, drop = (C.c_int32 * 2)(), C.c_int32(0)
+    n = int(lib.rpr_plan_forks(f, mu, int(Q), int(B), int(L), int(forced_tail), int(tail_extras), depths, C.byref(drop)))
+    if n < 0:
+        check(n, "rpr_plan_forks")
+    return [int(depths[i]) for i in range(n)], bool(drop.value)
 
 
 def trie_file_info(path: str) -> dict:
```

New measurement: 5023, median of 6. 1.02x the previous value.
